# Thealexbarney/VGAudio

Measured on AMD Instinct MI355X. Metric: Msamples/s encoded (GC-ADPCM, 4096 ch) at 1/2/4/8 GPUs; % HBM roofline, higher is better.
Workload: dtype int32; 1 GPU; BASELINE configs[1]: 4096 mono channels x 48 kHz x 60 s GC-ADPCM coefficient search + encode per GPU; parallelism=units sharded x1, channels_per_gpu=4096, samples_per_channel=2880000, bit_exact_channels_checked=0

## Files before the change

### include/vgaudio_hip_testing.h

```cpp
#ifndef VGAUDIO_HIP_TESTING_H
#define VGAUDIO_HIP_TESTING_H

#ifdef __cplusplus
extern "C" {
#endif

int vga_testing_force_open_seams_this_thread(int mode);

int vga_testing_gc_encoder_layout_this_thread(int channels_per_wave);
int vga_testing_gc_coefs_variant_this_thread(int variant);
int vga_testing_gc_encoder_segments_this_thread(int segments);
int vga_testing_gc_encoder_persistent_this_thread(int mode);

int vga_testing_gc_plan_pieces(int cus, int groups, int frames, long long group_frames, int ragged, int *out5);

int vga_testing_gc_encode_stats(unsigned long long *out8, int reset);
int vga_testing_gc_encode_stats_n(unsigned long long *out, int n, int reset);

int vga_testing_gc_seam_handover_this_thread(int on);
int vga_testing_gc_slow_order_host(const short *coefs, int nch, int *order);
int vga_testing_gc_slow_order_device(const void *d_coefs, int nch, int *order);

void vga_testing_host_pipeline_this_thread(int feeders, int drainers, int chunk_units, int slot_bytes);

void vga_testing_host_pipeline_tail_this_thread(int tail_units);

int vga_testing_plan_buckets(const int *group, const int *length, int n, int max_units, long long max_volume, int longest_first,
                             int *order_out, int *chunk_begin_out, int *chunk_length_out, int *chunk_group_out, int max_chunks);
void vga_testing_buckets_order_this_thread(int order);
void vga_testing_host_transfer_this_thread(int mode);
void vga_testing_host_transfer_piece_bytes_this_thread(int bytes);
void vga_testing_host_compute_lanes_this_thread(int lanes);

enum {
    VGA_TESTING_STEP_CHUNK_COMPUTE = 1,
    VGA_TESTING_STEP_TRANSFER = 2,
    VGA_TESTING_STEP_HCA_STREAM_FRAMES = 3
};
void vga_testing_fail_step_this_thread(int kind, int nth);

int vga_testing_last_pipeline_stats(double *out, int n);

int vga_testing_hca_frames_per_group_this_thread(int frames);

int vga_testing_hca_device_info(const void *hca_info, void *out, int out_bytes);

int vga_testing_hca_decode_classes(const void *infos, int nstreams, int *class_out);
int vga_testing_hca_decode_v_stats(long long *out, int n);
int vga_testing_hca_ragged_stats(const void *ragged, long long *out, int n);

int vga_testing_adx_read_general_this_thread(int on);

int vga_testing_adx_last_path_this_thread(int *encode, int *decode);
int vga_testing_adx_ragged_stats(const void *ragged, long long *out, int n);

int vga_testing_poison_allocations(int byte);

#ifdef __cplusplus
}
#endif
#endif
```

### vgaudio_amd/_lib.py

```python
import ctypes as C
import importlib.util
import os

_HERE = os.path.dirname(os.path.abspath(__file__))
SO_PATH = os.environ.get("VGAUDIO_HIP_LIBRARY") or os.path.join(_HERE, "libvgaudio_hip.so")

VGA_OK = 0
VGA_ERR_ARGUMENT = -1
VGA_ERR_OUT_OF_RANGE = -2
VGA_ERR_INVALID_DATA = -3
VGA_ERR_INVALID_OP = -4
VGA_ERR_DEVICE = -5

VGA_TESTING_STEP_CHUNK_COMPUTE = 1
VGA_TESTING_STEP_TRANSFER = 2
VGA_TESTING_STEP_HCA_STREAM_FRAMES = 3


class VgaError(RuntimeError):
    code = None


class ArgumentError(VgaError, ValueError):
    code = VGA_ERR_ARGUMENT


class ArgumentOutOfRangeError(ArgumentError):
    code = VGA_ERR_OUT_OF_RANGE


class InvalidDataError(VgaError):
    code = VGA_ERR_INVALID_DATA


class InvalidOperationError(VgaError):
    code = VGA_ERR_INVALID_OP


class DeviceError(VgaError):
    code = VGA_ERR_DEVICE


PROGRESS_FN = C.CFUNCTYPE(None, C.c_void_p, C.c_int64, C.c_int64)


class reporting:

    def __init__(self, progress, per_unit):
        self.progress, self.per_unit, self.last, self.fn = progress, per_unit, 0, None

    def _report(self, _user, done, _total):
        self.progress.ReportAdd((done - self.last) * self.per_unit)
        self.last = done

    def __enter__(self):
        if self.progress is not None:
            self.fn = PROGRESS_FN(self._report)
            lib().vga_set_progress_callback(C.cast(self.fn, C.c_void_p), None)
        return self

    def __exit__(self, *exc):
        if self.fn is not None:
            lib().vga_set_progress_callback(None, None)
        return False


_EXC = {e.code: e for e in (ArgumentError, ArgumentOutOfRangeError, InvalidDataError, InvalidOperationError,
                            DeviceError)}

_lib = None

i16p = C.POINTER(C.c_int16)
u8p = C.POINTER(C.c_uint8)
u32p = C.POINTER(C.c_uint32)
i16pp = C.POINTER(i16p)
u8pp = C.POINTER(u8p)
vp = C.c_void_p
i64 = C.c_int64
ci = C.c_int


class ADPCMINFO(C.Structure):
    _pack_ = 1
    _fields_ = [("coef", C.c_int16 * 16), ("gain", C.c_uint16), ("pred_scale", C.c_uint16), ("yn1", C.c_int16),
                ("yn2", C.c_int16), ("loop_pred_scale", C.c_uint16), ("loop_yn1", C.c_int16), ("loop_yn2", C.c_int16)]


SIGNATURES = {
    "vga_last_error": (C.c_char_p, []),
    "vga_device_count": (ci, []),
    "vga_set_device": (ci, [ci]),
    "vga_version": (C.c_char_p, []),
    "vga_gcadpcm_nibble_count_to_sample_count": (ci, [ci]),
    "vga_gcadpcm_sample_count_to_nibble_count": (ci, [ci]),
    "vga_gcadpcm_nibble_to_sample": (ci, [ci]),
    "vga_gcadpcm_sample_to_nibble": (ci, [ci]),
    "vga_gcadpcm_sample_count_to_byte_count": (ci, [ci]),
    "vga_gcadpcm_byte_count_to_sample_count": (ci, [ci]),
    "vga_gcadpcm_encode_batch": (ci, [i16pp, ci, ci, C.c_int16, C.c_int16, i16p, u8pp]),
    "vga_gcadpcm_calculate_coefficients_batch": (ci, [i16pp, ci, ci, i16p]),
    "vga_gcadpcm_encode_with_coefs_batch": (ci, [i16pp, ci, ci, ci, i16p, i16p, i16p, u8pp]),
    "vga_gcadpcm_decode_batch": (ci, [u8pp, i16p, ci, ci, i16p, i16p, i16pp]),
    "vga_gcadpcm_encode_batch_v": (ci, [i16pp, C.POINTER(ci), ci, i16p, i16p, i16p, u8pp]),
    "vga_gcadpcm_calculate_coefficients_batch_v": (ci, [i16pp, C.POINTER(ci), ci, i16p]),
    "vga_gcadpcm_encode_with_coefs_batch_v": (ci, [i16pp, C.POINTER(ci), ci, i16p, i16p, i16p, u8pp]),
    "vga_gcadpcm_decode_batch_v": (ci, [u8pp, i16p, C.POINTER(ci), ci, i16p, i16p, i16pp]),
    "vga_gcadpcm_ragged_create": (ci, [C.POINTER(ci), ci, C.POINTER(vp)]),
    "vga_gcadpcm_ragged_destroy": (None, [vp]),
    "vga_gcadpcm_ragged_channels": (ci, [vp]),
    "vga_gcadpcm_ragged_pcm_samples": (i64, [vp]),
    "vga_gcadpcm_ragged_adpcm_bytes": (i64, [vp]),
    "vga_gcadpcm_ragged_coefs_workspace_bytes": (C.c_size_t, [vp]),
    "vga_gcadpcm_ragged_offsets": (ci, [vp, C.POINTER(i64), C.POINTER(i64)]),
    "vga_gcadpcm_coefs_device_v": (ci, [vp, vp, vp, vp, C.c_size_t, vp]),
    "vga_gcadpcm_encode_device_v": (ci, [vp, vp, vp, vp, vp, vp, vp]),
    "vga_gcadpcm_decode_device_v": (ci, [vp, vp, vp, vp, vp, vp, vp, vp]),
    "encode": (None, [i16p, u8p, C.POINTER(ADPCMINFO), C.c_uint32]),
    "decode": (None, [u8p, i16p, C.POINTER(ADPCMINFO), C.c_uint32]),
    "correlateCoefs": (None, [i16p, C.c_uint32, i16p]),
    "encodeFrame": (None, [i16p, u8p, i16p, C.c_uint8]),
    "vga_gcadpcm_coefs_workspace_bytes": (C.c_size_t, [ci, ci]),
    "vga_gcadpcm_coefs_device": (ci, [vp, i64, ci, ci, vp, vp, C.c_size_t, vp]),
    "vga_gcadpcm_encode_device": (ci, [vp, i64, ci, ci, vp, vp, vp, vp, i64, vp]),
    "vga_gcadpcm_decode_device": (ci, [vp, i64, vp, ci, ci, vp, vp, vp, i64, vp, vp]),
    "vga_synth_pcm16_device": (ci, [vp, i64, ci, ci, ci, vp, vp]),
    "vga_adx_file_layout_for": (ci, [vp, ci, vp]),
    "vga_adx_write": (ci, [u8pp, ci, i16p, ci, vp, u8p]),
    "vga_adx_write_device": (ci, [vp, i64, ci, vp, ci, vp, vp, vp]),
    "vga_hca_file_size": (ci, [vp]),
    "vga_hca_file_header": (ci, [vp, C.c_char_p, C.c_float, ci, ci, u8p]),
    "vga_hca_write": (ci, [vp, u8p, C.c_char_p, C.c_float, ci, ci, u8p]),
    "vga_hca_write_device": (ci, [vp, vp, i64, ci, C.c_char_p, C.c_float, ci, ci, vp, i64, vp]),
    "vga_wave_parse": (ci, [u8p, i64, vp]),
    "vga_wave_read_pcm16": (ci, [u8p, i64, vp, i16pp]),
    "vga_wave_deinterleave_pcm16_device": (ci, [vp, ci, ci, vp, i64, vp]),
    "vga_wave_file_size": (i64, [vp, ci]),
    "vga_wave_write_pcm16": (ci, [i16pp, ci, vp, u8p]),
    "vga_wave_write_pcm16_device": (ci, [vp, i64, ci, vp, vp, vp]),
    "vga_adx_key_from_code": (ci, [C.c_uint64, vp]),
    "vga_adx_key_from_string": (ci, [C.c_char_p, vp]),
    "vga_adx_key_code": (C.c_uint64, [vp]),
    "vga_adx_crypt": (ci, [u8pp, ci, ci, vp, ci, ci]),
    "vga_adx_crypt_device": (ci, [vp, i64, ci, ci, vp, ci, ci, vp]),
    "vga_adx_find_key_device": (ci, [vp, i64, ci, ci, ci, ci, vp, ci, C.POINTER(ci), vp]),
    "vga_hca_key_tables": (ci, [ci, C.c_uint64, u8p, u8p]),
    "vga_hca_crypt": (ci, [u8p, ci, ci, u8p]),
    "vga_hca_find_key": (ci, [vp, u8p, ci, u8p, ci, vp]),
    "vga_hca_find_key_device": (ci, [vp, vp, ci, u8p, ci, vp, vp]),
    "vga_hca_byte_position_counts_device": (ci, [vp, i64, ci, ci, ci, ci, vp, vp]),
    "vga_adx_guess_default_candidates": (ci, [ci, vp, vp, vp, vp]),
    "vga_adx_guess_keys": (ci, [vp, ci, ci, ci, vp, ci, vp, ci, vp, ci, vp]),
    "vga_hca_crypt_device": (ci, [vp, i64, ci, ci, ci, u8p, vp]),
    "vga_release_cached_memory": (None, []),
    "vga_testing_force_open_seams_this_thread": (ci, [ci]),
    "vga_testing_host_pipeline_this_thread": (None, [ci, ci, ci, ci]),
    "vga_testing_gc_encoder_layout_this_thread": (ci, [ci]),
    "vga_testing_gc_coefs_variant_this_thread": (ci, [ci]),
    "vga_testing_gc_encoder_segments_this_thread": (ci, [ci]),
    "vga_testing_gc_encoder_persistent_this_thread": (ci, [ci]),
    "vga_testing_gc_seam_handover_this_thread": (ci, [ci]),
    "vga_testing_gc_slow_order_host": (ci, [vp, ci, vp]),
    "vga_testing_gc_slow_order_device": (ci, [vp, ci, vp]),
    "vga_testing_gc_encode_stats_n": (ci, [C.POINTER(C.c_ulonglong), ci, ci]),
    "vga_testing_last_pipeline_stats": (ci, [vp, ci]),
    "vga_testing_host_pipeline_tail_this_thread": (None, [ci]),
    "vga_testing_buckets_order_this_thread": (None, [ci]),
    "vga_testing_host_transfer_this_thread": (None, [ci]),
    "vga_testing_host_transfer_piece_bytes_this_thread": (None, [ci]),
    "vga_testing_host_compute_lanes_this_thread": (None, [ci]),
    "vga_testing_fail_step_this_thread": (None, [ci, ci]),
    "vga_testing_poison_allocations": (ci, [ci]),
    "vga_testing_plan_buckets": (ci, [C.POINTER(ci), C.POINTER(ci), ci, ci, C.c_longlong, ci, C.POINTER(ci), C.POINTER(ci), C.POINTER(ci),
                                 C.POINTER(ci), ci]),
    "vga_testing_hca_device_info": (ci, [vp, vp, ci]),
    "vga_testing_hca_decode_classes": (ci, [vp, ci, C.POINTER(ci)]),
    "vga_testing_hca_decode_v_stats": (ci, [C.POINTER(C.c_longlong), ci]),
    "vga_testing_hca_ragged_stats": (ci, [vp, C.POINTER(C.c_longlong), ci]),
    "vga_hca_ragged_layout_for": (ci, [vp, ci, C.POINTER(i64), C.POINTER(i64), vp]),
    "vga_hca_ragged_create": (ci, [vp, ci, C.POINTER(vp)]),
    "vga_hca_ragged_destroy": (None, [vp]),
    "vga_hca_ragged_streams": (ci, [vp]),
    "vga_hca_ragged_totals_of": (ci, [vp, vp]),
    "vga_hca_ragged_offsets": (ci, [vp, C.POINTER(i64), C.POINTER(i64)]),
    "vga_testing_adx_ragged_stats": (ci, [vp, C.POINTER(C.c_longlong), ci]),
    "vga_adx_ragged_layout_for": (ci, [vp, C.POINTER(ci), ci, C.POINTER(i64), C.POINTER(i64), vp]),
    "vga_adx_ragged_create": (ci, [vp, C.POINTER(ci), ci, C.POINTER(vp)]),
    "vga_adx_ragged_destroy": (None, [vp]),
    "vga_adx_ragged_channels": (ci, [vp]),
    "vga_adx_ragged_totals_of": (ci, [vp, vp]),
    "vga_adx_ragged_offsets": (ci, [vp, C.POINTER(i64), C.POINTER(i64)]),
    "vga_adx_encode_device_v": (ci, [vp, vp, vp, vp, vp, C.c_size_t, vp]),
    "vga_adx_decode_device_v": (ci, [vp, vp, vp, vp, C.c_size_t, vp, vp]),
    "vga_gc_files_layout_for": (ci, [vp, ci, vp, C.POINTER(ci), C.POINTER(i64), C.POINTER(i64), vp]),
    "vga_gc_files_create": (ci, [vp, ci, vp, C.POINTER(vp)]),
    "vga_gc_files_create_from_dsp": (ci, [C.POINTER(vp), ci, C.POINTER(i64), C.POINTER(vp)]),
    "vga_gc_files_destroy": (None, [vp]),
    "vga_gc_files_totals_of": (ci, [vp, vp]),
    "vga_gc_files_offsets": (ci, [vp, C.POINTER(ci), C.POINTER(i64), C.POINTER(i64)]),
    "vga_gc_files_ragged": (vp, [vp]),
    "vga_gcadpcm_build_channels_device_v": (ci, [vp, vp, vp, vp, vp, vp, vp, vp, C.c_size_t, vp]),
    "vga_dsp_write_device_v": (ci, [vp, vp, vp, vp, vp, vp, vp, vp]),
    "vga_dsp_read_device_v": (ci, [vp, vp, vp, vp, vp, vp, vp, vp]),
    "vga_gc_aligned_layout_for": (ci, [vp, ci, C.POINTER(ci), C.POINTER(i64), vp]),
    "vga_gc_aligned_create": (ci, [vp, ci, C.POINTER(vp)]),
    "vga_gc_aligned_destroy": (None, [vp]),
    "vga_gc_aligned_totals_of": (ci, [vp, vp]),
    "vga_gc_aligned_offsets": (ci, [vp, C.POINTER(ci), C.POINTER(i64)]),
    "vga_gc_aligned_ragged_in": (vp, [vp]),
    "vga_gc_aligned_ragged_out": (vp, [vp]),
    "vga_gcadpcm_align_channels_device_v": (ci, [vp, vp, vp, vp, vp, vp, vp, vp, vp, C.c_size_t, vp]),
    "vga_nw_files_layout_for": (ci, [vp, ci, vp, C.POINTER(ci), C.POINTER(i64), C.POINTER(i64), vp]),
    "vga_nw_files_create": (ci, [vp, ci, vp, C.POINTER(vp)]),
    "vga_nw_files_create_from_infos": (ci, [C.POINTER(vp), ci, C.POINTER(i64), C.POINTER(vp)]),
    "vga_nw_files_destroy": (None, [vp]),
    "vga_nw_files_totals_of": (ci, [vp, vp]),
    "vga_nw_files_offsets": (ci, [vp, C.POINTER(ci), C.POINTER(i64), C.POINTER(i64)]),
    "vga_nw_files_gc_files": (ci, [vp, vp]),
    "vga_nw_files_ragged": (vp, [vp]),
    "vga_nwstm_write_device_v": (ci, [vp, vp, vp, vp, vp, vp, vp, vp, vp]),
    "vga_nwstm_read_device_v": (ci, [vp, vp, vp, vp, vp, vp, vp, vp]),
    "vga_idsp_files_layout_for": (ci, [vp, ci, vp, C.POINTER(ci), C.POINTER(i64), vp]),
    "vga_idsp_files_create": (ci, [vp, ci, vp, C.POINTER(vp)]),
    "vga_idsp_files_create_from_infos": (ci, [C.POINTER(vp), ci, C.POINTER(i64), C.POINTER(vp)]),
    "vga_idsp_files_destroy": (None, [vp]),
    "vga_idsp_files_totals_of": (ci, [vp, vp]),
    "vga_idsp_files_offsets": (ci, [vp, C.POINTER(ci), C.POINTER(i64)]),
    "vga_idsp_files_gc_files": (ci, [vp, vp]),
    "vga_idsp_files_ragged": (vp, [vp]),
    "vga_idsp_write_device_v": (ci, [vp, vp, vp, vp, vp, vp, vp, vp]),
    "vga_idsp_read_device_v": (ci, [vp, vp, vp, vp, vp, vp, vp, vp]),
    "vga_idsp_files_write_regions_for": (ci, [vp, ci, vp, vp, i64, C.POINTER(i64)]),
    "vga_idsp_files_read_regions_for": (ci, [C.POINTER(vp), ci, C.POINTER(i64), vp, i64, C.POINTER(i64)]),
    "vga_idsp_files_stats": (ci, [vp, C.POINTER(i64)]),
    "vga_hps_files_layout_for": (ci, [vp, ci, C.POINTER(ci), C.POINTER(i64), C.POINTER(i64), vp]),
    "vga_hps_files_create": (ci, [vp, ci, C.POINTER(vp)]),
    "vga_hps_files_create_from_infos": (ci, [C.POINTER(vp), C.POINTER(vp), ci, C.POINTER(i64), C.POINTER(vp)]),
    "vga_hps_files_destroy": (None, [vp]),
    "vga_hps_files_totals_of": (ci, [vp, vp]),
    "vga_hps_files_offsets": (ci, [vp, C.POINTER(ci), C.POINTER(i64), C.POINTER(i64)]),
    "vga_hps_files_gc_files": (ci, [vp, vp]),
    "vga_hps_files_ragged": (vp, [vp]),
    "vga_hps_write_device_v": (ci, [vp, vp, vp, vp, vp, vp, vp, vp]),
    "vga_hps_read_device_v": (ci, [vp, vp, vp, vp, vp, vp, vp, vp]),
    "vga_hps_files_write_regions_for": (ci, [vp, ci, vp, i64, C.POINTER(i64)]),
    "vga_hps_files_read_regions_for": (ci, [C.POINTER(vp), C.POINTER(vp), ci, C.POINTER(i64), vp, i64, C.POINTER(i64)]),
    "vga_hps_files_stats": (ci, [vp, C.POINTER(i64)]),
    "vga_hca_decode_device_v": (ci, [vp, vp, vp, vp, C.c_size_t, vp, vp]),
    "vga_hca_encode_device_v": (ci, [vp, vp, vp, vp, vp]),
    "vga_hca_stream_create": (ci, [vp, vp, C.POINTER(vp)]),
    "vga_hca_stream_encode": (ci, [vp, vp, u8p, C.POINTER(ci)]),
    "vga_hca_stream_pending_frame_count": (ci, [vp]),
    "vga_hca_stream_get_pending_frame": (ci, [vp, u8p]),
    "vga_hca_stream_frames_processed": (ci, [vp]),
    "vga_hca_stream_frame_size": (ci, [vp]),
    "vga_hca_stream_destroy": (None, [vp]),
    "vga_testing_gc_encode_stats": (ci, [C.POINTER(C.c_ulonglong), ci]),
    "vga_testing_gc_plan_pieces": (ci, [ci, ci, ci, C.c_longlong, ci, C.POINTER(ci)]),
    "vga_set_devices": (ci, [vp, ci]),
    "vga_set_progress_callback": (ci, [vp, vp]),
    "vga_get_devices": (ci, [vp, ci]),
    "vga_testing_hca_frames_per_group_this_thread": (ci, [ci]),
    "vga_dsp_layout_for": (ci, [vp, ci, vp]),
    "vga_dsp_write": (ci, [u8pp, ci, i16p, i16p, i16p, i16p, ci, vp, u8p]),
    "vga_dsp_write_device": (ci, [vp, i64, ci, vp, vp, vp, vp, ci, vp, vp, vp]),
    "vga_nwstm_layout_for": (ci, [vp, ci, vp]),
    "vga_nwstm_write_device": (ci, [vp, ci, ci, vp, vp, i64, ci, vp, vp, vp, vp, vp, i64, ci, vp, i64, vp]),
    "vga_nwstm_write": (ci, [vp, ci, vp, u8pp, ci, i16p, i16p, i16p, i16p, i16pp, ci, u8p]),
    "vga_nwstm_parse": (ci, [u8p, C.c_size_t, vp]),
    "vga_nwstm_read_device": (ci, [vp, vp, i64, ci, vp, i64, vp]),
    "vga_nwstm_read": (ci, [u8p, C.c_size_t, vp, u8pp, i16pp]),
    "vga_pcm8_encode_device": (ci, [vp, i64, ci, ci, ci, vp, i64, vp]),
    "vga_pcm8_decode_device": (ci, [vp, i64, ci, ci, ci, vp, i64, vp]),
    "vga_nwstm_pcm_layout_for": (ci, [vp, ci, ci, vp]),
    "vga_nwstm_pcm_write_device": (ci, [vp, ci, ci, ci, vp, vp, ci, i64, vp, i64, vp]),
    "vga_nwstm_pcm_write": (ci, [vp, ci, ci, vp, vp, ci, u8p]),
    "vga_nwstm_pcm_parse": (ci, [u8p, C.c_size_t, vp]),
    "vga_nwstm_pcm_read_device": (ci, [vp, vp, i64, ci, vp, ci, i64, vp]),
    "vga_nwstm_pcm_read": (ci, [u8p, C.c_size_t, vp, vp, ci]),
    "vga_nwwav_parse": (ci, [u8p, C.c_size_t, vp]),
    "vga_nwwav_read": (ci, [u8p, C.c_size_t, vp, u8pp]),
    "vga_nwwav_bank_create": (ci, [vp, C.POINTER(i64), ci, C.POINTER(vp)]),
    "vga_nwwav_bank_destroy": (None, [vp]),
    "vga_nwwav_bank_channels": (ci, [vp]),
    "vga_nwwav_bank_codec_channels": (ci, [vp, ci]),
    "vga_nwwav_bank_rows": (ci, [vp, C.POINTER(ci), C.POINTER(ci), C.POINTER(ci), C.POINTER(ci), C.POINTER(i64)]),
    "vga_nwwav_bank_gc_sample_counts": (ci, [vp, C.POINTER(ci)]),
    "vga_nwwav_bank_gc_tables": (ci, [vp, i16p, i16p, i16p, i16p]),
    "vga_nwwav_bank_adpcm_bytes": (i64, [vp]),
    "vga_nwwav_bank_pcm16_samples": (i64, [vp]),
    "vga_nwwav_bank_pcm8_bytes": (i64, [vp]),
    "vga_nwwav_bank_source_bytes": (i64, [vp]),
    "vga_nwwav_bank_read_device": (ci, [vp, vp, vp, vp, vp, vp]),
    "vga_wave_pcm8_file_size": (i64, [vp, ci]),
    "vga_wave_write_pcm8": (ci, [vp, ci, ci, vp, u8p]),
    "vga_wave_write_pcm8_device": (ci, [vp, ci, i64, ci, vp, vp, vp]),
    "vga_wave_read_pcm8": (ci, [u8p, i64, vp, vp, ci]),
    "vga_wave_deinterleave_pcm8_device": (ci, [vp, ci, ci, vp, ci, i64, vp]),
    "vga_hps_layout_for": (ci, [vp, ci, vp]),
    "vga_hps_block_map": (ci, [vp, ci, vp, ci]),
    "vga_hps_write_device": (ci, [vp, ci, ci, vp, i64, ci, vp, vp, vp, vp, i64, ci, vp, i64, vp]),
    "vga_hps_write": (ci, [vp, ci, u8pp, ci, i16p, i16p, i16p, i16pp, ci, u8p]),
    "vga_hps_parse": (ci, [u8p, C.c_size_t, vp, vp, ci]),
    "vga_hps_read_device": (ci, [vp, vp, vp, i64, ci, vp, i64, vp]),
    "vga_hps_read": (ci, [u8p, C.c_size_t, vp, vp, u8pp]),
    "vga_idsp_layout_for": (ci, [vp, ci, vp]),
    "vga_idsp_write_device": (ci, [vp, ci, ci, vp, i64, ci, vp, vp, vp, vp, vp, i64, vp]),
    "vga_idsp_write": (ci, [vp, ci, u8pp, ci, i16p, i16p, i16p, i16p, u8p]),
    "vga_idsp_parse": (ci, [u8p, C.c_size_t, vp]),
    "vga_idsp_read_device": (ci, [vp, vp, i64, ci, vp, i64, vp]),
    "vga_idsp_read": (ci, [u8p, C.c_size_t, vp, u8pp]),
    "vga_genh_parse": (ci, [u8p, C.c_size_t, vp]),
    "vga_genh_read_device": (ci, [vp, vp, i64, ci, vp, i64, vp]),
    "vga_genh_read": (ci, [u8p, C.c_size_t, vp, u8pp]),
    "vga_dsp_parse": (ci, [u8p, C.c_size_t, vp]),
    "vga_dsp_read_device": (ci, [vp, vp, i64, ci, vp, i64, vp]),
    "vga_dsp_read": (ci, [u8p, C.c_size_t, vp, u8pp]),
    "vga_adx_parse": (ci, [u8p, C.c_size_t, vp]),
    "vga_adx_read_device": (ci, [vp, vp, i64, ci, vp, i64, vp]),
    "vga_adx_read": (ci, [u8p, C.c_size_t, vp, u8pp]),
    "vga_hca_parse": (ci, [u8p, C.c_size_t, vp]),
    "vga_hca_read_device": (ci, [vp, vp, i64, ci, vp, i64, vp, vp]),
    "vga_hca_read": (ci, [u8p, C.c_size_t, vp, u8p, C.POINTER(ci)]),
    "vga_testing_adx_read_general_this_thread": (ci, [ci]),
    "vga_testing_adx_last_path_this_thread": (ci, [C.POINTER(ci), C.POINTER(ci)]),
    "vga_gcadpcm_channel_layout_for": (ci, [vp, vp]),
    "vga_gcadpcm_build_channels_batch": (ci, [u8pp, i16p, ci, vp, u8pp, i16pp, i16pp, i16p]),
    "vga_gcadpcm_build_channels_workspace_bytes": (C.c_size_t, [ci, vp]),
    "vga_gcadpcm_build_channels_device": (ci, [vp, i64, vp, ci, vp, vp, i64, vp, i64, vp, i64, vp, vp, C.c_size_t, vp]),
    "vga_adx_default_params": (None, [vp]),
    "vga_adx_calculate_coefficients": (ci, [ci, ci, i16p]),
    "vga_adx_nibble_count_to_sample_count": (ci, [ci, ci]),
    "vga_adx_sample_count_to_nibble_count": (ci, [ci, ci]),
    "vga_adx_sample_count_to_byte_count": (ci, [ci, ci]),
    "vga_adx_encoded_byte_count": (ci, [ci, vp]),
    "vga_adx_encode_batch": (ci, [i16pp, ci, ci, vp, u8pp, i16p]),
    "vga_adx_decode_batch": (ci, [u8pp, ci, ci, ci, vp, i16pp]),
    "vga_adx_encode_batch_v": (ci, [i16pp, C.POINTER(ci), ci, vp, u8pp, i16p]),
    "vga_adx_decode_batch_v": (ci, [u8pp, C.POINTER(ci), ci, C.POINTER(ci), vp, i16pp]),
    "vga_hca_encode_batch_v": (ci, [i16pp, ci, vp, vp, u8pp]),
    "vga_hca_decode_batch_v": (ci, [vp, u8pp, ci, i16pp]),
    "vga_adx_encode_device": (ci, [vp, i64, ci, ci, vp, vp, i64, vp, vp]),
    "vga_adx_decode_device": (ci, [vp, i64, ci, ci, ci, vp, vp, i64, vp, vp]),
    "vga_hca_encoder_initialize": (ci, [vp, vp]),
    "vga_hca_encode_batch": (ci, [i16pp, ci, vp, vp, u8pp]),
    "vga_hca_decode_batch": (ci, [vp, u8pp, ci, i16pp]),
    "vga_hca_decode_workspace_bytes": (C.c_size_t, [vp, ci]),
    "vga_hca_encode_device": (ci, [vp, i64, i64, ci, ci, vp, vp, i64, vp, vp]),
    "vga_hca_decode_device": (ci, [vp, vp, i64, ci, vp, i64, i64, vp, C.c_size_t, vp, vp]),
    "vga_adx_files_layout_for": (ci, [vp, ci, C.POINTER(i64), C.POINTER(ci), C.POINTER(i64), C.POINTER(i64), vp]),
    "vga_adx_files_create": (ci, [vp, ci, C.POINTER(i64), C.POINTER(vp)]),
    "vga_adx_files_create_from_infos": (ci, [vp, ci, C.POINTER(i64), C.POINTER(vp)]),
    "vga_adx_files_destroy": (None, [vp]),
    "vga_adx_files_totals_of": (ci, [vp, vp]),
    "vga_adx_files_offsets": (ci, [vp, C.POINTER(ci), C.POINTER(i64), C.POINTER(i64)]),
    "vga_adx_write_device_v": (ci, [vp, vp, vp, vp, vp]),
    "vga_adx_read_device_v": (ci, [vp, vp, vp, vp, vp]),
    "vga_adx_files_write_items_for": (ci, [vp, ci, C.POINTER(i64), ci, vp, i64, C.POINTER(i64)]),
    "vga_adx_files_read_items_for": (ci, [vp, ci, C.POINTER(i64), ci, vp, i64, C.POINTER(i64)]),
    "vga_adx_files_stats": (ci, [vp, C.POINTER(i64)]),
    "vga_adx_files_force_general_this_thread": (ci, [ci]),
    "vga_wave_files_layout_for": (ci, [vp, ci, C.POINTER(i64), C.POINTER(i64), C.POINTER(ci), C.POINTER(i64), C.POINTER(i64), vp]),
    "vga_wave_files_create": (ci, [vp, ci, C.POINTER(i64), C.POINTER(i64), C.POINTER(vp)]),
    "vga_wave_files_create_from_infos": (ci, [vp, ci, C.POINTER(i64), C.POINTER(i64), C.POINTER(vp)]),
    "vga_wave_files_destroy": (None, [vp]),
    "vga_wave_files_totals_of": (ci, [vp, vp]),
    "vga_wave_files_offsets": (ci, [vp, C.POINTER(ci), C.POINTER(i64), C.POINTER(i64)]),
    "vga_wave_read_device_v": (ci, [vp, vp, vp, vp]),
    "vga_wave_write_device_v": (ci, [vp, vp, vp, vp]),
    "vga_wave_files_write_items_for": (ci, [vp, ci, C.POINTER(i64), C.POINTER(i64), ci, vp, i64, C.POINTER(i64)]),
    "vga_wave_files_read_items_for": (ci, [vp, ci, C.POINTER(i64), C.POINTER(i64), ci, vp, i64, C.POINTER(i64)]),
    "vga_wave_files_stats": (ci, [vp, C.POINTER(i64)]),
    "vga_wave_files_force_general_this_thread": (ci, [ci]),
    "vga_nw_pcm_files_layout_for": (ci, [vp, ci, vp, ci, C.POINTER(i64), C.POINTER(i64), C.POINTER(ci), C.POINTER(i64), C.POINTER(i64), vp]),
    "vga_nw_pcm_files_create": (ci, [vp, ci, vp, ci, C.POINTER(i64), C.POINTER(i64), C.POINTER(vp)]),
    "vga_nw_pcm_files_create_from_infos": (ci, [vp, ci, C.POINTER(i64), C.POINTER(i64), C.POINTER(vp)]),
    "vga_nw_pcm_files_destroy": (None, [vp]),
    "vga_nw_pcm_files_totals_of": (ci, [vp, vp]),
    "vga_nw_pcm_files_offsets": (ci, [vp, C.POINTER(ci), C.POINTER(i64), C.POINTER(i64)]),
    "vga_nwstm_pcm_write_device_v": (ci, [vp, vp, vp, vp]),
    "vga_nwstm_pcm_read_device_v": (ci, [vp, vp, vp, vp]),
    "vga_nw_pcm_files_write_items_for": (ci, [vp, ci, vp, ci, C.POINTER(i64), C.POINTER(i64), ci, vp, i64, C.POINTER(i64)]),
    "vga_nw_pcm_files_read_items_for": (ci, [vp, ci, C.POINTER(i64), C.POINTER(i64), ci, vp, i64, C.POINTER(i64)]),
    "vga_nw_pcm_files_stats": (ci, [vp, C.POINTER(i64)]),
    "vga_nw_pcm_files_force_general_this_thread": (ci, [ci]),
    "vga_hca_files_layout_for": (ci, [vp, ci, C.POINTER(i64), C.POINTER(i64), C.POINTER(i64), vp]),
    "vga_hca_files_create": (ci, [vp, ci, C.POINTER(i64), vp, ci, C.POINTER(vp)]),
    "vga_hca_files_create_from_infos": (ci, [vp, ci, C.POINTER(i64), C.POINTER(ci), vp, ci, C.POINTER(i64), C.POINTER(vp)]),
    "vga_hca_files_destroy": (None, [vp]),
    "vga_hca_files_totals_of": (ci, [vp, vp]),
    "vga_hca_files_offsets": (ci, [vp, C.POINTER(i64), C.POINTER(i64)]),
    "vga_hca_write_device_v": (ci, [vp, vp, vp, vp]),
    "vga_hca_read_device_v": (ci, [vp, vp, vp, vp, vp]),
    "vga_hca_files_write_items_for": (ci, [vp, ci, C.POINTER(i64), ci, vp, i64, C.POINTER(i64)]),
    "vga_hca_files_read_items_for": (ci, [vp, ci, C.POINTER(i64), C.POINTER(i64), ci, vp, i64, C.POINTER(i64)]),
    "vga_hca_files_stats": (ci, [vp, C.POINTER(i64)]),
    "vga_hca_files_force_general_this_thread": (ci, [ci]),
}


class AdxFileParamsC(C.Structure):
    _fields_ = [(n, C.c_int) for n in ("sample_rate", "sample_count", "looping", "loop_start", "loop_end", "alignment_samples",
                                       "frame_size", "version", "type", "highpass_frequency", "encryption_type", "trim_file")]


class AdxFileLayoutC(C.Structure):
    _fields_ = [(n, C.c_int) for n in ("sample_count", "frame_count", "base_header_size", "alignment_bytes", "header_size",
                                       "audio_offset", "audio_size", "footer_offset", "footer_size", "loop_start_offset",
                                       "loop_end_offset", "file_size")]


class AdxFileC(C.Structure):
    _fields_ = [("channels", C.c_int), ("params", AdxFileParamsC)]


class AdxFilesTotalsC(C.Structure):
    _fields_ = [("files", C.c_int), ("channels", C.c_int), ("audio_bytes", C.c_int64), ("image_bytes", C.c_int64)]


class AdxFilesItemC(C.Structure):
    _fields_ = [("form", C.c_int), ("file", C.c_int), ("x", C.c_int), ("y", C.c_uint32), ("granule", C.c_int),
                ("begin", C.c_int64), ("end", C.c_int64), ("keep_end", C.c_int64)]


class WaveInfoC(C.Structure):
    _fields_ = ([(n, C.c_int) for n in ("channel_count", "sample_rate", "bits_per_sample", "sample_count", "sample_count_declared",
                                        "looping", "loop_start", "loop_end")]
                + [("data_offset", C.c_int64), ("data_size", C.c_int), ("data_size_declared", C.c_int)])


class WaveParamsC(C.Structure):
    _fields_ = [(n, C.c_int) for n in ("sample_rate", "sample_count", "looping", "loop_start", "loop_end")]


class WaveFileC(C.Structure):
    _fields_ = [("channels", C.c_int), ("bits", C.c_int), ("params", WaveParamsC)]


class WaveFilesTotalsC(C.Structure):
    _fields_ = [("files", C.c_int), ("channels", C.c_int), ("pcm_samples", C.c_int64), ("image_bytes", C.c_int64)]


class WaveFilesItemC(C.Structure):
    _fields_ = [("form", C.c_int), ("file", C.c_int), ("x", C.c_int), ("y", C.c_uint32), ("span", C.c_int),
                ("begin", C.c_int64), ("end", C.c_int64)]


class AdxKeyC(C.Structure):
    _fields_ = [("seed", C.c_int), ("mult", C.c_int), ("inc", C.c_int)]


class DspParamsC(C.Structure):
    _fields_ = [(n, C.c_int) for n in ("sample_rate", "sample_count", "looping", "loop_start", "loop_end",
                                       "samples_per_interleave", "loop_point_alignment", "trim_file")]


class DspLayoutC(C.Structure):
    _fields_ = [(n, C.c_int) for n in ("sample_count", "loop_start", "loop_end", "start_addr", "end_addr", "cur_addr",
                                       "bytes_per_interleave", "frames_per_interleave", "audio_data_size", "file_size")]


class GcChannelParamsC(C.Structure):
    _fields_ = [(n, C.c_int) for n in ("sample_count", "looping", "loop_start", "loop_end", "loop_alignment_multiple",
                                       "samples_per_seek_table_entry")]


class GcChannelLayoutC(C.Structure):
    _fields_ = [(n, C.c_int) for n in ("alignment_needed", "loop_start_aligned", "sample_count_aligned",
                                       "seek_table_entries")]


class GcFileC(C.Structure):
    _fields_ = [("channels", C.c_int), ("sample_rate", C.c_int), ("channel", GcChannelParamsC)]


class DspFileConfigC(C.Structure):
    _fields_ = [(n, C.c_int) for n in ("samples_per_interleave", "loop_point_alignment", "trim_file")]


class GcFilesTotalsC(C.Structure):
    _fields_ = [("files", C.c_int), ("channels", C.c_int), ("pcm_samples", C.c_int64), ("adpcm_bytes", C.c_int64),
                ("seek_shorts", C.c_int64), ("image_bytes", C.c_int64), ("build_workspace_bytes", C.c_size_t)]


class GcAlignedTotalsC(C.Structure):
    _fields_ = [("files", C.c_int), ("channels", C.c_int), ("aligned_channels", C.c_int), ("pcm_samples", C.c_int64),
                ("adpcm_bytes", C.c_int64), ("out_pcm_samples", C.c_int64), ("out_adpcm_bytes", C.c_int64), ("seek_shorts", C.c_int64),
                ("workspace_bytes", C.c_size_t)]


NW_MAX_CHANNELS = NW_MAX_TRACKS = 255


class NwTrackC(C.Structure):
    _fields_ = [(n, C.c_int) for n in ("channel_count", "left", "right", "volume", "panning")]


class NwParamsC(C.Structure):
    _fields_ = ([(n, C.c_int) for n in ("target", "sample_rate", "sample_count", "looping", "loop_start", "loop_end",
                                        "samples_per_interleave", "samples_per_seek_table_entry", "loop_point_alignment",
                                        "track_type", "seek_table_type")]
                + [("version", C.c_uint32)]
                + [(n, C.c_int) for n in ("endianness", "track_count", "keep_seek_table", "keep_loop_context")])


class NwLayoutC(C.Structure):
    _fields_ = ([("target", C.c_int), ("endianness", C.c_int), ("version", C.c_uint32)]
                + [(n, C.c_int) for n in ("include_track_info", "include_region_info", "include_unaligned_loop",
                                          "version_word", "looping", "loop_start", "loop_end", "sample_count",
                                          "alignment_needed")]
                + [("channel", GcChannelParamsC)]
                + [(n, C.c_int) for n in (
                    "channel_sample_count", "channel_adpcm_bytes", "channel_seek_entries", "samples_per_interleave",
                    "interleave_size", "interleave_count", "last_block_samples", "last_block_size_without_padding",
                    "last_block_size", "samples_per_seek_table_entry", "bytes_per_seek_table_entry",
                    "seek_table_entry_count", "track_count", "header_size", "head_block_offset", "head_block_size",
                    "head1_size", "head2_size", "head3_size", "seek_block_offset", "seek_block_size",
                    "data_block_offset", "data_block_size", "audio_data_offset", "audio_data_size", "file_size")])


class NwInfoC(C.Structure):
    _fields_ = ([("target", C.c_int), ("endianness", C.c_int), ("version", C.c_uint32)]
                + [(n, C.c_int) for n in (
                    "codec", "looping", "loop_start", "sample_count", "sample_rate", "channel_count", "has_unaligned_loop",
                    "loop_start_unaligned", "loop_end_unaligned", "interleave_count", "interleave_size",
                    "samples_per_interleave", "last_block_size_without_padding", "last_block_samples", "last_block_size",
                    "bytes_per_seek_table_entry", "samples_per_seek_table_entry", "track_type", "seek_table_type",
                    "has_track_info", "track_count")]
                + [("tracks", NwTrackC * NW_MAX_TRACKS), ("coefs", (C.c_int16 * 16) * NW_MAX_CHANNELS),
                   ("gain", C.c_int16 * NW_MAX_CHANNELS), ("start_context", (C.c_int16 * 3) * NW_MAX_CHANNELS),
                   ("loop_context", (C.c_int16 * 3) * NW_MAX_CHANNELS)]
                + [(n, C.c_int) for n in (
                    "seek_table_offset", "seek_entries", "seek_big_endian", "head_block_offset", "head_block_size",
                    "seek_block_offset", "seek_block_size", "data_block_offset", "data_block_size", "audio_data_offset",
                    "audio_data_length", "adpcm_bytes", "file_size")])


class NwFileC(C.Structure):
    _fields_ = [(n, C.c_int) for n in ("channels", "sample_rate", "sample_count", "looping", "loop_start", "loop_end")]


class NwFileConfigC(C.Structure):
    _fields_ = ([(n, C.c_int) for n in ("target", "samples_per_interleave", "samples_per_seek_table_entry", "loop_point_alignment",
                                        "track_type", "seek_table_type")]
                + [("version", C.c_uint32), ("endianness", C.c_int)])


class NwFilesTotalsC(C.Structure):
    _fields_ = [("files", C.c_int), ("channels", C.c_int), ("pcm_samples", C.c_int64), ("adpcm_bytes", C.c_int64),
                ("seek_shorts", C.c_int64), ("image_bytes", C.c_int64)]


class NwPcmFilesTotalsC(C.Structure):
    _fields_ = [("files", C.c_int), ("channels", C.c_int), ("pcm_samples", C.c_int64), ("image_bytes", C.c_int64)]


class NwPcmFilesItemC(C.Structure):
    _fields_ = [("form", C.c_int), ("file", C.c_int), ("x", C.c_int), ("y", C.c_uint32), ("conv", C.c_int),
                ("begin", C.c_int64), ("end", C.c_int64)]


# ... 202 lines not shown
```

### vgaudio_amd/csrc/capi_gcadpcm.hip

```cpp
#include "gc_capi.hpp"
#include "../../include/vgaudio_hip_testing.h"

using namespace vga;

extern "C" {

int vga_testing_gc_plan_pieces(int cus, int groups, int frames, long long group_frames, int ragged, int *out5)
{
    if (!out5 || cus <= 0 || groups <= 0 || frames <= 0) return -1;
    bool persistent = false;
    gc::Pieces seg;
    const int segments = gc::plan_encode_pieces_on(cus, groups, frames, group_frames, ragged != 0, &persistent, &seg,
                                                     encoder_layout() == 1 ? 1 : 8);
    out5[0] = segments;
    out5[1] = seg.big;
    out5[2] = seg.nb;
    out5[3] = seg.small;
    out5[4] = persistent ? 1 : 0;
    return 0;
}

int vga_gcadpcm_nibble_count_to_sample_count(int nibble_count) { return gc::nibble_count_to_sample_count(nibble_count); }
int vga_gcadpcm_sample_count_to_nibble_count(int sample_count) { return gc::sample_count_to_nibble_count(sample_count); }
int vga_gcadpcm_nibble_to_sample(int nibble) { return gc::nibble_to_sample(nibble); }
int vga_gcadpcm_sample_to_nibble(int sample) { return gc::sample_to_nibble(sample); }
int vga_gcadpcm_sample_count_to_byte_count(int sample_count) { return gc::sample_count_to_byte_count(sample_count); }
int vga_gcadpcm_byte_count_to_sample_count(int byte_count) { return gc::byte_count_to_sample_count(byte_count); }

size_t vga_gcadpcm_coefs_workspace_bytes(int nch, int length)
{
    if (nch <= 0 || length < 0) return 0;
    const size_t frames = ((size_t)length + 13) / 14;
    return (size_t)nch * (size_t)vga::gc::coef_record_pitch((int64_t)frames) * 16;
}

int vga_gcadpcm_coefs_device(const int16_t *d_pcm, int64_t pcm_pitch, int nch, int length, int16_t *d_coefs,
                             void *d_workspace, size_t workspace_bytes, void *stream)
{
    if (nch < 0 || length < 0) { set_error("negative size"); return VGA_ERR_ARGUMENT; }
    if (nch == 0) return VGA_OK;
    if (int rc = gc::check_pcm_layout(d_pcm, pcm_pitch, length, "vga_gcadpcm_coefs_device")) return rc;
    if (workspace_bytes < vga_gcadpcm_coefs_workspace_bytes(nch, length) || !d_workspace) {
        set_error("workspace too small: need %zu bytes", vga_gcadpcm_coefs_workspace_bytes(nch, length));
        return VGA_ERR_ARGUMENT;
    }
    return gc::launch_coefs(d_pcm, pcm_pitch, nch, length, d_coefs, d_workspace, (hipStream_t)stream);
}

int vga_gcadpcm_encode_device(const int16_t *d_pcm, int64_t pcm_pitch, int nch, int sample_count,
                              const int16_t *d_coefs, const int16_t *d_hist1, const int16_t *d_hist2,
                              uint8_t *d_adpcm, int64_t adpcm_pitch, void *stream)
{
    if (nch < 0 || sample_count < 0) { set_error("negative size"); return VGA_ERR_ARGUMENT; }
    if (nch == 0 || sample_count == 0) return VGA_OK;
    if (int rc = gc::check_pcm_layout(d_pcm, pcm_pitch, sample_count, "vga_gcadpcm_encode_device")) return rc;
    if (int rc = gc::check_adpcm_layout(d_adpcm, adpcm_pitch, gc::sample_count_to_byte_count(sample_count),
                                    "vga_gcadpcm_encode_device"))
        return rc;
    return gc::launch_encode(d_pcm, pcm_pitch, nch, sample_count, d_coefs, d_hist1, d_hist2, d_adpcm, adpcm_pitch,
                             (hipStream_t)stream);
}

int vga_gcadpcm_decode_device(const uint8_t *d_adpcm, int64_t adpcm_pitch, const int16_t *d_coefs, int nch,
                              int sample_count, const int16_t *d_hist1, const int16_t *d_hist2, int16_t *d_pcm,
                              int64_t pcm_pitch, int *d_status, void *stream)
{
    if (nch < 0 || sample_count < 0) { set_error("negative size"); return VGA_ERR_ARGUMENT; }
    if (nch == 0 || sample_count == 0) return VGA_OK;
    if (int rc = gc::check_pcm_layout(d_pcm, pcm_pitch, sample_count, "vga_gcadpcm_decode_device")) return rc;
    if (int rc = gc::check_adpcm_layout(d_adpcm, adpcm_pitch, gc::sample_count_to_byte_count(sample_count),
                                    "vga_gcadpcm_decode_device"))
        return rc;
    return gc::launch_decode(d_adpcm, adpcm_pitch, d_coefs, nch, sample_count, d_hist1, d_hist2, d_pcm, pcm_pitch,
                             d_status, (hipStream_t)stream);
}

int vga_synth_pcm16_device(int16_t *d_pcm, int64_t pcm_pitch, int nch, int length, int first_channel,
                           const uint32_t *d_params, void *stream)
{
    if (nch < 0 || length < 0 || pcm_pitch < length) { set_error("bad synth arguments"); return VGA_ERR_ARGUMENT; }
    return gc::launch_synth(d_pcm, pcm_pitch, nch, length, first_channel, d_params, (hipStream_t)stream);
}

static constexpr int GC_CHUNK_CHANNELS = 1024;

static int calculate_coefficients_batch_one(const int16_t *const *pcm, int nch, int length, int16_t *coefs_out)
{
    if (length < 0) { set_error("negative length"); return VGA_ERR_ARGUMENT; }
    if (int rc = gc::check_ptrs((const void *const *)pcm, length > 0 ? nch : 0, "pcm")) return rc;
    if (nch < 0 || (nch > 0 && !coefs_out)) { set_error("bad coefs_out/nch"); return VGA_ERR_ARGUMENT; }
    if (nch == 0) return VGA_OK;
    if (int rc = require_device()) return rc;
    gc::GcBatch b;
    b.pcm_pitch = round_up(length > 0 ? length : 1, 8);
    VGA_HIP_TRY(b.pcm.alloc((size_t)nch * b.pcm_pitch * sizeof(int16_t)));
    VGA_HIP_TRY(b.coefs.alloc((size_t)nch * 32));
    pipe::Job job;
    job.units = nch;
    if (length > 0) bind_in(job, (const void *const *)pcm, (size_t)length * sizeof(int16_t), b.pcm.as<char>(), (size_t)b.pcm_pitch * sizeof(int16_t));
    job.compute = chunk_compute([&](int first, int count, hipStream_t s) {
        return gc::launch_coefs(b.pcm.as<int16_t>() + (int64_t)first * b.pcm_pitch, b.pcm_pitch, count, length,
                                b.coefs.as<int16_t>() + (int64_t)first * 16, b.ws.p, s);
    });
    VGA_HIP_TRY(b.ws.alloc(vga_gcadpcm_coefs_workspace_bytes(planned_chunk_units(job, GC_CHUNK_CHANNELS), length)));
    if (int rc = run_batch_pipeline(job, GC_CHUNK_CHANNELS)) return rc;
    VGA_HIP_TRY(hipMemcpy(coefs_out, b.coefs.p, (size_t)nch * 32, hipMemcpyDeviceToHost));
    return VGA_OK;
}

int vga_gcadpcm_calculate_coefficients_batch(const int16_t *const *pcm, int nch, int length, int16_t *coefs_out)
{
    if (nch <= 0 || !pcm || !coefs_out) return calculate_coefficients_batch_one(pcm, nch, length, coefs_out);
    return for_each_device_share(nch, gc::GC_MIN_SHARE_CHANNELS, [&](int first, int count) {
        return calculate_coefficients_batch_one(pcm + first, count, length, coefs_out + (size_t)first * 16);
    });
}

static int encode_with_coefs_batch_one(const int16_t *const *pcm, int nch, int pcm_length, int sample_count, const int16_t *coefs,
                                      const int16_t *hist1, const int16_t *hist2, uint8_t *const *adpcm_out)
{
    if (sample_count == -1) sample_count = pcm_length;
    if (pcm_length < 0 || sample_count < 0) { set_error("negative length"); return VGA_ERR_ARGUMENT; }
    if (sample_count > pcm_length) {
        set_error("SampleCount (%d) exceeds pcm length (%d)", sample_count, pcm_length);
        return VGA_ERR_ARGUMENT;
    }
    if (int rc = gc::check_ptrs((const void *const *)pcm, sample_count > 0 ? nch : 0, "pcm")) return rc;
    if (int rc = gc::check_ptrs((const void *const *)adpcm_out, sample_count > 0 ? nch : 0, "adpcm_out")) return rc;
    if (nch > 0 && !coefs) { set_error("null coefs"); return VGA_ERR_ARGUMENT; }
    if (nch <= 0 || sample_count == 0) return nch < 0 ? VGA_ERR_ARGUMENT : VGA_OK;
    if (int rc = require_device()) return rc;
    gc::GcBatch b;
    VGA_HIP_TRY(b.st.create());
    b.pcm_pitch = round_up(sample_count, 8);
    VGA_HIP_TRY(b.pcm.alloc((size_t)nch * b.pcm_pitch * sizeof(int16_t)));
    if (int rc = gc::upload_hist(b.h1, b.h2, nch, hist1, hist2, &b.st)) return rc;
    VGA_HIP_TRY(b.coefs.alloc((size_t)nch * 32));
    VGA_HIP_TRY(hipMemcpyAsync(b.coefs.p, coefs, (size_t)nch * 32, hipMemcpyHostToDevice, b.st.s));
    VGA_HIP_TRY(hipStreamSynchronize(b.st.s));
    const int nbytes = gc::sample_count_to_byte_count(sample_count);
    b.adpcm_pitch = round_up(nbytes, 16);
    VGA_HIP_TRY(b.adpcm.alloc((size_t)nch * b.adpcm_pitch));
    DevBuf scratch;
    pipe::Job job;
    job.units = nch;
    bind_in(job, (const void *const *)pcm, (size_t)sample_count * sizeof(int16_t), b.pcm.as<char>(), (size_t)b.pcm_pitch * sizeof(int16_t));
    bind_out(job, (void *const *)adpcm_out, (size_t)nbytes, b.adpcm.as<char>(), (size_t)b.adpcm_pitch);
    job.compute = chunk_compute([&](int first, int count, hipStream_t s) {
        return gc::launch_encode(b.pcm.as<int16_t>() + (int64_t)first * b.pcm_pitch, b.pcm_pitch, count, sample_count,
                                 b.coefs.as<int16_t>() + (int64_t)first * 16,
                                 b.h1.p ? b.h1.as<int16_t>() + first : nullptr, b.h2.p ? b.h2.as<int16_t>() + first : nullptr,
                                 b.adpcm.as<uint8_t>() + (int64_t)first * b.adpcm_pitch, b.adpcm_pitch, s, scratch.p, scratch.bytes);
    });
    VGA_HIP_TRY(scratch.alloc(gc::encode_scratch_bytes(planned_chunk_units(job, GC_CHUNK_CHANNELS))));
    return run_batch_pipeline(job, GC_CHUNK_CHANNELS);
}

int vga_gcadpcm_encode_with_coefs_batch(const int16_t *const *pcm, int nch, int pcm_length, int sample_count,
                                        const int16_t *coefs, const int16_t *hist1, const int16_t *hist2,
                                        uint8_t *const *adpcm_out)
{
    if (nch <= 0 || !pcm || !coefs || !adpcm_out)
        return encode_with_coefs_batch_one(pcm, nch, pcm_length, sample_count, coefs, hist1, hist2, adpcm_out);
    return for_each_device_share(nch, gc::GC_MIN_SHARE_CHANNELS, [&](int first, int count) {
        return encode_with_coefs_batch_one(pcm + first, count, pcm_length, sample_count, coefs + (size_t)first * 16,
                                          hist1 ? hist1 + first : nullptr, hist2 ? hist2 + first : nullptr, adpcm_out + first);
    });
}

static int encode_batch_one(const int16_t *const *pcm, int nch, int sample_count, int16_t hist1, int16_t hist2, int16_t *coefs_out,
                           uint8_t *const *adpcm_out)
{
    if (sample_count < 0) { set_error("negative sample count"); return VGA_ERR_ARGUMENT; }
    if (int rc = gc::check_ptrs((const void *const *)pcm, sample_count > 0 ? nch : 0, "pcm")) return rc;
    if (int rc = gc::check_ptrs((const void *const *)adpcm_out, sample_count > 0 ? nch : 0, "adpcm_out")) return rc;
    if (nch < 0 || (nch > 0 && !coefs_out)) { set_error("bad coefs_out/nch"); return VGA_ERR_ARGUMENT; }
    if (nch == 0) return VGA_OK;
    if (int rc = require_device()) return rc;
    const double t_entry = pipe::detail::now();
    gc::GcBatch b;
    VGA_HIP_TRY(b.st.create());
    b.pcm_pitch = round_up(sample_count > 0 ? sample_count : 1, 8);
    VGA_HIP_TRY(b.pcm.alloc((size_t)nch * b.pcm_pitch * sizeof(int16_t)));
    std::vector<int16_t> h1v((size_t)nch, hist1), h2v((size_t)nch, hist2);
    const bool use_hist = hist1 != 0 || hist2 != 0;
    if (use_hist)
        if (int rc = gc::upload_hist(b.h1, b.h2, nch, h1v.data(), h2v.data(), &b.st)) return rc;
    VGA_HIP_TRY(hipStreamSynchronize(b.st.s));
    VGA_HIP_TRY(b.coefs.alloc((size_t)nch * 32));
    const int nbytes = gc::sample_count_to_byte_count(sample_count);
    b.adpcm_pitch = round_up(nbytes > 0 ? nbytes : 1, 16);
    VGA_HIP_TRY(b.adpcm.alloc((size_t)nch * b.adpcm_pitch));
    DevBuf scratch[pipe::kMaxComputeLanes], ws[pipe::kMaxComputeLanes];
    pipe::Job job;
    job.units = nch;
    job.compute_lanes = nch > 1 ? planned_compute_lanes(hardware_queues_requested() >= 6 ? 2 : 1) : 1;
    if (sample_count > 0) {
        bind_in(job, (const void *const *)pcm, (size_t)sample_count * sizeof(int16_t), b.pcm.as<char>(), (size_t)b.pcm_pitch * sizeof(int16_t));
        bind_out(job, (void *const *)adpcm_out, (size_t)nbytes, b.adpcm.as<char>(), (size_t)b.adpcm_pitch);
    }
    job.compute = chunk_compute([&](int first, int count, hipStream_t s) {
        const int lane = pipe::compute_lane();
        int rc = gc::launch_coefs(b.pcm.as<int16_t>() + (int64_t)first * b.pcm_pitch, b.pcm_pitch, count, sample_count,
                                  b.coefs.as<int16_t>() + (int64_t)first * 16, ws[lane].p, s);
        if (!rc)
            rc = gc::launch_encode(b.pcm.as<int16_t>() + (int64_t)first * b.pcm_pitch, b.pcm_pitch, count, sample_count,
                                   b.coefs.as<int16_t>() + (int64_t)first * 16,
                                   b.h1.p ? b.h1.as<int16_t>() + first : nullptr, b.h2.p ? b.h2.as<int16_t>() + first : nullptr,
                                   b.adpcm.as<uint8_t>() + (int64_t)first * b.adpcm_pitch, b.adpcm_pitch, s, scratch[lane].p,
                                   scratch[lane].bytes);
        return rc;
    });
    const int chunk = planned_chunk_units(job, GC_CHUNK_CHANNELS);
    for (int l = 0; l < job.compute_lanes; l++) {
        VGA_HIP_TRY(scratch[l].alloc(gc::encode_scratch_bytes(chunk)));
        VGA_HIP_TRY(ws[l].alloc(vga_gcadpcm_coefs_workspace_bytes(chunk, sample_count)));
    }
    pipe_report().t_alloc = pipe::detail::now() - t_entry;
    if (int rc = run_batch_pipeline(job, GC_CHUNK_CHANNELS)) return rc;
    VGA_HIP_TRY(hipMemcpy(coefs_out, b.coefs.p, (size_t)nch * 32, hipMemcpyDeviceToHost));
    pipe_report().t_entry = pipe::detail::now() - t_entry;
    return VGA_OK;
}

int vga_gcadpcm_encode_batch(const int16_t *const *pcm, int nch, int sample_count, int16_t hist1, int16_t hist2,
                             int16_t *coefs_out, uint8_t *const *adpcm_out)
{
    if (nch <= 0 || !pcm || !coefs_out || !adpcm_out) return encode_batch_one(pcm, nch, sample_count, hist1, hist2, coefs_out, adpcm_out);
    return for_each_device_share(nch, gc::GC_MIN_SHARE_CHANNELS, [&](int first, int count) {
        return encode_batch_one(pcm + first, count, sample_count, hist1, hist2, coefs_out + (size_t)first * 16, adpcm_out + first);
    });
}

static int decode_batch_one(const uint8_t *const *adpcm, const int16_t *coefs, int nch, int sample_count, const int16_t *hist1,
                           const int16_t *hist2, int16_t *const *pcm_out)
{
    if (sample_count < 0) { set_error("negative sample count"); return VGA_ERR_ARGUMENT; }
    if (int rc = gc::check_ptrs((const void *const *)adpcm, sample_count > 0 ? nch : 0, "adpcm")) return rc;
    if (int rc = gc::check_ptrs((const void *const *)pcm_out, sample_count > 0 ? nch : 0, "pcm_out")) return rc;
    if (nch > 0 && !coefs) { set_error("null coefs"); return VGA_ERR_ARGUMENT; }
    if (nch <= 0 || sample_count == 0) return nch < 0 ? VGA_ERR_ARGUMENT : VGA_OK;
    if (int rc = require_device()) return rc;
    gc::GcBatch b;
    VGA_HIP_TRY(b.st.create());
    const int nbytes = gc::sample_count_to_byte_count(sample_count);
    b.adpcm_pitch = round_up(nbytes, 16);
    b.pcm_pitch = round_up(sample_count, 8);
    VGA_HIP_TRY(b.adpcm.alloc((size_t)nch * b.adpcm_pitch));
    VGA_HIP_TRY(b.pcm.alloc((size_t)nch * b.pcm_pitch * 2));
    VGA_HIP_TRY(b.coefs.alloc((size_t)nch * 32));
    VGA_HIP_TRY(b.status.alloc(sizeof(int)));
    VGA_HIP_TRY(hipMemsetAsync(b.status.p, 0, sizeof(int), b.st.s));
    VGA_HIP_TRY(hipMemcpyAsync(b.coefs.p, coefs, (size_t)nch * 32, hipMemcpyHostToDevice, b.st.s));
    if (int rc = gc::upload_hist(b.h1, b.h2, nch, hist1, hist2, &b.st)) return rc;
    VGA_HIP_TRY(hipStreamSynchronize(b.st.s));
    pipe::Job job;
    job.units = nch;
    bind_in(job, (const void *const *)adpcm, (size_t)nbytes, b.adpcm.as<char>(), (size_t)b.adpcm_pitch);
    bind_out(job, (void *const *)pcm_out, (size_t)sample_count * 2, b.pcm.as<char>(), (size_t)b.pcm_pitch * 2);
    job.compute_lanes = planned_compute_lanes(1);
    job.compute = chunk_compute([&](int first, int count, hipStream_t s) {
        return gc::launch_decode(b.adpcm.as<uint8_t>() + (int64_t)first * b.adpcm_pitch, b.adpcm_pitch,
                                 b.coefs.as<int16_t>() + (int64_t)first * 16, count, sample_count,
                                 b.h1.p ? b.h1.as<int16_t>() + first : nullptr, b.h2.p ? b.h2.as<int16_t>() + first : nullptr,
                                 b.pcm.as<int16_t>() + (int64_t)first * b.pcm_pitch, b.pcm_pitch, b.status.as<int>(), s);
    });
    return run_status_job(job, 2 * GC_CHUNK_CHANNELS, b.status, gc::BAD_PREDICTOR);
}

int vga_gcadpcm_decode_batch(const uint8_t *const *adpcm, const int16_t *coefs, int nch, int sample_count,
                             const int16_t *hist1, const int16_t *hist2, int16_t *const *pcm_out)
{
    if (nch <= 0 || !adpcm || !coefs || !pcm_out) return decode_batch_one(adpcm, coefs, nch, sample_count, hist1, hist2, pcm_out);
    return for_each_device_share(nch, gc::GC_MIN_SHARE_CHANNELS, [&](int first, int count) {
        return decode_batch_one(adpcm + first, coefs + (size_t)first * 16, count, sample_count, hist1 ? hist1 + first : nullptr,
                               hist2 ? hist2 + first : nullptr, pcm_out + first);
    });
}

void correlateCoefs(int16_t *src, uint32_t samples, int16_t *coefsOut)
{
    const int16_t *chans[1] = {src};
    (void)vga_gcadpcm_calculate_coefficients_batch(chans, 1, (int)samples, coefsOut);
}

void encode(int16_t *src, uint8_t *dst, ADPCMINFO *cxt, uint32_t samples)
{
    const int16_t *chans[1] = {src};
    uint8_t *outs[1] = {dst};
    int16_t coefs[16];
    if (vga_gcadpcm_encode_batch(chans, 1, (int)samples, 0, 0, coefs, outs) != VGA_OK) return;
    if (cxt) {
        memset(cxt, 0, sizeof *cxt);
        memcpy(cxt->coef, coefs, sizeof coefs);
        cxt->pred_scale = samples ? dst[0] : 0;
    }
}

void decode(uint8_t *src, int16_t *dst, ADPCMINFO *cxt, uint32_t samples)
{
    if (!cxt) return;
    const uint8_t *ins[1] = {src};
    int16_t *outs[1] = {dst};
    int16_t coefs[16];
    memcpy(coefs, cxt->coef, sizeof coefs);
    const int16_t h1 = cxt->yn1, h2 = cxt->yn2;
    (void)vga_gcadpcm_decode_batch(ins, coefs, 1, (int)samples, &h1, &h2, outs);
}

void encodeFrame(int16_t *src, uint8_t *dst, int16_t *coefs, uint8_t one)
{
    (void)one;
    const int16_t *chans[1] = {src + 2};
    uint8_t *outs[1] = {dst};
    const int16_t h2 = src[0], h1 = src[1];
    if (vga_gcadpcm_encode_with_coefs_batch(chans, 1, 14, 14, coefs, &h1, &h2, outs) != VGA_OK) return;
    const uint8_t *ins[1] = {dst};
    int16_t *rec[1] = {src + 2};
    (void)vga_gcadpcm_decode_batch(ins, coefs, 1, 14, &h1, &h2, rec);
}

// ... 2 lines not shown
```

### vgaudio_amd/csrc/common.hpp

```cpp
#pragma once
#include <hip/hip_runtime.h>
#include <cstdarg>
#include <cstdint>
#include <cstdio>
#include <cstdlib>
#include <cstring>
#include <mutex>
#include <vector>

#include "../../include/vgaudio_hip.h"
#include "poison.hpp"

namespace vga {

void set_error(const char *fmt, ...);
bool take_error_pending();

#define VGA_HIP_TRY(expr)                                                              \
    do {                                                                               \
        hipError_t _e = (expr);                                                        \
        if (_e != hipSuccess) {                                                        \
            vga::set_error("%s failed: %s (%s:%d)", #expr, hipGetErrorString(_e),      \
                           __FILE__, __LINE__);                                        \
            return VGA_ERR_DEVICE;                                                     \
        }                                                                              \
    } while (0)

inline hipError_t poison_block(void *p, size_t bytes)
{
    const int byte = poison_byte();
    if (byte < 0 || !p || !bytes) return hipSuccess;
    const hipError_t e = hipMemset(p, byte, bytes);
    return e != hipSuccess ? e : hipStreamSynchronize(nullptr);
}
inline hipError_t device_malloc(void **out, size_t bytes)
{
    const hipError_t e = hipMalloc(out, bytes);
    return e != hipSuccess ? e : poison_block(*out, bytes);
}

class DevicePool {
public:
    static DevicePool &get()
    {
        static DevicePool pool;
        return pool;
    }
    hipError_t acquire(void **out, size_t bytes)
    {
        const hipError_t e = acquire_block(out, bytes);
        return e != hipSuccess ? e : poison_block(*out, bytes ? bytes : 1);
    }
    void release(void *p)
    {
        std::vector<void *> drop;
        {
            std::lock_guard<std::mutex> g(m_);
            bool pooled = false;
            int device = -1;
            for (auto &b : blocks_)
                if (b.p == p) { b.busy = false; pooled = true; device = b.device; }
            size_t idle = 0;
            for (auto &b : blocks_)
                if (!b.busy && b.device == device) idle += b.bytes;
            if (!pooled) drop.push_back(p);
            const size_t keep = keep_bytes();
            while (idle > keep) {
                int big = -1;
                for (int i = 0; i < (int)blocks_.size(); i++)
                    if (!blocks_[i].busy && blocks_[i].device == device && (big < 0 || blocks_[i].bytes > blocks_[big].bytes)) big = i;
                if (big < 0) break;
                idle -= blocks_[big].bytes;
                drop.push_back(blocks_[big].p);
                blocks_.erase(blocks_.begin() + big);
            }
        }
        for (void *q : drop) (void)hipFree(q);
    }
    void trim()
    {
        std::vector<void *> drop;
        {
            std::lock_guard<std::mutex> g(m_);
            for (int i = (int)blocks_.size() - 1; i >= 0; i--)
                if (!blocks_[i].busy) {
                    drop.push_back(blocks_[i].p);
                    blocks_.erase(blocks_.begin() + i);
                }
        }
        for (void *q : drop) (void)hipFree(q);
    }

    int device_of(void *p)
    {
        std::lock_guard<std::mutex> g(m_);
        for (auto &b : blocks_)
            if (b.p == p) return b.device;
        return -1;
    }

private:
    static constexpr size_t kMinPooled = (size_t)1 << 20;
    hipError_t acquire_block(void **out, size_t bytes)
    {
        if (bytes < kMinPooled) return hipMalloc(out, bytes ? bytes : 1);
        int device = 0;
        (void)hipGetDevice(&device);
        {
            std::lock_guard<std::mutex> g(m_);
            int best = -1;
            for (int i = 0; i < (int)blocks_.size(); i++) {
                const Block &b = blocks_[i];
                if (!b.busy && b.device == device && b.bytes >= bytes && b.bytes / 2 <= bytes &&
                    (best < 0 || b.bytes < blocks_[best].bytes))
                    best = i;
            }
            if (best >= 0) {
                blocks_[best].busy = true;
                *out = blocks_[best].p;
                return hipSuccess;
            }
        }
        hipError_t e = hipMalloc(out, bytes);
        if (e != hipSuccess) {
            trim();
            e = hipMalloc(out, bytes);
        }
        if (e == hipSuccess) {
            std::lock_guard<std::mutex> g(m_);
            blocks_.push_back({*out, bytes, device, true});
        }
        return e;
    }
    static size_t keep_bytes()
    {
        static const size_t v = [] {
            const char *e = std::getenv("VGA_HIP_POOL_GIB");
            const long gib = e ? std::atol(e) : 64;
            return (size_t)(gib < 0 ? 0 : gib) << 30;
        }();
        return v;
    }
    struct Block { void *p; size_t bytes; int device; bool busy; };
    std::mutex m_;
    std::vector<Block> blocks_;
};

struct DevBuf {
    void *p = nullptr;
    size_t bytes = 0;
    DevBuf() = default;
    DevBuf(const DevBuf &) = delete;
    DevBuf &operator=(const DevBuf &) = delete;
    ~DevBuf() { drop(); }
    void drop()
    {
        if (!p) return;
        if (take_error_pending()) {
            const int dev = DevicePool::get().device_of(p);
            int cur = -1;
            if (dev >= 0 && hipGetDevice(&cur) == hipSuccess && cur != dev && hipSetDevice(dev) == hipSuccess) {
                (void)hipDeviceSynchronize();
                (void)hipSetDevice(cur);
            } else
                (void)hipDeviceSynchronize();
        }
        DevicePool::get().release(p);
        p = nullptr;
    }
    hipError_t alloc(size_t n) {
        drop();
        bytes = n;
        return DevicePool::get().acquire(&p, n ? n : 1);
    }
    template <class T> T *as() const { return reinterpret_cast<T *>(p); }
};

struct AsyncBuf {
    void *p = nullptr;
    hipStream_t stream = nullptr;
    AsyncBuf() = default;
    AsyncBuf(const AsyncBuf &) = delete;
    AsyncBuf &operator=(const AsyncBuf &) = delete;
    ~AsyncBuf() { if (p) (void)hipFreeAsync(p, stream); }
    hipError_t alloc(size_t n, hipStream_t s) {
        stream = s;
        const hipError_t e = hipMallocAsync(&p, n ? n : 1, s);
        const int byte = poison_byte();
        return e != hipSuccess || byte < 0 ? e : hipMemsetAsync(p, byte, n ? n : 1, s);
    }
    template <class T> T *as() const { return reinterpret_cast<T *>(p); }
};

template <class F>
inline hipError_t allow_dynamic_lds(F *kernel, size_t bytes)
{
    return hipFuncSetAttribute(reinterpret_cast<const void *>(kernel), hipFuncAttributeMaxDynamicSharedMemorySize, (int)bytes);
}

struct Stream {
    hipStream_t s = nullptr;
    ~Stream() { if (s) (void)hipStreamDestroy(s); }
    hipError_t create() { return hipStreamCreateWithFlags(&s, hipStreamNonBlocking); }
};

inline int64_t round_up(int64_t v, int64_t m) { return (v + m - 1) / m * m; }

__device__ __forceinline__ void lds_barrier()
{
#if defined(__HIP_DEVICE_COMPILE__)
    asm volatile("s_waitcnt lgkmcnt(0)\n\ts_barrier" ::: "memory");
#endif
}

int require_device();

inline int device_cu_count()
{
    int device = 0, cus = 256;
    if (hipGetDevice(&device) == hipSuccess) (void)hipDeviceGetAttribute(&cus, hipDeviceAttributeMultiprocessorCount, device);
    return cus > 0 ? cus : 256;
}

int force_open_seams();

int encoder_layout();
int coefs_kernel_variant();
int encoder_segments_override();
int encoder_persistent_mode();
int hca_frames_per_group_override();
bool gc_seam_handover_off();
void note_adx_encode_path(int path);
void note_adx_decode_path(int path);

__host__ __device__ inline bool seam_forced_open(int mode, int channel, int seam)
{
    return mode == 1 || mode == 3 || (mode == 2 && channel % 3 == 0 && seam % 2 == 0);
}

}
```

### vgaudio_amd/csrc/gc_encode_kernel.hip

```cpp
#include "common.hpp"
#include "gc_encode_core.hpp"
#include "gcadpcm_kernels.hpp"
#include "seams.hpp"
#include "gc_plan8.hpp"

#include <cstdio>
#include <cstdlib>
#include <vector>

namespace vga {
namespace gc {

constexpr int DPP_QUAD_XOR1 = 0xB1;
constexpr int DPP_QUAD_XOR2 = 0x4E;
constexpr int DPP_ROW_HALF_MIRROR = 0x141;
constexpr int DPP_ROW_MIRROR = 0x140;

template <int CTRL>
__device__ __forceinline__ int dpp(int v)
{
    return __builtin_amdgcn_update_dpp(0, v, CTRL, 0xF, 0xF, true);
}

__device__ __forceinline__ unsigned umin32(unsigned a, unsigned b) { return a < b ? a : b; }

template <class Op>
__device__ __forceinline__ unsigned row16_reduce(unsigned v, Op op)
{
    v = op(v, (unsigned)dpp<DPP_QUAD_XOR1>((int)v));
    v = op(v, (unsigned)dpp<DPP_QUAD_XOR2>((int)v));
    v = op(v, (unsigned)dpp<DPP_ROW_HALF_MIRROR>((int)v));
    v = op(v, (unsigned)dpp<DPP_ROW_MIRROR>((int)v));
    return v;
}


#ifdef VGA_DEBUG_TIMESTAMPS
__device__ unsigned long long g_vga_enc_ts[1 << 16];
extern "C" int vga_debug_encode_timestamps(unsigned long long *out, int n)
{
    return (int)hipMemcpyFromSymbol(out, HIP_SYMBOL(g_vga_enc_ts), (size_t)n * sizeof(unsigned long long));
}
#endif
constexpr int GC_STATS = 9;
__device__ unsigned long long g_vga_gc_stats[GC_STATS];
extern "C" int vga_testing_gc_encode_stats_n(unsigned long long *out, int n, int reset)
{
    if (n < 0 || n > GC_STATS) return -1;
    if (hipDeviceSynchronize() != hipSuccess) return -1;
    if (out && n > 0 && hipMemcpyFromSymbol(out, HIP_SYMBOL(g_vga_gc_stats), (size_t)n * sizeof(unsigned long long)) != hipSuccess) return -1;
#ifdef VGA_GC_STATS
    if (out && n > 7) out[7] = 1;
#else
    if (out && n > 7) out[7] = 0;
#endif
    if (reset) {
        const unsigned long long zero[GC_STATS] = {};
        if (hipMemcpyToSymbol(HIP_SYMBOL(g_vga_gc_stats), zero, sizeof zero) != hipSuccess) return -1;
    }
    return 0;
}
extern "C" int vga_testing_gc_encode_stats(unsigned long long *out8, int reset) { return vga_testing_gc_encode_stats_n(out8, 8, reset); }
constexpr int SW = 2;
constexpr int ENC_THREADS = 64 * (SW + 1);
#ifndef VGA_GC_ENCODER_PRIO
#define VGA_GC_ENCODER_PRIO 3
#endif
#ifndef VGA_GC_HELPER_PRIO
#define VGA_GC_HELPER_PRIO 0
#endif
#ifndef VGA_GC_PERSISTENT_WAVES_PER_EU
#define VGA_GC_PERSISTENT_WAVES_PER_EU 3, 3
#endif
template <int CPW, bool SELF = false>
struct Lay {
    static_assert(!SELF || CPW == 8, "the self-served shape is the (channel, predictor) layout");
    static constexpr int EW = SELF ? 1 : SW;
    static constexpr int CS = CPW * EW;
    static constexpr int TF = 64 / CS;
    static constexpr int THREADS = SELF ? 64 : ENC_THREADS;
    static constexpr int BUFS = SELF ? 1 : 2;
};
template <int CS, int TF>
struct GcTileT {
    struct Slot {
        uint32_t xw[8];
        int in2048p[16];
        uint32_t pre[8];
        int4 out[4];
    };
    struct Group { Slot f[TF]; uint32_t pad[4]; };
    Group g[CS];
};
typedef short short2v __attribute__((ext_vector_type(2)));
struct XW7 { uint32_t v[7]; };

#define VGA_COLD __device__ __forceinline__

VGA_COLD int prescan_sequential_cold(XW7 xs, uint32_t hist, int c0, int c1)
{
    int x[16];
    unpack_row(xs.v, hist, x);
    return prescan_sequential(x, c0, c1);
}

#ifdef VGA_GC_R05_COLD
#define VGA_COLD_OPAQUE(v) ((void)0)
#else
#define VGA_COLD_OPAQUE(v) VGA_OPAQUE(v)
#endif
struct ColdState {
    uint32_t xw[7];
    int mp[14];
    uint32_t hist;
    int c0, c1, s1;
    int generic, start, drop, wide, resume;
    int bump_a, ov_a, ov_b;
};
struct ColdOut { PassOutB r; int final_sp; int fin; int sum_exact; };
__device__ __forceinline__
ColdOut encode_frame_cold(ColdState st, PassOutB r, int final_sp, int fin)
{
    uint32_t xw[7];
    int mp[14];
#pragma unroll
    for (int i = 0; i < 7; i++) xw[i] = st.xw[i];
#pragma unroll
    for (int i = 0; i < 14; i++) mp[i] = st.mp[i];
    int sum_exact = 0;
    if (st.drop) fin = 0;
    if (__any(st.generic != 0)) {
        if (st.generic) {
            int xg[16];
            unpack_row(xw, st.hist, xg);
#pragma unroll
            for (int i = 0; i < 16; i++) VGA_COLD_OPAQUE(xg[i]);
            const int start = st.start != -100 ? st.start
                                               : (st.bump_a ? apply_bumps(st.s1, st.ov_a) : apply_bumps(st.s1 + 1, st.ov_b));
            r = as_pass_b(resume_passes(xg, st.c0, st.c1, start, final_sp));
            fin = 1;
            sum_exact = 1;
        }
    }
    if (st.wide) fin = 1;
    if (__any(st.resume != 0)) {
        if (st.resume) {
            int sp = st.s1 + 1;
            for (;;) {
                sp++;
#if defined(VGA_GC_NO_FAST_PASSES) || defined(VGA_GC_NO_FAST_THIRD)
                bool short_pass = false;
#else
                bool short_pass = !__any(sp > 9);
#endif
                if (short_pass) {
                    r = pass_fast_core_b<true>(xw, st.hist, mp, st.c0, st.c1, sp);
                    short_pass = !__any(!pass_no_round_is_exact(sp, r.max_overflow));
                }
                if (!short_pass) r = pass_fast_core_b<false>(xw, st.hist, mp, st.c0, st.c1, sp);
                const bool cap = sp >= 12;
                if ((unsigned)r.max_overflow > (cap ? 3u : 248u)) {
                    int xg[16];
                    unpack_row(xw, st.hist, xg);
#pragma unroll
                    for (int i = 0; i < 16; i++) VGA_COLD_OPAQUE(xg[i]);
                    r = as_pass_b(resume_passes(xg, st.c0, st.c1, sp - 1, final_sp));
                    sum_exact = 1;
                    break;
                }
                final_sp = sp;
                if (cap || r.max_overflow <= 1) break;
            }
            fin = 1;
        }
    }
    ColdOut o;
    o.r = r;
    o.final_sp = final_sp;
    o.fin = fin;
    o.sum_exact = sum_exact;
    return o;
}

template <bool REPAIR, int CPW, bool RAGGED, bool SELF = false>
__device__ __forceinline__ void gc_encode_piece(
    const int bx, const int by,
    const int16_t *__restrict__ pcm, int64_t pcm_pitch, int nch, int total_samples, const Pieces seg,
    const int16_t *__restrict__ coefs, const int16_t *__restrict__ hist1,
    const int16_t *__restrict__ hist2, uint8_t *__restrict__ adpcm, int64_t adpcm_pitch, int16_t *__restrict__ seg_state,
    const int *__restrict__ first_open, const Ragged &rg)
{
    constexpr bool repair = REPAIR;
    constexpr int CS = Lay<CPW, SELF>::CS, TF = Lay<CPW, SELF>::TF, BUFS = Lay<CPW, SELF>::BUFS;
    static_assert(!(SELF && REPAIR), "the repair launch keeps the 2 + 1 shape");
    using GcTile = GcTileT<CS, TF>;
    int64_t first_frame = seg.first(by);
    int repair_piece = 0;
    if (repair) {
        int k = SEAM_OPEN_LIMIT;
        for (int g = 0; g < CS; g++) {
            const int slot = bx * CS + g;
            if (slot < nch) {
                const int c = RAGGED ? rg.order[slot] : slot;
                k = first_open[c] < k ? first_open[c] : k;
            }
        }
        if (!is_open(k)) return;
        repair_piece = k;
        first_frame = seg.first(k);
    }
    const int total_wg = RAGGED ? rg.length[rg.order[bx * CS]] : total_samples;
    if (first_frame * 14 >= total_wg) return;
    const int64_t piece_samples = repair ? (int64_t)0x7fffffff : (int64_t)seg.frames(by) * 14;
    auto piece_samples_of = [&](int total) {
        const int64_t rem = (int64_t)total - first_frame * 14;
        return (int)(rem < 0 ? 0 : (rem < piece_samples ? rem : piece_samples));
    };
    pcm += first_frame * 14;
    adpcm += first_frame * 8;
    using Slot = typename GcTile::Slot;
    static_assert(TF % 2 == 0, "the frame loop takes a tile's frames in pairs");
    struct Tiles { GcTile t[BUFS]; Slot end; };
    __shared__ Tiles s_tiles;
    GcTile (&s_tile)[BUFS] = s_tiles.t;
    __shared__ int s_ncold[Lay<CPW, SELF>::EW];
    const int tid = threadIdx.x;
    const int wave = SELF ? 0 : tid >> 6;
    const bool helper = !SELF && wave == SW;
    const int lane = tid & 63;
    constexpr int LPC = 64 / CPW;
    int grp = helper ? lane / TF : wave * CPW + lane / LPC;
    const int l16 = lane & (LPC - 1);
    const int hfr = lane % TF;
    const int slot_raw = bx * CS + grp;
    const bool live = slot_raw < nch;
    const int slot = live ? slot_raw : nch - 1;
    const int ch = RAGGED ? rg.order[slot] : slot;
    const int16_t *src = pcm + (RAGGED ? rg.pcm_off[ch] : (int64_t)ch * pcm_pitch);
    uint8_t *dst = adpcm + (RAGGED ? rg.adpcm_off[ch] : (int64_t)ch * adpcm_pitch);

    const int sample_count = piece_samples_of(RAGGED ? rg.length[ch] : total_samples);
    const int full_frames = sample_count / 14;
    const int tail = sample_count - full_frames * 14;
    const int frames = full_frames + (tail ? 1 : 0);
    const int frames_wg = RAGGED ? (piece_samples_of(total_wg) + 13) / 14 : frames;
    const int tiles = (frames_wg + TF - 1) / TF;

    auto load_frame = [&](int tile, uint32_t (&w)[7], int (&in)[14]) __attribute__((always_inline)) {
        const int fr = RAGGED ? imax(imin(tile * TF + hfr, frames - 1), 0) : imin(tile * TF + hfr, frames - 1);
        if (fr < full_frames) {
            const uint32_t *p32 = reinterpret_cast<const uint32_t *>(src + (int64_t)fr * 14);
#pragma unroll
            for (int i = 0; i < 7; i++) w[i] = p32[i];
#pragma unroll
            for (int i = 0; i < 7; i++) {
                in[2 * i] = (int)(int16_t)(w[i] & 0xFFFF);
                in[2 * i + 1] = (int)w[i] >> 16;
            }
        } else {
#pragma unroll
            for (int s = 0; s < 14; s++) in[s] = (s < tail) ? (int)src[(int64_t)fr * 14 + s] : 0;
#pragma unroll
            for (int i = 0; i < 7; i++) w[i] = (uint32_t)(in[2 * i] & 0xFFFF) | ((uint32_t)in[2 * i + 1] << 16);
        }
    };
    auto prepare_from = [&](int tile, const uint32_t (&w)[7], const int (&in)[14], const uint32_t (&cpk)[8], const bool numer,
                            auto pair_of) __attribute__((always_inline)) {
        Slot &T = s_tile[tile & (BUFS - 1)].g[grp].f[hfr];
        uint4 *xr = reinterpret_cast<uint4 *>(&T.xw[0]);
        xr[0] = make_uint4(w[0], w[1], w[2], w[3]);
        xr[1] = make_uint4(w[4], w[5], w[6], (!RAGGED || tile * TF + hfr < frames) ? 1u : 0u);
        int4 *qr = reinterpret_cast<int4 *>(&T.in2048p[0]);
        qr[0] = make_int4(pass_b_row(in[0]), pass_b_row(in[1]), pass_b_row(in[2]), pass_b_row(in[3]));
        qr[1] = make_int4(pass_b_row(in[4]), pass_b_row(in[5]), pass_b_row(in[6]), pass_b_row(in[7]));
        qr[2] = make_int4(pass_b_row(in[8]), pass_b_row(in[9]), pass_b_row(in[10]), pass_b_row(in[11]));
        qr[3] = make_int4(pass_b_row(in[12]), pass_b_row(in[13]), 0, 0);
        uint32_t pair[12];
#pragma unroll
        for (int k = 0; k < 12; k++)
            pair[k] = (k & 1) ? __builtin_amdgcn_alignbit(w[(k + 1) / 2], w[(k - 1) / 2], 16) : w[k / 2];
        uint4 *pr = reinterpret_cast<uint4 *>(&T.pre[0]);
        if constexpr (!SELF) {
            uint32_t pre[8];
#pragma unroll
            for (int p = 0; p < 8; p++) {
                int dmax = 0, dmin = 0;
#ifdef VGA_GC_ABLATE_HELPER_PRESCAN
                dmax = in[2 + p] & 1023;
                dmin = -(in[3 + p] & 1023);
#else
#pragma unroll
                for (int k = 0; k < 12; k++) {
                    const int predicted = div2048(__builtin_amdgcn_sdot2(__builtin_bit_cast(short2v, pair[k]),
                                                                         __builtin_bit_cast(short2v, cpk[p]), 0, false));
                    const int d = in[k + 2] - predicted;
                    dmax = imax(dmax, d);
                    dmin = imin(dmin, d);
                }
#endif
                pre[p] = (uint32_t)(clamp16i(dmax) & 0xFFFF) | ((uint32_t)clamp16i(dmin) << 16);
            }
            pr[0] = make_uint4(pre[0], pre[1], pre[2], pre[3]);
            pr[1] = make_uint4(pre[4], pre[5], pre[6], pre[7]);
        } else if (__builtin_expect(numer, 1)) {
            int a2048[12];
#pragma unroll
            for (int k = 0; k < 12; k++) a2048[k] = in[k + 2] * 2048;
            uint32_t pre[8];
#pragma unroll
            for (int q = 0; q < 8; q++) pre[q] = prescan_numer_word(pair, a2048, cpk[q]);
            pr[0] = make_uint4(pre[0], pre[1], pre[2], pre[3]);
            pr[1] = make_uint4(pre[4], pre[5], pre[6], pre[7]);
        } else {
#pragma unroll 1
            for (int q = 0; q < 8; q++) {
                const uint32_t cp = pair_of(q);
                int dmax = 0, dmin = 0;
#pragma unroll
                for (int k = 0; k < 12; k++) {
                    const int d = in[k + 2] - div2048(dot2_i16_wrap(pair[k], cp));
                    dmax = imax(dmax, d);
                    dmin = imin(dmin, d);
                }
                T.pre[q] = sat_pack16(dmax, dmin);
            }
        }
    };
    auto flush = [&](int tile) __attribute__((always_inline)) {
        const int fr = tile * TF + hfr;
        if (!live || fr >= frames) return;
        const int4 *rec = &s_tile[tile & (BUFS - 1)].g[grp].f[hfr].out[0];
        const int4 r0 = rec[0], r1 = rec[1], r2 = rec[2], r3 = rec[3];
        const int q[14] = {r0.x, r0.y, r0.z, r0.w, r1.x, r1.y, r1.z, r1.w, r2.x, r2.y, r2.z, r2.w, r3.x, r3.y};
        uint2 v;
        pack_frame_mod16(q, r3.z, r3.w, v.x, v.y);
        if (fr < full_frames) {
            *reinterpret_cast<uint2 *>(dst + (int64_t)fr * 8) = v;
        } else {
            const int nbytes = (tail + 2 + 1) / 2;
            const uint64_t both = ((uint64_t)v.y << 32) | v.x;
            for (int b = 0; b < nbytes; b++) dst[(int64_t)fr * 8 + b] = (uint8_t)(both >> (8 * b));
        }
    };
    if (helper) {
        __builtin_amdgcn_s_setprio(VGA_GC_HELPER_PRIO);
        uint32_t cpk[8];
#pragma unroll
        for (int p = 0; p < 8; p++)
            cpk[p] = (uint32_t)(uint16_t)coefs[ch * 16 + 2 * p + 1] | ((uint32_t)(uint16_t)coefs[ch * 16 + 2 * p] << 16);
        auto prepare = [&](int tile) {
            uint32_t w[7];
            int in[14];
            load_frame(tile, w, in);
            prepare_from(tile, w, in, cpk, false, [](int) { return 0u; });
        };
        if (tiles > 0) prepare(0);
        __syncthreads();
        for (int tile = 0; tile < tiles; tile++) {
            if (tile + 1 < tiles) prepare(tile + 1);
            if (tile > 0) flush(tile - 1);
            __syncthreads();
        }
        if (tiles > 0) flush(tiles - 1);
        return;
    }

    if constexpr (!SELF) __builtin_amdgcn_s_setprio(VGA_GC_ENCODER_PRIO);
    const int wave_u = __builtin_amdgcn_readfirstlane(wave);
    int p = CPW == 4 ? l16 >> 1 : l16;
    const bool cand_b = CPW == 4 && (l16 & 1) != 0;
    const int c0 = coefs[ch * 16 + 2 * p];
    const int c1 = coefs[ch * 16 + 2 * p + 1];
    const bool coef_ok = pass_b_coef_ok(c0, c1);
    int h0 = hist2 ? hist2[ch] : 0;
    int h1 = hist1 ? hist1[ch] : 0;
    if (repair) {
        h0 = seg_state[((int64_t)(repair_piece - 1) * nch + ch) * 2];
        h1 = seg_state[((int64_t)(repair_piece - 1) * nch + ch) * 2 + 1];
    } else if (by > 0 && (!RAGGED || frames > 0)) {
        h0 = src[-2];
        h1 = src[-1];
    }
    uint32_t hpk = pack16(h0, h1);

    if (lane == 0) s_ncold[wave] = 0;
    struct Row { uint32_t xw[7]; int mp[14]; };
    auto read_row = [&](const Slot &T, Row &R) {
        const uint4 *xr = reinterpret_cast<const uint4 *>(&T.xw[0]);
        const uint4 a0 = xr[0], a1 = xr[1];
        asm volatile("" ::"v"(a1.w));
        uint32_t *xw = R.xw;
        xw[0] = a0.x; xw[1] = a0.y; xw[2] = a0.z; xw[3] = a0.w; xw[4] = a1.x; xw[5] = a1.y; xw[6] = a1.z;
        const int4 *qr = reinterpret_cast<const int4 *>(&T.in2048p[0]);
        const int4 e0 = qr[0], e1 = qr[1], e2 = qr[2], e3 = qr[3];
        asm volatile("" ::"v"(e3.z), "v"(e3.w));
        int *mp = R.mp;
        mp[0] = e0.x; mp[1] = e0.y; mp[2] = e0.z; mp[3] = e0.w; mp[4] = e1.x; mp[5] = e1.y; mp[6] = e1.z; mp[7] = e1.w;
        mp[8] = e2.x; mp[9] = e2.y; mp[10] = e2.z; mp[11] = e2.w; mp[12] = e3.x; mp[13] = e3.y;
    };
    auto read_pre = [&](const Slot &T) __attribute__((always_inline)) -> uint32_t {
        int pp = p;
        asm volatile("" : "+v"(pp));
        return T.pre[pp];
    };
    auto slot_has_frame = [&](const Slot &T) __attribute__((always_inline)) -> bool {
        if constexpr (RAGGED) return T.xw[7] != 0u;
        else return true;
    };
    auto pack = [](const uint32_t (&xw)[7]) {
        XW7 xs;
#pragma unroll
        for (int i = 0; i < 7; i++) xs.v[i] = xw[i];
        return xs;
    };
    const uint32_t cpk = pack16(c1, c0);
    auto wide_total = [&](const uint32_t (&xw)[7], const int (&mp)[14], int sp) -> uint64_t {
        int row[14];
#pragma unroll
        for (int i = 0; i < 14; i++) row[i] = mp[i] - PASS_B_OFF;
        return pass_fast_core_wide(xw, hpk, row, c0, c1, sp).total;
    };
    const bool head_numer = __builtin_amdgcn_ballot_w64(!coef_ok) == 0;
    auto prescan_head = [&](const Row &R, int &d0, int &d1, int &P0) __attribute__((always_inline)) {
        P0 = predicted_b(hpk, cpk);
        if (__builtin_expect(head_numer, 1)) {
            d0 = head_distance_numer_b(R.mp[0], P0);
            d1 = head_distance_numer_b(R.mp[1], predicted_b(__builtin_amdgcn_alignbit(R.xw[0], hpk, 16), cpk));
        } else {
            d0 = pair_lo(R.xw[0]) - div2048(dot2_i16_wrap(hpk, cpk));
            d1 = pair_hi(R.xw[0]) - div2048(dot2_i16_wrap(__builtin_amdgcn_alignbit(R.xw[0], hpk, 16), cpk));
        }
    };
    auto first_scale = [&](const Row &R, uint32_t pre, int d0, int d1) __attribute__((always_inline)) -> int {
        const int dmax = imax(imax((int)(int16_t)(pre & 0xFFFF), d0), d1);
        const int dmin = imin(imin((int)pre >> 16, d0), d1);
        int sum, pos;
        int s1 = first_scale_power_nt(dmax, dmin, sum, pos);
        if (__builtin_expect(__builtin_amdgcn_ballot_w64(sum == 0) != 0, 0)) {
            if (sum == 0 && first_scale_tie(pos)) s1 = first_scale_power_from_md(prescan_sequential_cold(pack(R.xw), hpk, c0, c1));
        }
        return s1;
    };

    auto encode_frame = [&](Row &R, Slot &S, uint32_t pre) {
        const uint32_t (&xw)[7] = R.xw;
        int s1, P0;
        {
            int d0, d1;
            prescan_head(R, d0, d1, P0);
            s1 = first_scale(R, pre, d0, d1);
        }
        int final_sp = imin(s1 + (cand_b ? 1 : 0), 12);
        const bool at_cap = final_sp >= 12;
        const unsigned ov_limit = at_cap ? 3u : 248u;
        PassOutB r = pass_fast_core_b<false, true>(xw, hpk, R.mp, c0, c1, final_sp, P0);
        const bool rare = !coef_ok || (!at_cap && (unsigned)r.max_overflow > ov_limit);
        const int eff = at_cap ? 0 : r.max_overflow;
        const int eff_other = dpp<DPP_QUAD_XOR1>(eff);
        bool fin = eff < 2 && (eff_other | (cand_b ? 0 : 2)) >= 2;
        const bool resume = !cand_b && imin(eff, eff_other) >= 2;
        const bool inexact = fin && at_cap && (unsigned)r.max_overflow > ov_limit;
        constexpr unsigned SAT = (1u << 28) - 1;
        auto argmin32 = [&](const PassOutB &r, bool fin, bool &sat) __attribute__((always_inline)) -> int {
            const unsigned tot = umin32((unsigned)(r.total >> 32) ? SAT : (unsigned)r.total, SAT);
            const unsigned key = fin ? ((tot << 4) | (unsigned)l16) : 0xFFFFFFFFu;
            const unsigned best = row16_reduce(key, [](unsigned a, unsigned b) { return a < b ? a : b; });
            sat = __any((best >> 4) >= SAT);
            return (int)(best & 15u);
        };
        auto argmin64 = [&](uint64_t total, bool fin) __attribute__((always_inline)) -> int {
            uint64_t key = fin ? ((total << 4) | (uint64_t)l16) : ~0ull;
#define VGA_MIN64_STAGE(CTRL)                                                          \
            {                                                                          \
                const unsigned olo = (unsigned)dpp<CTRL>((int)(uint32_t)key);          \
                const unsigned ohi = (unsigned)dpp<CTRL>((int)(uint32_t)(key >> 32));  \
                const uint64_t okey = ((uint64_t)ohi << 32) | olo;                     \
                key = okey < key ? okey : key;                                         \
            }
            VGA_MIN64_STAGE(DPP_QUAD_XOR1)
            VGA_MIN64_STAGE(DPP_QUAD_XOR2)
            VGA_MIN64_STAGE(DPP_ROW_HALF_MIRROR)
            VGA_MIN64_STAGE(DPP_ROW_MIRROR)
#undef VGA_MIN64_STAGE
            return (int)(key & 15u);
        };
        auto commit = [&](const PassOutB &r, int final_sp, int winner) __attribute__((always_inline)) {
            const bool won = l16 == winner;
            const unsigned pay = row16_reduce(won ? r.hist_pair : 0u,
                                              [](unsigned a, unsigned b) { return a | b; });
            if (won) {
// ... 205 lines not shown
        int unused[14];
        if (tiles > 0) {
            load_frame(0, wn, unused);
            prepare_self(0, wn);
            own_lds_done();
        }
        for (int tile = 0; tile < tiles; tile++) {
            const bool more = tile + 1 < tiles;
            if (more) load_frame(tile + 1, wn, unused);
            encode_tile(tile);
            own_lds_done();
            flush(tile);
            if (more) prepare_self(tile + 1, wn);
            own_lds_done();
        }
    } else {
    __syncthreads();
    for (int tile = 0; tile < tiles; tile++) {
        encode_tile(tile);
        __syncthreads();
    }
    }
    if (seg_state && !repair && live && l16 == 0) {
        int16_t *st = seg_state + ((int64_t)by * nch + ch) * 2;
        st[0] = (int16_t)pair_lo(hpk);
        st[1] = (int16_t)pair_hi(hpk);
    }
    if (lane == 0) {
        atomicAdd(&g_vga_gc_stats[3], (unsigned long long)frames_wg);
        atomicAdd(&g_vga_gc_stats[4], (unsigned long long)s_ncold[wave]);
        if (wave == 0) atomicAdd(&g_vga_gc_stats[6], 1ull);
    }
#ifdef VGA_DEBUG_TIMESTAMPS
    if (!repair && tid == 0 && gridDim.y != 1) g_vga_enc_ts[2 * ((blockIdx.y * gridDim.x + blockIdx.x) & 32767) + 1] = wall_clock64();
#endif
}


template <bool REPAIR, int CPW, bool RAGGED>
__global__ __launch_bounds__(ENC_THREADS) __attribute__((amdgpu_waves_per_eu(3, 3))) void gc_encode_kernel(
    const int16_t *__restrict__ pcm, int64_t pcm_pitch, int nch, int total_samples, const Pieces seg,
    const int16_t *__restrict__ coefs, const int16_t *__restrict__ hist1,
    const int16_t *__restrict__ hist2, uint8_t *__restrict__ adpcm, int64_t adpcm_pitch, int16_t *__restrict__ seg_state,
    const int *__restrict__ first_open, const Ragged rg)
{
    gc_encode_piece<REPAIR, CPW, RAGGED>(blockIdx.x, blockIdx.y, pcm, pcm_pitch, nch, total_samples, seg, coefs, hist1, hist2, adpcm,
                                         adpcm_pitch, seg_state, first_open, rg);
}

__device__ __forceinline__ void store_frame_bytes(uint8_t *dst, uint32_t d0, uint32_t d1, int nbytes)
{
    const uint64_t bits = ((uint64_t)d1 << 32) | d0;
    for (int b = 0; b < nbytes; b++) dst[b] = (uint8_t)(bits >> (8 * b));
}

template <int LPC>
__device__ __forceinline__ void seam_run(const int16_t *__restrict__ src, uint8_t *__restrict__ dst, int c0, int c1, bool coef_ok,
                                         int pr, int ch, int k, int64_t f0, int total_samples, int piece_frames, int max_frames, int force_open,
                                         int &h0, int &h1, int g2, int g1, bool &open, int &frames_run)
{
    static_assert(LPC == 8 || LPC == 16, "a lane per predictor, or per (predictor, candidate)");
    const bool cand_b = LPC == 16 && (threadIdx.x & 1) != 0;
    const int full_frames = total_samples / 14;
    const int64_t f_end = imin((int)imin((int)(f0 + piece_frames), (int)(f0 + max_frames)), full_frames);
    const int64_t f_last = full_frames > 0 ? full_frames - 1 : 0;
    auto fetch = [&](int64_t f, uint32_t (&w)[7], uint2 &old) {
        const int64_t fc = f < f_last ? f : f_last;
        const uint32_t *p32 = reinterpret_cast<const uint32_t *>(src + fc * 14);
#pragma unroll
        for (int i = 0; i < 7; i++) w[i] = p32[i];
        old = *reinterpret_cast<const uint2 *>(dst + fc * 8);
    };
    uint32_t w[7], wn[7];
    uint2 old, oldn;
    fetch(f0, w, old);
    for (int64_t f = f0; ; f++) {
        const bool in_range = f < f_end;
        if (!__any(open && in_range)) break;
        const bool act = open && in_range;
        frames_run += act ? 1 : 0;
        fetch(f + 1, wn, oldn);
        int x[16], mp[14];
        x[0] = h0;
        x[1] = h1;
        const uint32_t hpk = pack16(h0, h1);
#pragma unroll
        for (int i = 0; i < 7; i++) {
            x[2 + 2 * i] = (int)(int16_t)(w[i] & 0xFFFF);
            x[3 + 2 * i] = (int)w[i] >> 16;
        }
#pragma unroll
        for (int i = 0; i < 14; i++) mp[i] = x[2 + i] * 2048 + 1024;
        {
            const int ps = (int)(old.x & 0xFFu);
            const int scale = (1 << (ps & 0xF)) * 2048;
            const int pred = (ps >> 4) & 7;
            const int k1 = __shfl(c0, LPC == 16 ? 2 * pred : pred, LPC), k2 = __shfl(c1, LPC == 16 ? 2 * pred : pred, LPC);
            const uint64_t bits = ((uint64_t)old.y << 32) | old.x;
#pragma unroll
            for (int s2 = 0; s2 < 14; s2++) {
                const int byte = (int)((bits >> (8 * (1 + (s2 >> 1)))) & 0xFFu);
                const int nib = (s2 & 1) ? (byte & 0xF) : (byte >> 4);
                const int v = clamp16i((k1 * g1 + k2 * g2 + scale * ((nib ^ 8) - 8) + 1024) >> 11);
                g2 = g1;
                g1 = v;
            }
        }
        int s1;
        {
            int dmax = 0, dmin = 0;
            prescan_range(x, c0, c1, 0, 14, dmax, dmin);
            s1 = first_scale_power_from_range(dmax, dmin);
            if (s1 == -100) s1 = first_scale_power_from_md(prescan_sequential(x, c0, c1));
        }
        const int sp_a = imin(s1, 12), sp_b = imin(s1 + 1, 12);
        PassOut r;
        int final_sp;
        bool fin = true;
        if (LPC == 8) {
        const PassOut rb = pass_fast_core(w, hpk, mp, c0, c1, sp_b);
        const PassOut ra = pass_fast_core(w, hpk, mp, c0, c1, sp_a);
        const bool cap_a = sp_a >= 12, cap_b = sp_b >= 12;
        const bool rare = !coef_ok || (unsigned)ra.max_overflow > (cap_a ? 2u : 248u) || (unsigned)rb.max_overflow > (cap_b ? 2u : 248u);
        const int eff_a = cap_a ? 0 : ra.max_overflow, eff_b = cap_b ? 0 : rb.max_overflow;
        const bool fin_a = eff_a < 2;
        const bool resume = !fin_a && eff_b >= 2;
#pragma unroll
        for (int i = 0; i < 14; i++) r.q[i] = fin_a ? ra.q[i] : rb.q[i];
        r.total = fin_a ? ra.total : rb.total;
        r.hist_pair = fin_a ? ra.hist_pair : rb.hist_pair;
        final_sp = fin_a ? sp_a : sp_b;
        if (__any(rare || resume)) {
            if (rare || resume) {
                const PassOut rc = resume_passes(x, c0, c1, rare ? s1 - 1 : s1 + 1, final_sp);
#pragma unroll
                for (int i = 0; i < 14; i++) r.q[i] = rc.q[i];
                r.total = rc.total;
                r.hist_pair = rc.hist_pair;
            }
        }
        } else {
            final_sp = cand_b ? sp_b : sp_a;
            r = pass_fast_core(w, hpk, mp, c0, c1, final_sp);
            const bool cap = final_sp >= 12;
            const bool rare_mine = !coef_ok || (unsigned)r.max_overflow > (cap ? 2u : 248u);
            const int eff = cap ? 0 : r.max_overflow;
            const int eff_other = dpp<DPP_QUAD_XOR1>(eff);
            const int rare_other = dpp<DPP_QUAD_XOR1>(rare_mine ? 1 : 0);
            const bool rare = rare_mine || rare_other != 0;
            const int eff_a = cand_b ? eff_other : eff, eff_b = cand_b ? eff : eff_other;
            const bool fin_a = eff_a < 2;
            const bool resume = !fin_a && eff_b >= 2;
            fin = cand_b ? !fin_a : fin_a;
            if (__any(rare || resume)) {
                if (rare || resume) {
                    fin = !cand_b;
                    if (!cand_b) r = resume_passes(x, c0, c1, rare ? s1 - 1 : s1 + 1, final_sp);
                }
            }
        }
        const int lidx = LPC == 16 ? (int)(threadIdx.x & 15) : pr;
        uint64_t key = (act && fin) ? ((r.total << 4) | (uint64_t)lidx) : ~0ull;
#define VGA_MIN64_STAGE(CTRL)                                                          \
        {                                                                              \
            const unsigned olo = (unsigned)dpp<CTRL>((int)(uint32_t)key);              \
            const unsigned ohi = (unsigned)dpp<CTRL>((int)(uint32_t)(key >> 32));      \
            const uint64_t okey = ((uint64_t)ohi << 32) | olo;                         \
            key = okey < key ? okey : key;                                             \
        }
        VGA_MIN64_STAGE(DPP_QUAD_XOR1)
        VGA_MIN64_STAGE(DPP_QUAD_XOR2)
        VGA_MIN64_STAGE(DPP_ROW_HALF_MIRROR)
        if (LPC == 16) VGA_MIN64_STAGE(DPP_ROW_MIRROR)
#undef VGA_MIN64_STAGE
        const bool won = act && fin && lidx == (int)(key & 15u);
        unsigned pay = won ? r.hist_pair : 0u;
        pay |= (unsigned)dpp<DPP_QUAD_XOR1>((int)pay);
        pay |= (unsigned)dpp<DPP_QUAD_XOR2>((int)pay);
        pay |= (unsigned)dpp<DPP_ROW_HALF_MIRROR>((int)pay);
        if (LPC == 16) pay |= (unsigned)dpp<DPP_ROW_MIRROR>((int)pay);
        if (won) {
            uint32_t d0, d1;
            pack_frame(r.q, pr, final_sp, d0, d1);
            *reinterpret_cast<uint2 *>(dst + f * 8) = make_uint2(d0, d1);
        }
        if (act) {
            h0 = (int)(int16_t)(pay & 0xFFFF);
            h1 = (int)pay >> 16;
            if (h0 == g2 && h1 == g1 && !seam_forced_open(force_open, ch, k)) open = false;
        }
#pragma unroll
        for (int i = 0; i < 7; i++) w[i] = wn[i];
        old = oldn;
    }
}

template <int LPC>
__device__ __forceinline__ void encode_tail_frame(const int16_t *__restrict__ src, uint8_t *__restrict__ dst, int c0, int c1,
                                                  bool coef_ok, int pr, int total_samples, int h0, int h1, bool act)
{
    const int full_frames = total_samples / 14, tail = total_samples - full_frames * 14;
    int x[16], mp[14];
    x[0] = h0;
    x[1] = h1;
    const uint32_t hpk = pack16(h0, h1);
#pragma unroll
    for (int i = 0; i < 14; i++) x[2 + i] = i < tail ? (int)src[(int64_t)full_frames * 14 + i] : 0;
#pragma unroll
    for (int i = 0; i < 14; i++) mp[i] = x[2 + i] * 2048 + 1024;
    int s1;
    {
        int dmax = 0, dmin = 0;
        prescan_range(x, c0, c1, 0, 14, dmax, dmin);
        s1 = first_scale_power_from_range(dmax, dmin);
        if (s1 == -100) s1 = first_scale_power_from_md(prescan_sequential(x, c0, c1));
    }
    const int sp_a = imin(s1, 12), sp_b = imin(s1 + 1, 12);
    uint32_t w[7];
    pack_row(x, w);
    const PassOut rb = pass_fast_core(w, hpk, mp, c0, c1, sp_b);
    const PassOut ra = pass_fast_core(w, hpk, mp, c0, c1, sp_a);
    const bool cap_a = sp_a >= 12, cap_b = sp_b >= 12;
    const bool rare = !coef_ok || (unsigned)ra.max_overflow > (cap_a ? 2u : 248u) || (unsigned)rb.max_overflow > (cap_b ? 2u : 248u);
    const int eff_a = cap_a ? 0 : ra.max_overflow, eff_b = cap_b ? 0 : rb.max_overflow;
    const bool fin_a = eff_a < 2;
    const bool resume = !fin_a && eff_b >= 2;
    PassOut r;
#pragma unroll
    for (int i = 0; i < 14; i++) r.q[i] = fin_a ? ra.q[i] : rb.q[i];
    r.total = fin_a ? ra.total : rb.total;
    int final_sp = fin_a ? sp_a : sp_b;
    if (rare || resume) {
        const PassOut rc = resume_passes(x, c0, c1, rare ? s1 - 1 : s1 + 1, final_sp);
#pragma unroll
        for (int i = 0; i < 14; i++) r.q[i] = rc.q[i];
        r.total = rc.total;
    }
    const bool in_it = act && (LPC == 8 || (threadIdx.x & 1) == 0);
    uint64_t key = in_it ? ((r.total << 3) | (uint64_t)pr) : ~0ull;
#define VGA_MIN64_STAGE(CTRL)                                                          \
    {                                                                                  \
        const unsigned olo = (unsigned)dpp<CTRL>((int)(uint32_t)key);                  \
        const unsigned ohi = (unsigned)dpp<CTRL>((int)(uint32_t)(key >> 32));          \
        const uint64_t okey = ((uint64_t)ohi << 32) | olo;                             \
        key = okey < key ? okey : key;                                                 \
    }
    VGA_MIN64_STAGE(DPP_QUAD_XOR1)
    VGA_MIN64_STAGE(DPP_QUAD_XOR2)
    VGA_MIN64_STAGE(DPP_ROW_HALF_MIRROR)
    if (LPC == 16) VGA_MIN64_STAGE(DPP_ROW_MIRROR)
#undef VGA_MIN64_STAGE
    if (in_it && pr == (int)(key & 7u)) {
        uint32_t d0, d1;
        pack_frame(r.q, pr, final_sp, d0, d1);
        const int nibbles = tail + 2;
        store_frame_bytes(dst + (int64_t)full_frames * 8, d0, d1, nibbles / 2 + (nibbles & 1));
    }
}

template <int LPC>
__device__ __forceinline__ void seam_piece(
    const int slot_raw, const int k, const int lane,
    const int16_t *__restrict__ pcm, int64_t pcm_pitch, int nch, int total_samples, const Pieces seg,
    const int16_t *__restrict__ coefs, uint8_t *adpcm, int64_t adpcm_pitch,
    const int16_t *seg_state, int *first_open, int *seam_flag, int *seam_end, int force_open, const Ragged &rg)
{
    const int pr = LPC == 16 ? (lane >> 1) & 7 : lane & 7;
    const bool lead = (lane & (LPC - 1)) == 0;
    const int64_t f0 = seg.first(k);
    const int slot = slot_raw < nch ? slot_raw : nch - 1;
    const int ch = rg.order ? rg.order[slot] : slot;
    if (rg.order) total_samples = rg.length[ch];
    const bool valid = slot_raw < nch && f0 * 14 < total_samples;
    const int16_t *src = pcm + (rg.order ? rg.pcm_off[ch] : (int64_t)ch * pcm_pitch);
    uint8_t *dst = adpcm + (rg.order ? rg.adpcm_off[ch] : (int64_t)ch * adpcm_pitch);
    const int16_t *cf = coefs + ch * 16;
    const int c0 = cf[2 * pr], c1 = cf[2 * pr + 1];
    const bool coef_ok = (c0 < 0 ? -c0 : c0) + (c1 < 0 ? -c1 : c1) <= 32767;
    int h0 = valid ? seg_state[((int64_t)(k - 1) * nch + ch) * 2] : 0;
    int h1 = valid ? seg_state[((int64_t)(k - 1) * nch + ch) * 2 + 1] : 0;
    const int g2 = valid ? src[f0 * 14 - 2] : 0, g1 = valid ? src[f0 * 14 - 1] : 0;
    bool open = valid;
    int frames_run = 0;
    seam_run<LPC>(src, dst, c0, c1, coef_ok, pr, ch, k, f0, total_samples, seg.frames(k), seg.frames(k), force_open, h0, h1, g2, g1, open, frames_run);
    if (valid && lead) {
        atomicAdd(&g_vga_gc_stats[open ? 1 : 0], 1ull);
        atomicAdd(&g_vga_gc_stats[2], (unsigned long long)frames_run);
        seam_flag[(int64_t)(k - 1) * nch + ch] = open ? 1 : 0;
        if (open) {
            seam_end[(int64_t)(k - 1) * nch + ch] = (int)(((unsigned)h1 << 16) | ((unsigned)h0 & 0xFFFFu));
            atomicMin(&first_open[ch], k);
        }
    }
}

constexpr int HAND_ARRIVED = 1;
constexpr int HAND_V = 2;
constexpr int HAND_EVER = 4;
struct Handover {
    int *word = nullptr;
    int *token = nullptr, *v = nullptr;
};

__device__ __forceinline__ void self_served_seams(
    const int g, const int seam_a, const int seam_b, const int lane, const int groups, const int segments,
    const int16_t *__restrict__ pcm, int64_t pcm_pitch, int nch, int total_samples, const Pieces seg,
    const int16_t *__restrict__ coefs, uint8_t *adpcm, int64_t adpcm_pitch,
    const int16_t *seg_state, int *first_open, int *seam_flag, int *seam_end, int force_open, const Handover hand)
{
    const int pr = lane & 7;
    const bool lead = pr == 0;
    const int slot_raw = g * PLAN8_SLOTS + (lane >> 3);
    const bool live = slot_raw < nch;
    const int ch = live ? slot_raw : nch - 1;
    const int16_t *src = pcm + (int64_t)ch * pcm_pitch;
    uint8_t *dst = adpcm + (int64_t)ch * adpcm_pitch;
    const int16_t *cf = coefs + ch * 16;
    const int c0 = cf[2 * pr], c1 = cf[2 * pr + 1];
    const bool coef_ok = (c0 < 0 ? -c0 : c0) + (c1 < 0 ? -c1 : c1) <= 32767;
    auto second_on = [&](int piece) {
        __threadfence();
        int old = 0;
        if (lane == 0) old = atomicAdd(&hand.word[(int64_t)(piece - 1) * groups + g], 1);
        const bool second = __builtin_amdgcn_readfirstlane(old) == 1;
        if (second) __threadfence();
        return second;
    };
    int own = 0;
    int p = 0;
    int state = 0, v0 = 0, v1 = 0;
    for (;;) {
        const bool cont = p != 0;
        int k;
        if (cont) k = p;
        else if (own == 0) { own = 1; k = seam_a; }
        else if (own == 1) { own = 2; k = seam_b; }
        else break;
        p = 0;
        if (k == 0) continue;
        const int64_t f0 = seg.first(k);
        const bool valid = live && f0 * 14 < total_samples;
        const int64_t idx = (int64_t)(k - 1) * nch + ch;
        const int t0 = valid ? seg_state[idx * 2] : 0, t1 = valid ? seg_state[idx * 2 + 1] : 0;
        int h0 = cont ? v0 : t0, h1 = cont ? v1 : t1;
        const int g2 = cont ? t0 : (valid ? src[f0 * 14 - 2] : 0), g1 = cont ? t1 : (valid ? src[f0 * 14 - 1] : 0);
        bool open = cont ? valid && (state & HAND_V) != 0 : valid;
        const bool ran = open;
        int frames_run = 0;
        if (__any(open))
            seam_run<8>(src, dst, c0, c1, coef_ok, pr, ch, k, f0, total_samples, seg.frames(k), seg.frames(k), force_open, h0, h1, g2, g1, open, frames_run);
        if (!cont) {
            if (valid && lead) {
                atomicAdd(&g_vga_gc_stats[open ? 1 : 0], 1ull);
                atomicAdd(&g_vga_gc_stats[2], (unsigned long long)frames_run);
                seam_flag[idx] = open ? 1 : 0;
                if (open) {
                    seam_end[idx] = (int)(((unsigned)h1 << 16) | ((unsigned)h0 & 0xFFFFu));
                    atomicMin(&first_open[ch], k);
                }
            }
            if (!hand.word) continue;
            if (k == 1) {
                state = HAND_ARRIVED | (open ? HAND_V | HAND_EVER : 0);
                v0 = h0;
                v1 = h1;
            } else {
                if (second_on(k)) {
                    state = hand.token[idx];
                    const int v = hand.v[idx];
                    v0 = (int)(int16_t)(v & 0xFFFF);
                    v1 = v >> 16;
                    p = k;
                }
                continue;
            }
        } else {
            if (valid && lead && frames_run) atomicAdd(&g_vga_gc_stats[2], (unsigned long long)frames_run);
            const bool flagged = valid && seam_flag[idx] != 0;
            if (ran && open) {
                v0 = h0;
                v1 = h1;
            } else if (flagged) {
                const int ended = seam_end[idx];
                state |= HAND_V | HAND_EVER;
                v0 = (int)(int16_t)(ended & 0xFFFF);
                v1 = ended >> 16;
            } else
                state &= ~HAND_V;
        }
        const bool last = k + 1 >= segments || seg.first(k + 1) * 14 >= total_samples;
        const int64_t nidx = (int64_t)(last ? segments - 1 : k) * nch + ch;
        if (live && lead) {
            hand.v[nidx] = (int)(((unsigned)v1 << 16) | ((unsigned)v0 & 0xFFFFu));
            hand.token[nidx] = state;
            if (last && (state & HAND_EVER) != 0) atomicAdd(&g_vga_gc_stats[8], 1ull);
        }
        if (last) continue;
        if (second_on(k + 1)) p = k + 1;
    }
}

template <int LPC>
__global__ __launch_bounds__(64) void gc_encode_seam_kernel(
    const int16_t *__restrict__ pcm, int64_t pcm_pitch, int nch, int total_samples, const Pieces seg,
    const int16_t *__restrict__ coefs, uint8_t *__restrict__ adpcm, int64_t adpcm_pitch,
    const int16_t *__restrict__ seg_state, int *__restrict__ first_open, int *__restrict__ seam_flag,
    int *__restrict__ seam_end, int force_open, const Ragged rg)
{
    seam_piece<LPC>(blockIdx.x * (64 / LPC) + (threadIdx.x / LPC), blockIdx.y + 1, threadIdx.x, pcm, pcm_pitch, nch, total_samples, seg, coefs, adpcm,
               adpcm_pitch, seg_state, first_open, seam_flag, seam_end, force_open, rg);
}

template <int CPW, bool RAGGED>
__global__ __launch_bounds__(ENC_THREADS) __attribute__((amdgpu_waves_per_eu(VGA_GC_PERSISTENT_WAVES_PER_EU))) void gc_encode_persistent_kernel(
    const int16_t *__restrict__ pcm, int64_t pcm_pitch, int nch, int total_samples, const Pieces seg,
    const int16_t *__restrict__ coefs, const int16_t *__restrict__ hist1,
    const int16_t *__restrict__ hist2, uint8_t *adpcm, int64_t adpcm_pitch, int16_t *seg_state,
    const Ragged rg, int groups, int segments, int *__restrict__ queue, int *__restrict__ seam_count, int *first_open,
    int *seam_flag, int *seam_end, int force_open)
{
    static_assert(CPW == 8, "the seams inside the persistent kernel use the (channel, predictor) layout");
    constexpr int CS = Lay<CPW>::CS;
    __shared__ int s_item;
    __shared__ int s_seam[2];
    const int items = RAGGED && rg.items ? rg.n_items : groups * segments;
#ifdef VGA_DEBUG_TIMESTAMPS
    if (threadIdx.x == 0) g_vga_enc_ts[2 * (blockIdx.x & 32767)] = wall_clock64();
#endif
    for (;;) {
        if (threadIdx.x == 0) s_item = atomicAdd(queue, 1);
        __syncthreads();
        const int item = s_item;
        __syncthreads();
        if (item >= items) {
#ifdef VGA_DEBUG_TIMESTAMPS
            if (threadIdx.x == 0) g_vga_enc_ts[2 * (blockIdx.x & 32767) + 1] = wall_clock64();
#endif
            return;
        }
        int g = item % groups, y = item / groups;
        if (RAGGED && rg.items) {
            const uint32_t v = rg.items[item];
            g = (int)(v & 0xFFFFFu);
            y = (int)(v >> 20);
        }
        gc_encode_piece<false, CPW, RAGGED>(g, y, pcm, pcm_pitch, nch, total_samples, seg, coefs, hist1, hist2, adpcm, adpcm_pitch,
                                            seg_state, (const int *)nullptr, rg);
        if (segments <= 1) continue;
        __threadfence();
        __syncthreads();
        if (threadIdx.x == 0) {
            const int total_wg = RAGGED ? rg.length[rg.order[g * CS]] : total_samples;
            auto exists = [&](int piece) { return piece < segments && seg.first(piece) * 14 < total_wg; };
            int at_start = 0, at_end = 0;
            if (exists(y)) {
                if (y >= 1 && atomicAdd(&seam_count[(int64_t)(y - 1) * groups + g], 1) == 1) at_start = y;
                if (exists(y + 1) && atomicAdd(&seam_count[(int64_t)y * groups + g], 1) == 1) at_end = y + 1;
            }
            s_seam[0] = at_start;
            s_seam[1] = at_end;
        }
        __syncthreads();
        const int seam_a = s_seam[0], seam_b = s_seam[1];
        if ((seam_a | seam_b) != 0) {
            __threadfence();
            const int wave = threadIdx.x >> 6, lane = threadIdx.x & 63;
            if (wave < SW) {
                const int slot = g * CS + wave * CPW + (lane >> 3);
                if (seam_a)
                    seam_piece<8>(slot, seam_a, lane, pcm, pcm_pitch, nch, total_samples, seg, coefs, adpcm, adpcm_pitch, seg_state,
                               first_open, seam_flag, seam_end, force_open, rg);
                if (seam_b)
                    seam_piece<8>(slot, seam_b, lane, pcm, pcm_pitch, nch, total_samples, seg, coefs, adpcm, adpcm_pitch, seg_state,
                               first_open, seam_flag, seam_end, force_open, rg);
            }
        }
    }
}

__global__ __launch_bounds__(64) void gc_slow_groups_kernel(const int16_t *__restrict__ coefs, int nch, int groups8, int *__restrict__ order)
{
    const int lane = threadIdx.x;
    auto flagged = [&](int g) {
        bool slow = false;
        if (g < groups8)
            for (int s = 0; s < PLAN8_SLOTS; s++) {
                const int ch = g * PLAN8_SLOTS + s;
                if (ch < nch) slow = plan8_slow_channel(coefs + (int64_t)ch * 16) || slow;
            }
        return slow;
    };
    int total = 0;
    for (int base = 0; base < groups8; base += 64) total += __popcll(__ballot(flagged(base + lane)));
    int s = 0, r = total;
    const unsigned long long lower = (1ull << lane) - 1;
    for (int base = 0; base < groups8; base += 64) {
        const int g = base + lane;
        const bool f = flagged(g);
        const unsigned long long m = __ballot(f), rest = __ballot(!f && g < groups8);
        if (g < groups8) order[f ? s + __popcll(m & lower) : r + __popcll(rest & lower)] = g;
        s += __popcll(m);
        r += __popcll(rest);
    }
    if (lane == 0) order[groups8] = total;
}
extern "C" int vga_testing_gc_slow_order_host(const int16_t *coefs, int nch, int *order)
{
    if (!coefs || !order || nch <= 0) return -1;
    const int groups8 = (nch + PLAN8_SLOTS - 1) / PLAN8_SLOTS;
    std::vector<unsigned char> flagged((size_t)groups8, 0);
    for (int ch = 0; ch < nch; ch++)
        if (plan8_slow_channel(coefs + (int64_t)ch * 16)) flagged[(size_t)(ch / PLAN8_SLOTS)] = 1;
    return plan8_slow_order(flagged.data(), groups8, order);
}
extern "C" int vga_testing_gc_slow_order_device(const void *d_coefs, int nch, int *order)
{
    if (!d_coefs || !order || nch <= 0) return -1;
    const int groups8 = (nch + PLAN8_SLOTS - 1) / PLAN8_SLOTS;
    int *d_order = nullptr;
    if (hipMalloc(&d_order, (size_t)(groups8 + 1) * sizeof(int)) != hipSuccess) return -1;
    hipLaunchKernelGGL(gc_slow_groups_kernel, dim3(1), dim3(64), 0, (hipStream_t)0, static_cast<const int16_t *>(d_coefs), nch, groups8, d_order);
    std::vector<int> host((size_t)groups8 + 1);
    const bool ok = hipGetLastError() == hipSuccess &&
                    hipMemcpy(host.data(), d_order, host.size() * sizeof(int), hipMemcpyDeviceToHost) == hipSuccess;
    (void)hipFree(d_order);
    if (!ok) return -1;
    for (int g = 0; g < groups8; g++) order[g] = host[(size_t)g];
    return host[(size_t)groups8];
}

template <bool RAGGED>
__global__ __launch_bounds__(64) __attribute__((amdgpu_waves_per_eu(3, 3))) void gc_encode_self_served_kernel(
    const int16_t *__restrict__ pcm, int64_t pcm_pitch, int nch, int total_samples, const Pieces seg,
    const int16_t *__restrict__ coefs, const int16_t *__restrict__ hist1,
    const int16_t *__restrict__ hist2, uint8_t *adpcm, int64_t adpcm_pitch, int16_t *seg_state,
    const Ragged rg, int groups, int items, int segments, int *__restrict__ queue, int *__restrict__ seam_count, int *first_open,
    int *seam_flag, int *seam_end, int force_open, const Handover hand, const int *__restrict__ slow_order)
{
    constexpr int CS = PLAN8_SLOTS;
    static_assert(Lay<8, true>::CS == CS && Lay<8, true>::THREADS == 64, "one wave, eight channel slots");
    const int lane = threadIdx.x;
    const uint32_t *host_items = RAGGED ? rg.items : nullptr;
    const int *order = RAGGED ? nullptr : slow_order;
    const int slow = order ? order[groups] : 0;
#ifdef VGA_DEBUG_TIMESTAMPS
    if (lane == 0) g_vga_enc_ts[2 * (blockIdx.x & 32767)] = wall_clock64();
#endif
    for (;;) {
        int item = 0;
        if (lane == 0) item = atomicAdd(queue, 1);
        item = __builtin_amdgcn_readfirstlane(item);
        if (item >= items) {
#ifdef VGA_DEBUG_TIMESTAMPS
            if (lane == 0) g_vga_enc_ts[2 * (blockIdx.x & 32767) + 1] = wall_clock64();
#endif
            return;
        }
        int g, y;
        if (!plan8_item(item, groups, nch, host_items, order, slow, segments, g, y)) continue;
        gc_encode_piece<false, 8, RAGGED, true>(g, y, pcm, pcm_pitch, nch, total_samples, seg, coefs, hist1, hist2, adpcm, adpcm_pitch,
                                                seg_state, (const int *)nullptr, rg);
        if (segments <= 1) continue;
        __threadfence();
        int at_start = 0, at_end = 0;
        if (lane == 0) {
            const int total_wg = RAGGED ? rg.length[rg.order[g * CS]] : total_samples;
            auto exists = [&](int piece) { return piece < segments && seg.first(piece) * 14 < total_wg; };
            if (exists(y)) {
                if (y >= 1 && atomicAdd(&seam_count[(int64_t)(y - 1) * groups + g], 1) == 1) at_start = y;
                if (exists(y + 1) && atomicAdd(&seam_count[(int64_t)y * groups + g], 1) == 1) at_end = y + 1;
            }
        }
        const int seam_a = __builtin_amdgcn_readfirstlane(at_start), seam_b = __builtin_amdgcn_readfirstlane(at_end);
        if ((seam_a | seam_b) != 0) {
            __threadfence();
            if constexpr (RAGGED) {
                const int slot = g * CS + (lane >> 3);
                if (seam_a)
                    seam_piece<8>(slot, seam_a, lane, pcm, pcm_pitch, nch, total_samples, seg, coefs, adpcm, adpcm_pitch, seg_state,
                               first_open, seam_flag, seam_end, force_open, rg);
                if (seam_b)
                    seam_piece<8>(slot, seam_b, lane, pcm, pcm_pitch, nch, total_samples, seg, coefs, adpcm, adpcm_pitch, seg_state,
                               first_open, seam_flag, seam_end, force_open, rg);
            } else
                self_served_seams(g, seam_a, seam_b, lane, groups, segments, pcm, pcm_pitch, nch, total_samples, seg, coefs, adpcm,
                                  adpcm_pitch, seg_state, first_open, seam_flag, seam_end, force_open, hand);
        }
    }
}

template <int LPC>
__global__ __launch_bounds__(64) void gc_encode_chain_kernel(
    const int16_t *__restrict__ pcm, int64_t pcm_pitch, int nch, int total_samples, const Pieces seg, int segments,
    const int16_t *__restrict__ coefs, uint8_t *__restrict__ adpcm, int64_t adpcm_pitch,
    int16_t *__restrict__ seg_state, int *__restrict__ first_open, const int *__restrict__ seam_flag,
    const int *__restrict__ seam_end, int force_open, const Ragged rg, const int *__restrict__ hand_token,
    const int *__restrict__ hand_v)
{
    const int lane = threadIdx.x;
    const int pr = LPC == 16 ? (lane >> 1) & 7 : lane & 7;
    const bool lead = (lane & (LPC - 1)) == 0;
    const int slot_raw = blockIdx.x * (64 / LPC) + lane / LPC;
    const bool live = slot_raw < nch;
    const int slot = live ? slot_raw : nch - 1;
    const int ch = rg.order ? rg.order[slot] : slot;
    if (rg.order) total_samples = rg.length[ch];
    const int64_t rec_idx = (int64_t)(segments - 1) * nch + ch;
    const int record = hand_token && live ? hand_token[rec_idx] : 0;
    const bool resolved = record != 0;
    const int mine_raw = live ? first_open[ch] : SEAM_NONE;
    const int mine = resolved ? SEAM_NONE : mine_raw;
    int kmin = mine, kmin_raw = mine_raw;
#pragma unroll
    for (int o = LPC; o < 64; o <<= 1) {
        kmin = imin(kmin, __shfl_xor(kmin, o));
        kmin_raw = imin(kmin_raw, __shfl_xor(kmin_raw, o));
    }
    if (kmin_raw >= segments) return;
    const bool tail_left = resolved && (record & HAND_V) != 0 && total_samples % 14 != 0;
    if (live && lead && (mine < segments || tail_left)) atomicAdd(&g_vga_gc_stats[5], 1ull);
    int frames_run = 0;
    const int16_t *src = pcm + (rg.order ? rg.pcm_off[ch] : (int64_t)ch * pcm_pitch);
    uint8_t *dst = adpcm + (rg.order ? rg.adpcm_off[ch] : (int64_t)ch * adpcm_pitch);
    const int16_t *cf = coefs + ch * 16;
    const int c0 = cf[2 * pr], c1 = cf[2 * pr + 1];
    const bool coef_ok = (c0 < 0 ? -c0 : c0) + (c1 < 0 ? -c1 : c1) <= 32767;
    bool have = false;
    int v0 = 0, v1 = 0;
    int last_k = 0;
    for (int k = kmin; k < segments; k++) {
        const int64_t f0 = seg.first(k);
        const bool exists = f0 * 14 < total_samples;
        if (!__any(exists)) break;
        last_k = k;
        const bool is_last = seg.first(k + 1) * 14 >= total_samples || k == segments - 1;
        const int64_t idx = (int64_t)(k - 1) * nch + ch;
        const bool flagged = live && !resolved && exists && seam_flag[idx] != 0;
        const int ended = seam_end[idx];
        const bool ran = live && have && exists;
        bool open = ran;
        int h0 = v0, h1 = v1;
        if (__any(ran)) {
            const int g2 = seg_state[idx * 2], g1 = seg_state[idx * 2 + 1];
            if (ran && lead && is_last) {
                seg_state[idx * 2] = (int16_t)v0;
                seg_state[idx * 2 + 1] = (int16_t)v1;
            }
            seam_run<LPC>(src, dst, c0, c1, coef_ok, pr, ch, k, f0, total_samples, seg.frames(k), seg.frames(k), force_open, h0, h1, g2, g1, open, frames_run);
        }
        if (!exists) {
        } else if (ran && open) {
            v0 = h0;
            v1 = h1;
        } else if (flagged) {
            have = true;
            v0 = (int)(int16_t)(ended & 0xFFFF);
            v1 = ended >> 16;
        } else
            have = false;
    }
    if (tail_left) {
        const int v = hand_v[rec_idx];
        have = true;
        v0 = (int)(int16_t)(v & 0xFFFF);
        v1 = v >> 16;
    }
    if (__any(live && have && total_samples % 14 != 0))
        encode_tail_frame<LPC>(src, dst, c0, c1, coef_ok, pr, total_samples, v0, v1, live && have && total_samples % 14 != 0);
    (void)last_k;
    if (live && lead && frames_run) atomicAdd(&g_vga_gc_stats[2], (unsigned long long)frames_run);
    if (live && lead) first_open[ch] = SEAM_NONE;
}

constexpr int MIN_PIECE_FRAMES = 3584;

constexpr int RAGGED_OVERSUBSCRIPTION = 4;
constexpr int PERSISTENT_MIN_GROUPS_FACTOR = 32;
constexpr int PERSISTENT_SCHEDULE_GROUPS_FACTOR = 8;
constexpr int PERSISTENT_ITEMS_PER_WORKGROUP = 4;
constexpr int PERSISTENT_BIG_ROUNDS = 3;
constexpr int PERSISTENT_SMALL_ROUNDS = 2;
constexpr int PERSISTENT_SMALL_FRAMES = 4096;
constexpr int SELF_SERVED_BIG_ROUNDS = 4;
constexpr int SELF_SERVED_SMALL_ROUNDS = 1;
constexpr int MAX_PIECES = 1024;

static int persistent_wgs_per_cu()
{
#ifdef VGA_TUNING
    if (const char *e = std::getenv("VGA_HIP_GC_WGS_PER_CU")) return imin(imax(std::atoi(e), 1), 5);
#endif
    return 4;
}

int plan_encode_pieces(int groups, int frames, int64_t group_frames, bool ragged, bool *persistent_out, Pieces *seg_out, int layout)
{
    return plan_encode_pieces_on(device_cu_count(), groups, frames, group_frames, ragged, persistent_out, seg_out, layout);
}

int plan_encode_pieces_on(int cus, int groups, int frames, int64_t group_frames, bool ragged, bool *persistent_out, Pieces *seg_out, int layout)
{
    const bool self = layout == 1;
    const int pmode = encoder_persistent_mode();
    const bool persistent = self || (layout != 4 && (pmode == 2 || (pmode == 0 && (ragged || groups * PERSISTENT_MIN_GROUPS_FACTOR >= cus * 4))));
    int segments = cus * 4 / (groups > 0 ? groups : 1);
    if (persistent && (pmode == 2 || ragged)) segments = (cus * 4 * PERSISTENT_ITEMS_PER_WORKGROUP + groups - 1) / groups;
    if (ragged) {
        const int64_t want = (int64_t)cus * 4 * (persistent ? PERSISTENT_ITEMS_PER_WORKGROUP : RAGGED_OVERSUBSCRIPTION);
        int64_t piece = (group_frames + want - 1) / want;
        if (piece < MIN_PIECE_FRAMES) piece = MIN_PIECE_FRAMES;
        segments = (int)((frames + piece - 1) / piece);
    }
    if (segments > frames / MIN_PIECE_FRAMES) segments = frames / MIN_PIECE_FRAMES;
    if (segments < 1) segments = 1;
    if (segments > MAX_PIECES) segments = MAX_PIECES;
    if (encoder_segments_override() > 0) segments = imin(imin(imax(frames / 64, 1), encoder_segments_override()), MAX_PIECES);
    Pieces seg;
    seg.big = (frames + segments - 1) / segments;
    seg.nb = segments;
    seg.small = seg.big;
    if (persistent && encoder_segments_override() <= 0 && frames >= 4 * MIN_PIECE_FRAMES &&
        (ragged || groups * PERSISTENT_SCHEDULE_GROUPS_FACTOR >= cus * 4)) {
        int big_rounds = ragged ? PERSISTENT_BIG_ROUNDS + 1 : PERSISTENT_BIG_ROUNDS, small_rounds = PERSISTENT_SMALL_ROUNDS, small = PERSISTENT_SMALL_FRAMES;
        if (self && !ragged) { big_rounds = SELF_SERVED_BIG_ROUNDS; small_rounds = SELF_SERVED_SMALL_ROUNDS; }
#ifdef VGA_TUNING
        if (const char *e = std::getenv("VGA_HIP_GC_SCHEDULE")) std::sscanf(e, "%d,%d,%d", &big_rounds, &small_rounds, &small);
#endif
        small = imax(small, MIN_PIECE_FRAMES);
        big_rounds = imax(big_rounds, 1);
        const int wgs = cus * (self ? PLAN8_WGS_PER_CU : persistent_wgs_per_cu());
        const int queue_groups = self ? 2 * groups : groups;
        const int64_t per_wg = group_frames * (self ? 2 : 1) / wgs + 1;
        int ns = (small_rounds * wgs + queue_groups / 2) / queue_groups;
        if ((int64_t)ns * small > frames / 2) ns = frames / (2 * small);
        int big = (int)imax((int)((per_wg - (int64_t)small_rounds * small) / big_rounds), small);
        int nb = (int)((frames - (int64_t)ns * small + big - 1) / big);
        if (nb < 1) nb = 1;
        if (!ragged) big = (int)((frames - (int64_t)ns * small + nb - 1) / nb);
        if (big < small) big = small;
        seg.big = big;
        seg.nb = nb;
        seg.small = small;
        segments = nb + ns;
        while (segments > 1 && seg.first(segments - 1) >= frames) segments--;
        if (segments > MAX_PIECES) {
            segments = MAX_PIECES;
            seg.big = seg.small = (frames + segments - 1) / segments;
            seg.nb = segments;
            while (segments > 1 && seg.first(segments - 1) >= frames) segments--;
        }
    }
    if (seg.first(segments) < frames) {
        seg.big = seg.small = (frames + segments - 1) / segments;
        seg.nb = segments;
    }
    *persistent_out = persistent;
    *seg_out = seg;
    return segments;
}

#ifndef VGA_GC_SELF_SERVED_DEFAULT
#define VGA_GC_SELF_SERVED_DEFAULT 1
#endif
static bool self_served_shape(int layout_hook, int groups16, int cus, bool ragged)
{
    if (layout_hook == 1) return true;
    if (layout_hook != 0 || encoder_persistent_mode() != 0) return false;
    return VGA_GC_SELF_SERVED_DEFAULT != 0 && (ragged || groups16 * PERSISTENT_SCHEDULE_GROUPS_FACTOR >= cus * 4);
}
int encoder_plan_layout(int groups16, bool ragged) { return self_served_shape(encoder_layout(), groups16, device_cu_count(), ragged) ? 1 : 8; }

template <int CPW, bool RAGGED>
static int launch_encode_layout(const int16_t *d_pcm, int64_t pcm_pitch, int nch, int sample_count, const int16_t *d_coefs,
                                const int16_t *d_hist1, const int16_t *d_hist2, uint8_t *d_adpcm, int64_t adpcm_pitch,
                                hipStream_t stream, void *d_scratch, size_t scratch_bytes, const Ragged &rg)
{
    constexpr int CS = Lay<CPW>::CS;
    if (RAGGED) sample_count = rg.max_length;
    if (nch <= 0 || sample_count <= 0) return VGA_OK;
    const int groups = (nch + CS - 1) / CS;
    const int cus = device_cu_count();
    const int frames = (sample_count + 13) / 14;
    bool persistent = false;
    Pieces seg;
    int segments;
    const bool want_self = CPW == 8 && self_served_shape(encoder_layout(), groups, cus, RAGGED);
    if (RAGGED && rg.items) {
        persistent = rg.persistent != 0;
        seg = rg.seg;
        segments = rg.segments;
    } else {
        segments = plan_encode_pieces(groups, frames, RAGGED ? rg.total_frames / CS : (int64_t)groups * frames, RAGGED, &persistent, &seg,
                                      want_self ? 1 : CPW);
    }
    const bool self = want_self && persistent;
    const Plan8 p8 = self ? plan_groups_of_eight(cus, nch, segments, RAGGED && rg.items ? rg.n_items : -1) : Plan8{};
    const int seam_groups = self ? p8.groups : groups;
    AsyncBuf scratch;
    int16_t *seg_state = nullptr;
    int *first_open = nullptr, *seam_flag = nullptr, *seam_end = nullptr, *queue = nullptr, *seam_count = nullptr;
    const bool handover = self && !RAGGED && segments > 1 && !gc_seam_handover_off();
    Handover hand;
    int *slow_order = nullptr;
    if (segments > 1 || persistent) {
        const size_t state_bytes = segments > 1 ? (size_t)round_up((int64_t)segments * nch * 2 * (int64_t)sizeof(int16_t), 16) : 0;
        const size_t open_bytes = (size_t)round_up((int64_t)nch * (int64_t)sizeof(int), 16);
        const size_t count_bytes = persistent && segments > 1 ? (size_t)round_up((int64_t)(segments - 1) * seam_groups * (int64_t)sizeof(int), 16) : 0;
        const size_t order_bytes = handover ? (size_t)round_up((int64_t)(seam_groups + 1) * (int64_t)sizeof(int), 16) : 0;
        const size_t need = 3 * state_bytes + open_bytes + 16 + count_bytes + (handover ? count_bytes + 2 * state_bytes + order_bytes : 0);
        unsigned char *base = static_cast<unsigned char *>(d_scratch);
        if (!base || scratch_bytes < need) {
            VGA_HIP_TRY(scratch.alloc(need, stream));
            base = scratch.as<unsigned char>();
        }
        seam_flag = reinterpret_cast<int *>(base + state_bytes);
        seam_end = reinterpret_cast<int *>(base + 2 * state_bytes);
        first_open = reinterpret_cast<int *>(base + 3 * state_bytes);
        queue = reinterpret_cast<int *>(base + 3 * state_bytes + open_bytes);
        if (segments > 1) {
            seg_state = reinterpret_cast<int16_t *>(base);
            VGA_HIP_TRY(fill_no_open_seams(first_open, nch, stream));
        } else
            seg_state = nullptr;
        seam_count = queue + 4;
        if (persistent) VGA_HIP_TRY(hipMemsetAsync(queue, 0, 16 + count_bytes * (handover ? 2 : 1), stream));
        if (handover) {
            unsigned char *words = base + 3 * state_bytes + open_bytes + 16 + count_bytes;
            hand.word = reinterpret_cast<int *>(words);
            hand.token = reinterpret_cast<int *>(words + count_bytes);
            hand.v = reinterpret_cast<int *>(words + count_bytes + state_bytes);
            slow_order = reinterpret_cast<int *>(words + count_bytes + 2 * state_bytes);
            VGA_HIP_TRY(hipMemsetAsync(hand.token + (size_t)(segments - 1) * nch, 0, (size_t)nch * sizeof(int), stream));
        }
    }
    if (self) {
        if constexpr (CPW == 8) {
            if (slow_order) hipLaunchKernelGGL(gc_slow_groups_kernel, dim3(1), dim3(64), 0, stream, d_coefs, nch, p8.groups, slow_order);
            hipLaunchKernelGGL((gc_encode_self_served_kernel<RAGGED>), dim3(p8.wgs), dim3(Lay<8, true>::THREADS), 0, stream, d_pcm, pcm_pitch,
                               nch, sample_count, seg, d_coefs, d_hist1, d_hist2, d_adpcm, adpcm_pitch, seg_state, rg, p8.groups, p8.items,
                               segments, queue, seam_count, first_open, seam_flag, seam_end, force_open_seams(), hand, (const int *)slow_order);
        }
    } else if (persistent) {
        const int items = RAGGED && rg.items ? rg.n_items : groups * segments;
        const int wgs = imin(items, cus * persistent_wgs_per_cu());
        if constexpr (CPW == 8)
            hipLaunchKernelGGL((gc_encode_persistent_kernel<CPW, RAGGED>), dim3(wgs), dim3(ENC_THREADS), 0, stream, d_pcm, pcm_pitch, nch,
                               sample_count, seg, d_coefs, d_hist1, d_hist2, d_adpcm, adpcm_pitch, seg_state, rg, groups, segments, queue,
                               seam_count, first_open, seam_flag, seam_end, force_open_seams());
    } else
        hipLaunchKernelGGL((gc_encode_kernel<false, CPW, RAGGED>), dim3(groups, segments), dim3(ENC_THREADS), 0, stream, d_pcm, pcm_pitch, nch,
                           sample_count, seg, d_coefs, d_hist1, d_hist2, d_adpcm, adpcm_pitch, seg_state,
                           (const int *)nullptr, rg);
    VGA_HIP_TRY(hipGetLastError());
    if (segments > 1) {
        if (!persistent) {
#ifdef VGA_GC_SEAM16_ALWAYS
            const bool wide = CPW == 4;
#else
            const bool wide = CPW == 4 && nch > 64;
#endif
            if (wide)
                hipLaunchKernelGGL(gc_encode_seam_kernel<16>, dim3((nch + 3) / 4, segments - 1), dim3(64), 0, stream, d_pcm, pcm_pitch, nch,
                                   sample_count, seg, d_coefs, d_adpcm, adpcm_pitch, seg_state, first_open, seam_flag, seam_end,
                                   force_open_seams(), rg);
            else
                hipLaunchKernelGGL(gc_encode_seam_kernel<8>, dim3((nch + 7) / 8, segments - 1), dim3(64), 0, stream, d_pcm, pcm_pitch, nch,
                                   sample_count, seg, d_coefs, d_adpcm, adpcm_pitch, seg_state, first_open, seam_flag, seam_end,
                                   force_open_seams(), rg);
            VGA_HIP_TRY(hipGetLastError());
        }
#ifdef VGA_GC_SEAM16_ALWAYS
        if (CPW == 4)
#else
        if (CPW == 4 && nch > 64)
#endif
            hipLaunchKernelGGL(gc_encode_chain_kernel<16>, dim3((nch + 3) / 4), dim3(64), 0, stream, d_pcm, pcm_pitch, nch, sample_count,
                               seg, segments, d_coefs, d_adpcm, adpcm_pitch, seg_state, first_open, seam_flag, seam_end,
                               force_open_seams(), rg, (const int *)hand.token, (const int *)hand.v);
        else
            hipLaunchKernelGGL(gc_encode_chain_kernel<8>, dim3((nch + 7) / 8), dim3(64), 0, stream, d_pcm, pcm_pitch, nch, sample_count,
                               seg, segments, d_coefs, d_adpcm, adpcm_pitch, seg_state, first_open, seam_flag, seam_end,
                               force_open_seams(), rg, (const int *)hand.token, (const int *)hand.v);
        VGA_HIP_TRY(hipGetLastError());
        hipLaunchKernelGGL((gc_encode_kernel<true, CPW, RAGGED>), dim3(groups, 1), dim3(ENC_THREADS), 0, stream, d_pcm, pcm_pitch, nch, sample_count,
                           seg, d_coefs, d_hist1, d_hist2, d_adpcm, adpcm_pitch, seg_state, (const int *)first_open, rg);
        VGA_HIP_TRY(hipGetLastError());
    }
    return VGA_OK;
}

size_t encode_scratch_bytes(int nch) { return (size_t)(nch > 0 ? nch : 0) * (1024 * 20 + 4 + 1024 + 1) + 8192 + 32; }

int launch_encode(const int16_t *d_pcm, int64_t pcm_pitch, int nch, int sample_count, const int16_t *d_coefs,
                  const int16_t *d_hist1, const int16_t *d_hist2, uint8_t *d_adpcm, int64_t adpcm_pitch,
                  hipStream_t stream, void *d_scratch, size_t scratch_bytes, const Ragged *rg)
{
    if (rg)
        return launch_encode_layout<8, true>(d_pcm, 0, nch, 0, d_coefs, d_hist1, d_hist2, d_adpcm, 0, stream, d_scratch,
                                             scratch_bytes, *rg);
    int layout = encoder_layout();
    if (layout == 0)
        layout = encoder_persistent_mode() != 2 && ((nch + 15) / 16) * PERSISTENT_MIN_GROUPS_FACTOR < device_cu_count() * 4 ? 4 : 8;
    if (layout == 4)
        return launch_encode_layout<4, false>(d_pcm, pcm_pitch, nch, sample_count, d_coefs, d_hist1, d_hist2, d_adpcm, adpcm_pitch, stream,
                                              d_scratch, scratch_bytes, Ragged{});
    return launch_encode_layout<8, false>(d_pcm, pcm_pitch, nch, sample_count, d_coefs, d_hist1, d_hist2, d_adpcm, adpcm_pitch, stream,
                                          d_scratch, scratch_bytes, Ragged{});
}

}
}
```

### vgaudio_amd/csrc/gcadpcm_kernels.hpp

```cpp
#pragma once
#include <hip/hip_runtime.h>
#include <cstdint>

namespace vga {
namespace gc {

struct Pieces {
    int big = 0, nb = 0, small = 0;
    __host__ __device__ int64_t first(int k) const { return (int64_t)(k < nb ? k : nb) * big + (int64_t)(k > nb ? k - nb : 0) * small; }
    __host__ __device__ int frames(int k) const { return k < nb ? big : small; }
};
int encoder_plan_layout(int groups, bool ragged);
int plan_encode_pieces(int groups, int frames, int64_t group_frames, bool ragged, bool *persistent, Pieces *seg, int layout = 8);
int plan_encode_pieces_on(int cus, int groups, int frames, int64_t group_frames, bool ragged, bool *persistent, Pieces *seg, int layout = 8);

struct Ragged {
    const uint32_t *items = nullptr;
    int n_items = 0, segments = 0, persistent = 0;
    Pieces seg;
    const int *order = nullptr;
    const int *length = nullptr;
    const int64_t *pcm_off = nullptr;
    const int64_t *adpcm_off = nullptr;
    const int64_t *rec_off = nullptr;
    int solo_channels = 0;
    int solo_usable = 0;
    int max_length = 0;
    int64_t total_frames = 0;
};

constexpr int COEF_RECORD_BLOCK = 256;
__host__ __device__ inline int64_t coef_record_pitch(int64_t frames)
{
    return (frames > 0 ? frames + COEF_RECORD_BLOCK - 1 : COEF_RECORD_BLOCK) / COEF_RECORD_BLOCK * COEF_RECORD_BLOCK;
}

int ragged_solo_count(const int *lengths_longest_first, int nch, int64_t total_frames, int cus, int *usable_out = nullptr);
int launch_coefs(const int16_t *d_pcm, int64_t pcm_pitch, int nch, int length, int16_t *d_coefs,
                 void *d_workspace, hipStream_t stream, const Ragged *rg = nullptr);
int launch_encode(const int16_t *d_pcm, int64_t pcm_pitch, int nch, int sample_count, const int16_t *d_coefs,
                  const int16_t *d_hist1, const int16_t *d_hist2, uint8_t *d_adpcm, int64_t adpcm_pitch,
                  hipStream_t stream, void *d_scratch = nullptr, size_t scratch_bytes = 0, const Ragged *rg = nullptr);
size_t encode_scratch_bytes(int nch);
int launch_decode(const uint8_t *d_adpcm, int64_t adpcm_pitch, const int16_t *d_coefs, int nch, int sample_count,
                  const int16_t *d_hist1, const int16_t *d_hist2, int16_t *d_pcm, int64_t pcm_pitch, int *d_status,
                  hipStream_t stream, const Ragged *rg = nullptr);
int launch_align_gather(const int16_t *d_pcm, int64_t pcm_pitch, int nch, int loop_start, int loop_end,
                        int samples_to_keep, int samples_to_encode, int16_t *d_new_pcm, int64_t new_pitch,
                        int16_t *d_hist1, int16_t *d_hist2, hipStream_t stream);
int launch_channel_meta(const uint8_t *d_adpcm, int64_t adpcm_pitch, const int16_t *d_pcm, int64_t pcm_pitch, int nch,
                        int loop_start, int samples_per_entry, int entries, int16_t *d_seek, int64_t seek_pitch,
                        int16_t *d_loop_context, hipStream_t stream);
int launch_dsp_image(const uint8_t *d_adpcm, int64_t adpcm_pitch, int adpcm_len, const int16_t *d_coefs,
                     const int16_t *d_gain, const int16_t *d_start_context, const int16_t *d_loop_context, int nch,
                     int sample_count, int nibble_count, int sample_rate, int looping, int start_addr, int end_addr,
                     int cur_addr, int bytes_per_interleave, int frames_per_interleave, int audio_data_size,
                     int mono_bytes, uint8_t *d_file, size_t file_size, hipStream_t stream);
int launch_synth(int16_t *d_pcm, int64_t pitch, int nch, int length, int first_channel, const uint32_t *d_params,
                 hipStream_t stream);

}
}
```

### vgaudio_amd/csrc/host_batch.hpp

```cpp
#pragma once
#include <algorithm>
#include <atomic>
#include <cstdlib>
#include <memory>
#include <mutex>
#include "common.hpp"
#include "host_pipeline.hpp"
#include "../../include/vgaudio_hip_testing.h"

namespace vga {

struct PipeOverride {
    int feeders = 0, drainers = 0, chunk_units = 0, slot_bytes = 0, tail_units = 0;
    int buckets_order = 0;
    int transfer = 0;
    int piece_bytes = 0;
    int compute_lanes = 0;
};
struct FailStep {
    int kind = 0, nth = 0, seen = 0;
};
constexpr const char *kRefusedStep = "step refused by vga_testing_fail_step_this_thread";
int launch_transfer(const pipe::Job::TransferPiece *pieces, int n, hipStream_t stream);
int device_cu_count();

struct ThreadSettings {
    int force_open_seams = 0;
    int encoder_layout = 0;
    int coefs_variant = 0;
    int encoder_segments = 0;
    int encoder_persistent = 0;
    int hca_frames_per_group = 0;
    int gc_seam_handover_off = 0;
    PipeOverride pipe;
    FailStep fail;
};
ThreadSettings &thread_settings();
inline PipeOverride &pipe_override() { return thread_settings().pipe; }
inline bool refuse_step(int kind)
{
    FailStep &f = thread_settings().fail;
    return f.kind == kind && ++f.seen == f.nth;
}
struct PipeReport { pipe::Stats stats; double t_alloc = 0, t_entry = 0; };
PipeReport &pipe_report();
int hardware_queues_requested();
inline int planned_compute_lanes(int own_choice)
{
    const int hook = pipe_override().compute_lanes;
    return std::max(1, std::min(hook > 0 ? hook : own_choice, pipe::kMaxComputeLanes));
}

std::vector<int> batch_devices();

struct ProgressCallback { void (*fn)(void *user, int64_t done, int64_t total) = nullptr; void *user = nullptr; };
ProgressCallback progress_callback();
struct ProgressSink {
    ProgressCallback cb;
    int64_t total = 0, done = 0;
    std::mutex m;
    void add(int64_t units)
    {
        std::lock_guard<std::mutex> g(m);
        done += units;
        cb.fn(cb.user, done, total);
    }
};
ProgressSink *&current_progress_sink();

template <class Body>
inline int for_each_device_share(int units, int min_units, Body &&body)
{
    ProgressSink sink;
    sink.cb = progress_callback();
    sink.total = units;
    struct SinkScope {
        ProgressSink *before;
        explicit SinkScope(ProgressSink *s) : before(current_progress_sink()) { current_progress_sink() = s; }
        ~SinkScope() { current_progress_sink() = before; }
    } scope(sink.cb.fn && units > 0 ? &sink : nullptr);
    const std::vector<int> devices = batch_devices();
    if (devices.empty() || units <= 0) return body(0, units);
    const std::vector<pipe::Share> shares = pipe::plan_shares(devices, units, min_units);
    const ThreadSettings settings = thread_settings();
    if (shares.size() == 1) {
        int before = 0;
        VGA_HIP_TRY(hipGetDevice(&before));
        VGA_HIP_TRY(hipSetDevice(shares[0].device));
        const int rc = body(0, units);
        (void)hipSetDevice(before);
        return rc;
    }
    ProgressSink *const shared_sink = current_progress_sink();
    const pipe::Result r = pipe::run_on_devices(shares, [&](const pipe::Share &sh, std::string &why) -> int {
        if (sh.index != 0) {
            thread_settings() = settings;
            current_progress_sink() = shared_sink;
        }
        const int rc = body(sh.first, sh.count);
        if (rc) why = vga_last_error();
        return rc;
    });
    if (r.code) set_error("%s", r.why.c_str());
    return r.code;
}

template <class Body>
inline decltype(pipe::Job::compute) chunk_compute(Body body)
{
    return [body](int first, int count, hipStream_t s, std::string &why) -> int {
        if (refuse_step(VGA_TESTING_STEP_CHUNK_COMPUTE)) {
            why = kRefusedStep;
            return VGA_ERR_DEVICE;
        }
        const int rc = body(first, count, s);
        if (rc) why = vga_last_error();
        return rc;
    };
}

inline size_t job_in_total(const pipe::Job &job)
{
    if (!job.in_rows) return 0;
    const size_t rows = (size_t)job.units * job.in_rows_per_unit;
    if (!job.in_row_sizes) return rows * job.in_row_bytes;
    size_t t = 0;
    for (size_t r = 0; r < rows; r++) t += job.in_row_sizes[r];
    return t;
}
inline size_t job_out_total(const pipe::Job &job)
{
    if (!job.out_rows) return 0;
    const size_t rows = (size_t)job.units * job.out_rows_per_unit;
    if (!job.out_row_sizes) return rows * job.out_row_bytes;
    size_t t = 0;
    for (size_t r = 0; r < rows; r++) t += job.out_row_sizes[r];
    return t;
}

inline int planned_chunk_units(const pipe::Job &job, int default_chunk_units)
{
    const PipeOverride &o = pipe_override();
    const size_t in_total = job_in_total(job);
    const size_t out_total = job_out_total(job);
    int chunk = o.chunk_units > 0 ? o.chunk_units : default_chunk_units;
    if (o.chunk_units <= 0 && out_total > in_total) chunk = std::max(1, chunk / 4);
    if (o.chunk_units <= 0 && in_total + out_total < ((size_t)256 << 20)) chunk = job.units;
    return std::max(1, std::min(chunk, job.units));
}

inline int run_batch_pipeline(pipe::Job &job, int default_chunk_units)
{
    const PipeOverride &o = pipe_override();
    VGA_HIP_TRY(hipStreamSynchronize(nullptr));
    int device = 0;
    VGA_HIP_TRY(hipGetDevice(&device));
    job.device = device;
    const size_t in_total = job_in_total(job);
    const size_t out_total = job_out_total(job);
    const size_t in_row_typical = job.in_row_sizes ? in_total / std::max<size_t>(1, (size_t)job.units * job.in_rows_per_unit) : job.in_row_bytes;
    const size_t out_row_typical = job.out_row_sizes ? out_total / std::max<size_t>(1, (size_t)job.units * job.out_rows_per_unit) : job.out_row_bytes;
    job.feeders = o.feeders > 0 ? o.feeders : (o.feeders < 0 ? -o.feeders : 1);
    job.drainers = o.drainers > 0 ? o.drainers : (out_total >= ((size_t)256 << 20) ? 2 : 1);
    job.direct = o.slot_bytes < 0 || (o.slot_bytes == 0 && in_row_typical >= ((size_t)256 << 10));
    job.direct_out = o.slot_bytes < 0 || (o.slot_bytes == 0 && out_row_typical >= ((size_t)256 << 10) && out_total > in_total);
    job.shared_streams = o.feeders >= 0;
    job.slot_bytes = o.slot_bytes > 0 ? (size_t)o.slot_bytes : (o.slot_bytes < -1 ? (size_t)(-o.slot_bytes) : (size_t)32 << 20);
    job.chunk_units = planned_chunk_units(job, default_chunk_units);
    job.tail_units = in_total + out_total >= ((size_t)256 << 20) ? std::max(1, job.chunk_units * 3 / 8) : 0;
    if (o.tail_units > 0) job.tail_units = o.tail_units;
    job.head_units = 0;
    std::shared_ptr<std::atomic<int>> transfers_seen;
    if (o.transfer == 2 || (o.transfer == 0 && in_total + out_total >= ((size_t)256 << 20) && in_row_typical < ((size_t)4 << 20))) {
        const FailStep fail = thread_settings().fail;
        auto seen = std::make_shared<std::atomic<int>>(fail.seen);
        job.transfer = [fail, seen](const pipe::Job::TransferPiece *pieces, int n, hipStream_t s, std::string &why) -> int {
            if (fail.kind == VGA_TESTING_STEP_TRANSFER && seen->fetch_add(1) + 1 == fail.nth) {
                why = kRefusedStep;
                return VGA_ERR_DEVICE;
            }
            const int rc = launch_transfer(pieces, n, s);
            if (rc) why = vga_last_error();
            return rc;
        };
        job.gather_in = job.direct && job.feeders == 1;
        job.scatter_out = true;
        if (o.drainers == 0 && !job.direct_out && out_total >= ((size_t)1 << 30)) job.drainers = 4;
        job.total_cus = device_cu_count();
        job.transfer_cus = 16;
        if (o.piece_bytes > 0) job.piece_bytes = (size_t)o.piece_bytes;
        transfers_seen = seen;
    }
    if (ProgressSink *sink = current_progress_sink())
        job.chunk_done = [sink](int, int count) { sink->add(count); };
    const pipe::Result r = pipe::run(job);
    if (transfers_seen && thread_settings().fail.kind == VGA_TESTING_STEP_TRANSFER) thread_settings().fail.seen = transfers_seen->load();
    pipe_report().stats = r.stats;
    if (r.code) {
        set_error("%s", r.why.c_str());
        return r.code;
    }
    return VGA_OK;
}

inline int run_status_job(pipe::Job &job, int chunk_units, DevBuf &d_status, const char *message)
{
    if (int rc = run_batch_pipeline(job, chunk_units)) return rc;
    int status = 0;
    VGA_HIP_TRY(hipMemcpy(&status, d_status.p, sizeof(int), hipMemcpyDeviceToHost));
    if (status != 0) {
        set_error("%s", message);
        return VGA_ERR_ARGUMENT;
    }
    return VGA_OK;
}

struct BucketPlan {
    std::vector<int> order;
    std::vector<int> chunk_begin;
    std::vector<int> chunk_length;
    std::vector<int> chunk_group;
    int chunk_of(int first) const { return (int)(std::upper_bound(chunk_begin.begin(), chunk_begin.end(), first) - chunk_begin.begin()) - 1; }
};
inline BucketPlan plan_buckets(const std::vector<int> &group, const std::vector<int> &length, int max_units, int64_t max_volume,
                               bool longest_first)
{
    BucketPlan b;
    const int n = (int)group.size();
    b.order.resize(n);
    for (int i = 0; i < n; i++) b.order[i] = i;
    std::stable_sort(b.order.begin(), b.order.end(), [&](int x, int y) {
        return group[x] != group[y] ? group[x] < group[y] : length[x] < length[y];
    });
    const PipeOverride &o = pipe_override();
    if (o.chunk_units > 0) max_units = o.chunk_units;
    int first = 0;
    for (int i = 0; i <= n; i++) {
        bool cut = i == n;
        if (!cut && i > first) {
            const int u = b.order[i], f = b.order[first];
            cut = group[u] != group[f] || (int64_t)length[u] > (int64_t)length[f] + length[f] / 4 + 1024 || i - first >= max_units ||
                  (int64_t)(i - first + 1) * std::max(length[u], 1) > max_volume;
        }
        if (cut && i > first) {
            b.chunk_begin.push_back(first);
            b.chunk_length.push_back(length[b.order[i - 1]]);
            b.chunk_group.push_back(group[b.order[first]]);
            first = i;
        }
    }
    b.chunk_begin.push_back(n);
    if (o.buckets_order ? o.buckets_order == 1 : !longest_first) return b;
    BucketPlan r;
    const int chunks = (int)b.chunk_length.size();
    r.order.reserve(n);
    for (int k = chunks - 1; k >= 0; k--) {
        r.chunk_begin.push_back((int)r.order.size());
        r.chunk_length.push_back(b.chunk_length[k]);
        r.chunk_group.push_back(b.chunk_group[k]);
        r.order.insert(r.order.end(), b.order.begin() + b.chunk_begin[k], b.order.begin() + b.chunk_begin[k + 1]);
    }
    r.chunk_begin.push_back(n);
    return r;
}

struct RaggedRows {
    std::vector<size_t> size, off;
    size_t max_pitch = 16;
};
inline void bind_in(pipe::Job &job, const void *const *rows, const RaggedRows &r, char *d)
{
    job.in_rows = rows;
    job.in_row_sizes = r.size.data();
    job.d_in_offsets = r.off.data();
    job.in_row_bytes = r.max_pitch;
    job.d_in_pitch = r.max_pitch;
    job.d_in = d;
}
inline void bind_out(pipe::Job &job, void *const *rows, const RaggedRows &r, const char *d)
{
    job.out_rows = rows;
    job.out_row_sizes = r.size.data();
    job.d_out_offsets = r.off.data();
    job.out_row_bytes = r.max_pitch;
    job.d_out_pitch = r.max_pitch;
    job.d_out = d;
}

inline void bind_in(pipe::Job &job, const void *const *rows, size_t row_bytes, char *d, size_t pitch)
{
    job.in_rows = rows;
    job.in_row_bytes = row_bytes;
    job.d_in = d;
    job.d_in_pitch = pitch;
}
inline void bind_out(pipe::Job &job, void *const *rows, size_t row_bytes, const char *d, size_t pitch)
{
    job.out_rows = rows;
    job.out_row_bytes = row_bytes;
    job.d_out = d;
    job.d_out_pitch = pitch;
}

struct BucketLayout {
    struct Side {
        int rows_per_unit = 1;
        std::vector<int64_t> base, pitch;
        RaggedRows rows;
    };
    std::vector<int> chunk_begin;
    Side in, out;
    std::vector<const void *> in_host;
    std::vector<void *> out_host;

    int alloc(DevBuf &d_in, DevBuf &d_out) const
    {
        VGA_HIP_TRY(d_in.alloc((size_t)in.base.back() + 64));
        VGA_HIP_TRY(hipMemset(d_in.p, 0, (size_t)in.base.back() + 64));
        VGA_HIP_TRY(d_out.alloc((size_t)out.base.back() + 64));
        return VGA_OK;
    }
    void bind(pipe::Job &job, const DevBuf &d_in, const DevBuf &d_out) const
    {
        job.chunk_begin = chunk_begin;
        job.in_rows_per_unit = in.rows_per_unit;
        job.out_rows_per_unit = out.rows_per_unit;
        bind_in(job, in_host.data(), in.rows, d_in.as<char>());
        bind_out(job, out_host.data(), out.rows, d_out.as<char>());
    }
};
struct RowPitch { int64_t in, out; };
struct InRow { const void *p; size_t bytes; };
struct OutRow { void *p; size_t bytes; };

template <class Ptr, class RowOf>
inline void lay_out_rows(const BucketPlan &plan, BucketLayout::Side &s, std::vector<Ptr> &host, RowOf row_of)
// ... 41 lines not shown
```

### vgaudio_amd/csrc/runtime.hip

```cpp
#include "common.hpp"
#include "host_batch.hpp"
#include "../../include/vgaudio_hip_testing.h"

namespace vga {

static thread_local char g_err[512] = "";
static thread_local bool g_err_pending = false;

void set_error(const char *fmt, ...)
{
    va_list ap;
    va_start(ap, fmt);
    vsnprintf(g_err, sizeof g_err, fmt, ap);
    va_end(ap);
    g_err_pending = true;
}

bool take_error_pending()
{
    const bool was = g_err_pending;
    g_err_pending = false;
    return was;
}

int require_device()
{
    g_err_pending = false;
    int n = 0;
    hipError_t e = hipGetDeviceCount(&n);
    if (e != hipSuccess || n <= 0) {
        set_error("no HIP device available (%s); libvgaudio_hip has no CPU fallback",
                  e == hipSuccess ? "device count 0" : hipGetErrorString(e));
        return VGA_ERR_DEVICE;
    }
    return VGA_OK;
}

static thread_local ThreadSettings g_settings;
ThreadSettings &thread_settings() { return g_settings; }
int force_open_seams() { return g_settings.force_open_seams; }
int encoder_layout() { return g_settings.encoder_layout; }
int coefs_kernel_variant() { return g_settings.coefs_variant; }
int encoder_segments_override() { return g_settings.encoder_segments; }
int encoder_persistent_mode() { return g_settings.encoder_persistent; }
int hca_frames_per_group_override() { return g_settings.hca_frames_per_group; }
bool gc_seam_handover_off() { return g_settings.gc_seam_handover_off != 0; }
static thread_local int g_adx_encode_path = 0, g_adx_decode_path = 0;
void note_adx_encode_path(int path) { g_adx_encode_path = path; }
void note_adx_decode_path(int path) { g_adx_decode_path = path; }

static int g_queues_seen_by_runtime = 4;
__attribute__((constructor)) static void read_hardware_queues()
{
    if (const char *host = std::getenv("GPU_MAX_HW_QUEUES"))
        g_queues_seen_by_runtime = std::atoi(host);
}
int hardware_queues_requested() { return g_queues_seen_by_runtime; }

static std::mutex g_devices_mutex;
static std::vector<int> g_devices;
std::vector<int> batch_devices()
{
    std::lock_guard<std::mutex> g(g_devices_mutex);
    return g_devices;
}

static thread_local PipeReport g_pipe_report;
PipeReport &pipe_report() { return g_pipe_report; }
static thread_local ProgressCallback g_progress_callback;
ProgressCallback progress_callback() { return g_progress_callback; }
static thread_local ProgressSink *g_progress_sink = nullptr;
ProgressSink *&current_progress_sink() { return g_progress_sink; }

}

using namespace vga;

extern "C" {

const char *vga_last_error(void) { return g_err; }

const char *vga_version(void) { return "vgaudio_hip 0.2 (gfx950)"; }

void vga_release_cached_memory(void)
{
    DevicePool::get().trim();
    pipe::PinnedPool::get().trim();
    pipe::MaskedStreamPool::get().trim();
}

int vga_device_count(void)
{
    int n = 0;
    if (hipGetDeviceCount(&n) != hipSuccess) return 0;
    return n;
}

int vga_set_device(int device)
{
    VGA_HIP_TRY(hipSetDevice(device));
    return VGA_OK;
}

int vga_set_devices(const int *devices, int count)
{
    if (count < 0 || (count > 0 && !devices) || count > 64) { set_error("vga_set_devices: bad device list"); return VGA_ERR_ARGUMENT; }
    int n = 0;
    if (count > 0 && (hipGetDeviceCount(&n) != hipSuccess || n <= 0)) {
        set_error("no HIP device available; libvgaudio_hip has no CPU fallback");
        return VGA_ERR_DEVICE;
    }
    for (int i = 0; i < count; i++)
        if (devices[i] < 0 || devices[i] >= n) { set_error("vga_set_devices: device %d of %d does not exist", devices[i], n); return VGA_ERR_ARGUMENT; }
    std::lock_guard<std::mutex> g(g_devices_mutex);
    g_devices.assign(devices, devices + count);
    return VGA_OK;
}

int vga_get_devices(int *devices, int capacity)
{
    std::lock_guard<std::mutex> g(g_devices_mutex);
    for (int i = 0; i < (int)g_devices.size() && i < capacity && devices; i++) devices[i] = g_devices[i];
    return (int)g_devices.size();
}

int vga_set_progress_callback(vga_progress_fn fn, void *user)
{
    g_progress_callback.fn = fn;
    g_progress_callback.user = fn ? user : nullptr;
    return VGA_OK;
}

int vga_testing_force_open_seams_this_thread(int mode)
{
    const int old = g_settings.force_open_seams;
    g_settings.force_open_seams = mode;
    return old;
}
int vga_testing_gc_encoder_layout_this_thread(int channels_per_wave)
{
    const int old = g_settings.encoder_layout;
    if (channels_per_wave == 0 || channels_per_wave == 1 || channels_per_wave == 4 || channels_per_wave == 8)
        g_settings.encoder_layout = channels_per_wave;
    return old;
}
int vga_testing_gc_coefs_variant_this_thread(int variant)
{
    const int old = g_settings.coefs_variant;
    if (variant >= 0 && variant <= 3) g_settings.coefs_variant = variant;
    return old;
}
int vga_testing_gc_encoder_segments_this_thread(int segments)
{
    const int old = g_settings.encoder_segments;
    g_settings.encoder_segments = segments > 0 ? segments : 0;
    return old;
}
int vga_testing_gc_encoder_persistent_this_thread(int mode)
{
    const int old = g_settings.encoder_persistent;
    g_settings.encoder_persistent = mode >= 0 && mode <= 2 ? mode : 0;
    return old;
}
int vga_testing_gc_seam_handover_this_thread(int on)
{
    const int old = g_settings.gc_seam_handover_off ? 0 : 1;
    g_settings.gc_seam_handover_off = on ? 0 : 1;
    return old;
}
int vga_testing_hca_frames_per_group_this_thread(int frames)
{
    const int old = g_settings.hca_frames_per_group;
    g_settings.hca_frames_per_group = frames > 0 ? frames : 0;
    return old;
}
int vga_testing_adx_last_path_this_thread(int *encode, int *decode)
{
    if (encode) *encode = g_adx_encode_path;
    if (decode) *decode = g_adx_decode_path;
    return 0;
}
void vga_testing_host_pipeline_this_thread(int feeders, int drainers, int chunk_units, int slot_bytes)
{
    PipeOverride &o = g_settings.pipe;
    o.feeders = feeders;
    o.drainers = drainers;
    o.chunk_units = chunk_units;
    o.slot_bytes = slot_bytes;
}
void vga_testing_host_pipeline_tail_this_thread(int tail_units) { g_settings.pipe.tail_units = tail_units > 0 ? tail_units : 0; }
void vga_testing_buckets_order_this_thread(int order) { g_settings.pipe.buckets_order = order == 1 || order == 2 ? order : 0; }
void vga_testing_host_transfer_this_thread(int mode) { g_settings.pipe.transfer = mode == 1 || mode == 2 ? mode : 0; }
void vga_testing_host_transfer_piece_bytes_this_thread(int bytes) { g_settings.pipe.piece_bytes = bytes > 0 ? bytes : 0; }
void vga_testing_fail_step_this_thread(int kind, int nth)
{
    const bool on = kind >= VGA_TESTING_STEP_CHUNK_COMPUTE && kind <= VGA_TESTING_STEP_HCA_STREAM_FRAMES && nth > 0;
    g_settings.fail = FailStep{on ? kind : 0, on ? nth : 0, 0};
}
void vga_testing_host_compute_lanes_this_thread(int lanes) { g_settings.pipe.compute_lanes = lanes > 0 ? lanes : 0; }
int vga_testing_poison_allocations(int byte)
{
    if (byte < -1 || byte > 255) return poison_byte();
    return poison_setting().exchange(byte, std::memory_order_relaxed);
}

int vga_testing_plan_buckets(const int *group, const int *length, int n, int max_units, long long max_volume, int longest_first,
                             int *order_out, int *chunk_begin_out, int *chunk_length_out, int *chunk_group_out, int max_chunks)
{
    if (n < 0 || (n > 0 && (!group || !length))) return -1;
    const BucketPlan plan = plan_buckets(std::vector<int>(group, group + n), std::vector<int>(length, length + n), max_units, max_volume, longest_first != 0);
    const int chunks = (int)plan.chunk_begin.size() - 1;
    if (chunks > max_chunks) return -1;
    for (int i = 0; i < n && order_out; i++) order_out[i] = plan.order[i];
    for (int k = 0; k <= chunks && chunk_begin_out; k++) chunk_begin_out[k] = plan.chunk_begin[k];
    for (int k = 0; k < chunks; k++) {
        if (chunk_length_out) chunk_length_out[k] = plan.chunk_length[k];
        if (chunk_group_out) chunk_group_out[k] = plan.chunk_group[k];
    }
    return chunks;
}
int vga_testing_last_pipeline_stats(double *out, int n)
{
    const PipeReport &r = g_pipe_report;
    const double v[] = {r.stats.total, r.stats.setup, r.stats.feed_copy, r.stats.feed_wait_slot, r.stats.feed_issue, r.stats.feed_max,
                        r.stats.main_wait_upload, r.stats.main_launch, r.stats.main_tail_sync, r.stats.drain_wait_compute,
                        r.stats.drain_wait_copy, r.stats.drain_copy, r.stats.drain_max, (double)r.stats.feeders, (double)r.stats.drainers,
                        (double)r.stats.chunks, (double)r.stats.chunk_units, r.t_alloc, r.t_entry, r.stats.feed_boundary, r.stats.feed_final, r.stats.drain_register};
    const int m = (int)(sizeof v / sizeof v[0]);
    for (int i = 0; i < n && i < m; i++) out[i] = v[i];
    return m;
}

}
```

Baseline: 90930 Msamples/s.

## Add tail-graded piece schedule, coarse slow-group pieces, and fused encoder prologue kernel

```diff
diff --git a/include/vgaudio_hip_testing.h b/include/vgaudio_hip_testing.h
--- a/include/vgaudio_hip_testing.h
+++ b/include/vgaudio_hip_testing.h
@@ -13,13 +13,16 @@
 int vga_testing_gc_encoder_persistent_this_thread(int mode);
 
 int vga_testing_gc_plan_pieces(int cus, int groups, int frames, long long group_frames, int ragged, int *out5);
+int vga_testing_gc_plan_pieces_n(int cus, int groups, int frames, long long group_frames, int ragged, int coarse, int *out10);
 
 int vga_testing_gc_encode_stats(unsigned long long *out8, int reset);
 int vga_testing_gc_encode_stats_n(unsigned long long *out, int n, int reset);
 
 int vga_testing_gc_seam_handover_this_thread(int on);
+int vga_testing_gc_schedule_this_thread(int big_rounds, const int *tail_counts, const int *tail_frames, int min_tail_frames);
 int vga_testing_gc_slow_order_host(const short *coefs, int nch, int *order);
 int vga_testing_gc_slow_order_device(const void *d_coefs, int nch, int *order);
+int vga_testing_gc_prologue_device(const void *d_coefs, int nch, int zero_ints, int *order_flags, int *bad_words);
 
 void vga_testing_host_pipeline_this_thread(int feeders, int drainers, int chunk_units, int slot_bytes);
 
diff --git a/vgaudio_amd/_lib.py b/vgaudio_amd/_lib.py
--- a/vgaudio_amd/_lib.py
+++ b/vgaudio_amd/_lib.py
@@ -159,8 +159,10 @@
     "vga_testing_gc_encoder_segments_this_thread": (ci, [ci]),
     "vga_testing_gc_encoder_persistent_this_thread": (ci, [ci]),
     "vga_testing_gc_seam_handover_this_thread": (ci, [ci]),
+    "vga_testing_gc_schedule_this_thread": (ci, [ci, C.POINTER(ci), C.POINTER(ci), ci]),
     "vga_testing_gc_slow_order_host": (ci, [vp, ci, vp]),
     "vga_testing_gc_slow_order_device": (ci, [vp, ci, vp]),
+    "vga_testing_gc_prologue_device": (ci, [vp, ci, ci, vp, vp]),
     "vga_testing_gc_encode_stats_n": (ci, [C.POINTER(C.c_ulonglong), ci, ci]),
     "vga_testing_last_pipeline_stats": (ci, [vp, ci]),
     "vga_testing_host_pipeline_tail_this_thread": (None, [ci]),
@@ -256,6 +258,7 @@
     "vga_hca_stream_destroy": (None, [vp]),
     "vga_testing_gc_encode_stats": (ci, [C.POINTER(C.c_ulonglong), ci]),
     "vga_testing_gc_plan_pieces": (ci, [ci, ci, ci, C.c_longlong, ci, C.POINTER(ci)]),
+    "vga_testing_gc_plan_pieces_n": (ci, [ci, ci, ci, C.c_longlong, ci, ci, C.POINTER(ci)]),
     "vga_set_devices": (ci, [vp, ci]),
     "vga_set_progress_callback": (ci, [vp, vp]),
     "vga_get_devices": (ci, [vp, ci]),
diff --git a/vgaudio_amd/csrc/capi_gcadpcm.hip b/vgaudio_amd/csrc/capi_gcadpcm.hip
--- a/vgaudio_amd/csrc/capi_gcadpcm.hip
+++ b/vgaudio_amd/csrc/capi_gcadpcm.hip
@@ -17,6 +17,18 @@
     out5[2] = seg.nb;
     out5[3] = seg.small;
     out5[4] = persistent ? 1 : 0;
+    return 0;
+}
+
+int vga_testing_gc_plan_pieces_n(int cus, int groups, int frames, long long group_frames, int ragged, int coarse, int *out10)
+{
+    if (!out10 || cus <= 0 || groups <= 0 || frames <= 0) return -1;
+    bool persistent = false;
+    gc::TailPieces seg;
+    const int segments = gc::plan_encode_tail_pieces_on(cus, groups, frames, group_frames, ragged != 0, &persistent, &seg,
+                                                          encoder_layout() == 1 ? 1 : 8, coarse != 0);
+    const int out[10] = {segments, seg.big, seg.nb, seg.small, seg.n1, seg.s2, seg.n2, seg.s3, persistent ? 1 : 0, 0};
+    for (int i = 0; i < 10; i++) out10[i] = out[i];
     return 0;
 }
 
diff --git a/vgaudio_amd/csrc/common.hpp b/vgaudio_amd/csrc/common.hpp
--- a/vgaudio_amd/csrc/common.hpp
+++ b/vgaudio_amd/csrc/common.hpp
@@ -229,6 +229,7 @@
 int encoder_segments_override();
 int encoder_persistent_mode();
 int hca_frames_per_group_override();
+const int *gc_schedule_override();
 bool gc_seam_handover_off();
 void note_adx_encode_path(int path);
 void note_adx_decode_path(int path);
diff --git a/vgaudio_amd/csrc/gc_encode_kernel.hip b/vgaudio_amd/csrc/gc_encode_kernel.hip
--- a/vgaudio_amd/csrc/gc_encode_kernel.hip
+++ b/vgaudio_amd/csrc/gc_encode_kernel.hip
@@ -182,10 +182,10 @@
     return o;
 }
 
-template <bool REPAIR, int CPW, bool RAGGED, bool SELF = false>
+template <bool REPAIR, int CPW, bool RAGGED, bool SELF = false, class P = Pieces>
 __device__ __forceinline__ void gc_encode_piece(
     const int bx, const int by,
-    const int16_t *__restrict__ pcm, int64_t pcm_pitch, int nch, int total_samples, const Pieces seg,
+    const int16_t *__restrict__ pcm, int64_t pcm_pitch, int nch, int total_samples, const P seg,
     const int16_t *__restrict__ coefs, const int16_t *__restrict__ hist1,
     const int16_t *__restrict__ hist2, uint8_t *__restrict__ adpcm, int64_t adpcm_pitch, int16_t *__restrict__ seg_state,
     const int *__restrict__ first_open, const Ragged &rg)
@@ -997,9 +997,10 @@
     int *token = nullptr, *v = nullptr;
 };
 
+template <class P>
 __device__ __forceinline__ void self_served_seams(
-    const int g, const int seam_a, const int seam_b, const int lane, const int groups, const int segments,
-    const int16_t *__restrict__ pcm, int64_t pcm_pitch, int nch, int total_samples, const Pieces seg,
+    const int g, const int seam_a, const int seam_b, const int lane, const int groups, const int segments, const int rec_row,
+    const int16_t *__restrict__ pcm, int64_t pcm_pitch, int nch, int total_samples, const P seg,
     const int16_t *__restrict__ coefs, uint8_t *adpcm, int64_t adpcm_pitch,
     const int16_t *seg_state, int *first_open, int *seam_flag, int *seam_end, int force_open, const Handover hand)
 {
@@ -1084,7 +1085,7 @@
                 state &= ~HAND_V;
         }
         const bool last = k + 1 >= segments || seg.first(k + 1) * 14 >= total_samples;
-        const int64_t nidx = (int64_t)(last ? segments - 1 : k) * nch + ch;
+        const int64_t nidx = (int64_t)(last ? rec_row : k) * nch + ch;
         if (live && lead) {
             hand.v[nidx] = (int)(((unsigned)v1 << 16) | ((unsigned)v0 & 0xFFFFu));
             hand.token[nidx] = state;
@@ -1173,31 +1174,63 @@
     }
 }
 
-__global__ __launch_bounds__(64) void gc_slow_groups_kernel(const int16_t *__restrict__ coefs, int nch, int groups8, int *__restrict__ order)
-{
-    const int lane = threadIdx.x;
-    auto flagged = [&](int g) {
+constexpr int PROLOGUE_THREADS = 1024;
+__global__ __launch_bounds__(PROLOGUE_THREADS) void gc_self_served_prologue_kernel(
+    const int16_t *__restrict__ coefs, int nch, int groups8, int *__restrict__ order, int *__restrict__ zero, int64_t zero_ints,
+    int *__restrict__ token_row, int *__restrict__ first_open)
+{
+    const int64_t step = (int64_t)gridDim.x * PROLOGUE_THREADS;
+    for (int64_t i = (int64_t)blockIdx.x * PROLOGUE_THREADS + threadIdx.x; i < zero_ints; i += step) zero[i] = 0;
+    for (int64_t i = (int64_t)blockIdx.x * PROLOGUE_THREADS + threadIdx.x; i < nch; i += step) {
+        token_row[i] = 0;
+        first_open[i] = SEAM_NONE;
+    }
+    if (blockIdx.x != 0 || order == nullptr) return;
+    __shared__ int s_wave[PROLOGUE_THREADS / 64];
+    const int t = threadIdx.x, lane = t & 63, wave = t >> 6;
+    int *flag = order + groups8 + 1;
+    for (int base = 0; base < groups8; base += PROLOGUE_THREADS / 8) {
+        const int g = base + (t >> 3), pr = t & 7;
         bool slow = false;
         if (g < groups8)
-            for (int s = 0; s < PLAN8_SLOTS; s++) {
-                const int ch = g * PLAN8_SLOTS + s;
-                if (ch < nch) slow = plan8_slow_channel(coefs + (int64_t)ch * 16) || slow;
-            }
-        return slow;
-    };
-    int total = 0;
-    for (int base = 0; base < groups8; base += 64) total += __popcll(__ballot(flagged(base + lane)));
-    int s = 0, r = total;
-    const unsigned long long lower = (1ull << lane) - 1;
-    for (int base = 0; base < groups8; base += 64) {
-        const int g = base + lane;
-        const bool f = flagged(g);
-        const unsigned long long m = __ballot(f), rest = __ballot(!f && g < groups8);
-        if (g < groups8) order[f ? s + __popcll(m & lower) : r + __popcll(rest & lower)] = g;
-        s += __popcll(m);
-        r += __popcll(rest);
-    }
-    if (lane == 0) order[groups8] = total;
+            for (int sl = 0; sl < PLAN8_SLOTS; sl++) {
+                const int ch = g * PLAN8_SLOTS + sl;
+                if (ch < nch) slow = plan8_slow_predictor(coefs[(int64_t)ch * 16 + 2 * pr], coefs[(int64_t)ch * 16 + 2 * pr + 1]) || slow;
+            }
+        const unsigned long long m = __ballot(slow);
+        if (g < groups8 && pr == 0) flag[g] = ((m >> (lane & 56)) & 0xFFull) != 0 ? 1 : 0;
+    }
+    __syncthreads();
+    const int run = (groups8 + PROLOGUE_THREADS - 1) / PROLOGUE_THREADS;
+    const int g0 = imin(t * run, groups8), g1 = imin(g0 + run, groups8);
+    int mine = 0;
+    for (int g = g0; g < g1; g++) mine += flag[g];
+    int inc = mine;
+#pragma unroll
+    for (int o = 1; o < 64; o <<= 1) {
+        const int up = __shfl_up(inc, o);
+        if (lane >= o) inc += up;
+    }
+    if (lane == 63) s_wave[wave] = inc;
+    __syncthreads();
+    int before = 0, total = 0;
+    for (int w = 0; w < PROLOGUE_THREADS / 64; w++) {
+        const int c = s_wave[w];
+        before += w < wave ? c : 0;
+        total += c;
+    }
+    int s = before + inc - mine;
+    for (int g = g0; g < g1; g++) {
+        const int f = flag[g];
+        order[f ? s : total + (g - s)] = g;
+        s += f;
+    }
+    if (t == 0) order[groups8] = total;
+}
+static int prologue_workgroups(int64_t zero_ints, int nch)
+{
+    const int64_t want = (zero_ints + 2 * (int64_t)nch + 4 * PROLOGUE_THREADS - 1) / (4 * PROLOGUE_THREADS);
+    return want < 1 ? 1 : want > 64 ? 64 : (int)want;
 }
 extern "C" int vga_testing_gc_slow_order_host(const int16_t *coefs, int nch, int *order)
 {
@@ -1208,29 +1241,50 @@
         if (plan8_slow_channel(coefs + (int64_t)ch * 16)) flagged[(size_t)(ch / PLAN8_SLOTS)] = 1;
     return plan8_slow_order(flagged.data(), groups8, order);
 }
+extern "C" int vga_testing_gc_prologue_device(const void *d_coefs, int nch, int zero_ints, int *order_flags, int *bad_words)
+{
+    if (!d_coefs || !order_flags || nch <= 0 || zero_ints < 0) return -1;
+    const int groups8 = (nch + PLAN8_SLOTS - 1) / PLAN8_SLOTS;
+    const size_t n_order = (size_t)2 * groups8 + 1, n_all = n_order + (size_t)zero_ints + 2 * (size_t)nch + 4;
+    int *d = nullptr;
+    if (hipMalloc(&d, n_all * sizeof(int)) != hipSuccess) return -1;
+    std::vector<int> host(n_all);
+    bool ok = hipMemset(d, 0xFF, n_all * sizeof(int)) == hipSuccess;
+    int *d_zero = d + n_order, *d_token = d_zero + zero_ints, *d_open = d_token + nch;
+    if (ok) {
+        hipLaunchKernelGGL(gc_self_served_prologue_kernel, dim3(prologue_workgroups(zero_ints, nch)), dim3(PROLOGUE_THREADS), 0, (hipStream_t)0,
+                           static_cast<const int16_t *>(d_coefs), nch, groups8, d, d_zero, (int64_t)zero_ints, d_token, d_open);
+        ok = hipGetLastError() == hipSuccess && hipMemcpy(host.data(), d, n_all * sizeof(int), hipMemcpyDeviceToHost) == hipSuccess;
+    }
+    (void)hipFree(d);
+    if (!ok) return -1;
+    for (size_t i = 0; i < n_order; i++) order_flags[i] = host[i];
+    int bad = 0;
+    for (size_t i = 0; i < (size_t)zero_ints + (size_t)nch; i++) bad += host[n_order + i] != 0;
+    for (int i = 0; i < nch; i++) bad += host[n_order + (size_t)zero_ints + (size_t)nch + (size_t)i] != SEAM_NONE;
+    for (int i = 0; i < 4; i++) bad += host[n_all - 4 + (size_t)i] != -1;
+    if (bad_words) *bad_words = bad;
+    return host[(size_t)groups8];
+}
 extern "C" int vga_testing_gc_slow_order_device(const void *d_coefs, int nch, int *order)
 {
     if (!d_coefs || !order || nch <= 0) return -1;
     const int groups8 = (nch + PLAN8_SLOTS - 1) / PLAN8_SLOTS;
-    int *d_order = nullptr;
-    if (hipMalloc(&d_order, (size_t)(groups8 + 1) * sizeof(int)) != hipSuccess) return -1;
-    hipLaunchKernelGGL(gc_slow_groups_kernel, dim3(1), dim3(64), 0, (hipStream_t)0, static_cast<const int16_t *>(d_coefs), nch, groups8, d_order);
-    std::vector<int> host((size_t)groups8 + 1);
-    const bool ok = hipGetLastError() == hipSuccess &&
-                    hipMemcpy(host.data(), d_order, host.size() * sizeof(int), hipMemcpyDeviceToHost) == hipSuccess;
-    (void)hipFree(d_order);
-    if (!ok) return -1;
-    for (int g = 0; g < groups8; g++) order[g] = host[(size_t)g];
-    return host[(size_t)groups8];
+    std::vector<int> table((size_t)2 * groups8 + 1);
+    const int s = vga_testing_gc_prologue_device(d_coefs, nch, 0, table.data(), nullptr);
+    if (s < 0) return -1;
+    for (int g = 0; g < groups8; g++) order[g] = table[(size_t)g];
+    return s;
 }
 
 template <bool RAGGED>
 __global__ __launch_bounds__(64) __attribute__((amdgpu_waves_per_eu(3, 3))) void gc_encode_self_served_kernel(
-    const int16_t *__restrict__ pcm, int64_t pcm_pitch, int nch, int total_samples, const Pieces seg,
+    const int16_t *__restrict__ pcm, int64_t pcm_pitch, int nch, int total_samples, const std::conditional_t<RAGGED, Pieces, TailPieces> seg,
     const int16_t *__restrict__ coefs, const int16_t *__restrict__ hist1,
     const int16_t *__restrict__ hist2, uint8_t *adpcm, int64_t adpcm_pitch, int16_t *seg_state,
     const Ragged rg, int groups, int items, int segments, int *__restrict__ queue, int *__restrict__ seam_count, int *first_open,
-    int *seam_flag, int *seam_end, int force_open, const Handover hand, const int *__restrict__ slow_order)
+    int *seam_flag, int *seam_end, int force_open, const Handover hand, const int *__restrict__ slow_order, const TailPieces segc,
+    int segments_c)
 {
     constexpr int CS = PLAN8_SLOTS;
     static_assert(Lay<8, true>::CS == CS && Lay<8, true>::THREADS == 64, "one wave, eight channel slots");
@@ -1238,6 +1292,10 @@
     const uint32_t *host_items = RAGGED ? rg.items : nullptr;
     const int *order = RAGGED ? nullptr : slow_order;
     const int slow = order ? order[groups] : 0;
+    const bool two = !RAGGED && order != nullptr && segments_c > 0;
+    const int front = two ? slow * segments_c : 0;
+    if (two) items = front + (groups - slow) * segments;
+    const int rec_row = (two && segments_c > segments ? segments_c : segments) - 1;
 #ifdef VGA_DEBUG_TIMESTAMPS
     if (lane == 0) g_vga_enc_ts[2 * (blockIdx.x & 32767)] = wall_clock64();
 #endif
@@ -1252,15 +1310,23 @@
             return;
         }
         int g, y;
-        if (!plan8_item(item, groups, nch, host_items, order, slow, segments, g, y)) continue;
-        gc_encode_piece<false, 8, RAGGED, true>(g, y, pcm, pcm_pitch, nch, total_samples, seg, coefs, hist1, hist2, adpcm, adpcm_pitch,
+        const bool coarse = two && item < front;
+        if (!plan8_item(item, groups, nch, host_items, order, slow, two ? segments_c : segments, g, y)) continue;
+        std::conditional_t<RAGGED, Pieces, TailPieces> sg = seg;
+        int ns = segments;
+        if constexpr (!RAGGED)
+            if (coarse) {
+                sg = segc;
+                ns = segments_c;
+            }
+        gc_encode_piece<false, 8, RAGGED, true, std::conditional_t<RAGGED, Pieces, TailPieces>>(g, y, pcm, pcm_pitch, nch, total_samples, sg, coefs, hist1, hist2, adpcm, adpcm_pitch,
                                                 seg_state, (const int *)nullptr, rg);
-        if (segments <= 1) continue;
+        if (ns <= 1) continue;
         __threadfence();
         int at_start = 0, at_end = 0;
         if (lane == 0) {
             const int total_wg = RAGGED ? rg.length[rg.order[g * CS]] : total_samples;
-            auto exists = [&](int piece) { return piece < segments && seg.first(piece) * 14 < total_wg; };
+            auto exists = [&](int piece) { return piece < ns && sg.first(piece) * 14 < total_wg; };
             if (exists(y)) {
                 if (y >= 1 && atomicAdd(&seam_count[(int64_t)(y - 1) * groups + g], 1) == 1) at_start = y;
                 if (exists(y + 1) && atomicAdd(&seam_count[(int64_t)y * groups + g], 1) == 1) at_end = y + 1;
@@ -1278,19 +1344,19 @@
                     seam_piece<8>(slot, seam_b, lane, pcm, pcm_pitch, nch, total_samples, seg, coefs, adpcm, adpcm_pitch, seg_state,
                                first_open, seam_flag, seam_end, force_open, rg);
             } else
-                self_served_seams(g, seam_a, seam_b, lane, groups, segments, pcm, pcm_pitch, nch, total_samples, seg, coefs, adpcm,
+                self_served_seams(g, seam_a, seam_b, lane, groups, ns, rec_row, pcm, pcm_pitch, nch, total_samples, sg, coefs, adpcm,
                                   adpcm_pitch, seg_state, first_open, seam_flag, seam_end, force_open, hand);
         }
     }
 }
 
-template <int LPC>
-__global__ __launch_bounds__(64) void gc_encode_chain_kernel(
-    const int16_t *__restrict__ pcm, int64_t pcm_pitch, int nch, int total_samples, const Pieces seg, int segments,
+template <int LPC, class P>
+__device__ __forceinline__ void chain_walk(
+    const int16_t *__restrict__ pcm, int64_t pcm_pitch, int nch, int total_samples, const P seg, int segments,
     const int16_t *__restrict__ coefs, uint8_t *__restrict__ adpcm, int64_t adpcm_pitch,
     int16_t *__restrict__ seg_state, int *__restrict__ first_open, const int *__restrict__ seam_flag,
-    const int *__restrict__ seam_end, int force_open, const Ragged rg, const int *__restrict__ hand_token,
-    const int *__restrict__ hand_v)
+    const int *__restrict__ seam_end, int force_open, const Ragged &rg, const int *__restrict__ hand_token,
+    const int *__restrict__ hand_v, const int rec_row)
 {
     const int lane = threadIdx.x;
     const int pr = LPC == 16 ? (lane >> 1) & 7 : lane & 7;
@@ -1300,7 +1366,7 @@
     const int slot = live ? slot_raw : nch - 1;
     const int ch = rg.order ? rg.order[slot] : slot;
     if (rg.order) total_samples = rg.length[ch];
-    const int64_t rec_idx = (int64_t)(segments - 1) * nch + ch;
+    const int64_t rec_idx = (int64_t)rec_row * nch + ch;
     const int record = hand_token && live ? hand_token[rec_idx] : 0;
     const bool resolved = record != 0;
     const int mine_raw = live ? first_open[ch] : SEAM_NONE;
@@ -1366,6 +1432,28 @@
     if (live && lead && frames_run) atomicAdd(&g_vga_gc_stats[2], (unsigned long long)frames_run);
     if (live && lead) first_open[ch] = SEAM_NONE;
 }
+template <int LPC>
+__global__ __launch_bounds__(64) void gc_encode_chain_kernel(
+    const int16_t *__restrict__ pcm, int64_t pcm_pitch, int nch, int total_samples, const Pieces seg, int segments,
+    const int16_t *__restrict__ coefs, uint8_t *__restrict__ adpcm, int64_t adpcm_pitch,
+    int16_t *__restrict__ seg_state, int *__restrict__ first_open, const int *__restrict__ seam_flag,
+    const int *__restrict__ seam_end, int force_open, const Ragged rg, const int *__restrict__ hand_token,
+    const int *__restrict__ hand_v)
+{
+    chain_walk<LPC, Pieces>(pcm, pcm_pitch, nch, total_samples, seg, segments, coefs, adpcm, adpcm_pitch, seg_state, first_open, seam_flag, seam_end,
+                            force_open, rg, hand_token, hand_v, segments - 1);
+}
+__global__ __launch_bounds__(64) void gc_encode_chain_tail_kernel(
+    const int16_t *__restrict__ pcm, int64_t pcm_pitch, int nch, int total_samples, const TailPieces seg, int segments,
+    const int16_t *__restrict__ coefs, uint8_t *__restrict__ adpcm, int64_t adpcm_pitch,
+    int16_t *__restrict__ seg_state, int *__restrict__ first_open, const int *__restrict__ seam_flag,
+    const int *__restrict__ seam_end, int force_open, const int *__restrict__ hand_token,
+    const int *__restrict__ hand_v, int rec_row, const int *__restrict__ slow_flag, const TailPieces segc, int segments_c)
+{
+    const bool coarse = slow_flag != nullptr && slow_flag[blockIdx.x] != 0;
+    chain_walk<8, TailPieces>(pcm, pcm_pitch, nch, total_samples, coarse ? segc : seg, coarse ? segments_c : segments, coefs, adpcm, adpcm_pitch,
+                              seg_state, first_open, seam_flag, seam_end, force_open, Ragged{}, hand_token, hand_v, rec_row);
+}
 
 constexpr int MIN_PIECE_FRAMES = 3584;
 
@@ -1378,6 +1466,10 @@
 constexpr int PERSISTENT_SMALL_FRAMES = 4096;
 constexpr int SELF_SERVED_BIG_ROUNDS = 4;
 constexpr int SELF_SERVED_SMALL_ROUNDS = 1;
+constexpr int SELF_SERVED_TAIL_ROUNDS[3] = {1, 1, 1};
+constexpr int SELF_SERVED_TAIL_FRAMES[3] = {4096, 2048, 1024};
+constexpr int SELF_SERVED_MIN_TAIL_FRAMES = 1024;
+constexpr int SELF_SERVED_COARSE_FRAMES = 4096;
 constexpr int MAX_PIECES = 1024;
 
 static int persistent_wgs_per_cu()
@@ -1394,6 +1486,15 @@
 }
 
 int plan_encode_pieces_on(int cus, int groups, int frames, int64_t group_frames, bool ragged, bool *persistent_out, Pieces *seg_out, int layout)
+{
+    TailPieces seg;
+    const int segments = plan_encode_tail_pieces_on(cus, groups, frames, group_frames, ragged, persistent_out, &seg, layout, true);
+    *seg_out = seg.two();
+    return segments;
+}
+
+int plan_encode_tail_pieces_on(int cus, int groups, int frames, int64_t group_frames, bool ragged, bool *persistent_out, TailPieces *seg_out,
+                               int layout, bool coarse)
 {
     const bool self = layout == 1;
     const int pmode = encoder_persistent_mode();
@@ -1410,42 +1511,74 @@
     if (segments < 1) segments = 1;
     if (segments > MAX_PIECES) segments = MAX_PIECES;
     if (encoder_segments_override() > 0) segments = imin(imin(imax(frames / 64, 1), encoder_segments_override()), MAX_PIECES);
-    Pieces seg;
+    TailPieces seg;
     seg.big = (frames + segments - 1) / segments;
     seg.nb = segments;
     seg.small = seg.big;
-    if (persistent && encoder_segments_override() <= 0 && frames >= 4 * MIN_PIECE_FRAMES &&
-        (ragged || groups * PERSISTENT_SCHEDULE_GROUPS_FACTOR >= cus * 4)) {
-        int big_rounds = ragged ? PERSISTENT_BIG_ROUNDS + 1 : PERSISTENT_BIG_ROUNDS, small_rounds = PERSISTENT_SMALL_ROUNDS, small = PERSISTENT_SMALL_FRAMES;
-        if (self && !ragged) { big_rounds = SELF_SERVED_BIG_ROUNDS; small_rounds = SELF_SERVED_SMALL_ROUNDS; }
+    const int *forced = self && !ragged ? gc_schedule_override() : nullptr;
+    if (persistent && encoder_segments_override() <= 0 &&
+        (forced || (frames >= 4 * MIN_PIECE_FRAMES && (ragged || groups * PERSISTENT_SCHEDULE_GROUPS_FACTOR >= cus * 4)))) {
+        int big_rounds = ragged ? PERSISTENT_BIG_ROUNDS + 1 : PERSISTENT_BIG_ROUNDS;
+        int rounds[3] = {PERSISTENT_SMALL_ROUNDS, 0, 0}, size[3] = {PERSISTENT_SMALL_FRAMES, 0, 0}, count[3] = {-1, -1, -1}, floor = MIN_PIECE_FRAMES;
+        if (self && !ragged) {
+            big_rounds = SELF_SERVED_BIG_ROUNDS;
+            rounds[0] = SELF_SERVED_SMALL_ROUNDS;
+            if (!coarse) {
+                for (int i = 0; i < 3; i++) { rounds[i] = SELF_SERVED_TAIL_ROUNDS[i]; size[i] = SELF_SERVED_TAIL_FRAMES[i]; }
+                floor = SELF_SERVED_MIN_TAIL_FRAMES;
+            }
+        }
 #ifdef VGA_TUNING
-        if (const char *e = std::getenv("VGA_HIP_GC_SCHEDULE")) std::sscanf(e, "%d,%d,%d", &big_rounds, &small_rounds, &small);
-#endif
-        small = imax(small, MIN_PIECE_FRAMES);
+        if (const char *e = std::getenv("VGA_HIP_GC_SCHEDULE"))
+            if (!coarse) std::sscanf(e, "%d,%d,%d,%d,%d,%d,%d", &big_rounds, &rounds[0], &size[0], &rounds[1], &size[1], &rounds[2], &size[2]);
+#endif
+        if (forced) {
+            big_rounds = forced[0];
+            floor = forced[7];
+            for (int i = 0; i < 3; i++) { count[i] = forced[1 + i]; size[i] = forced[4 + i]; rounds[i] = 0; }
+            if (coarse) {
+                floor = size[0] = imax(size[0], imin(SELF_SERVED_COARSE_FRAMES, 4 * floor));
+                count[1] = count[2] = 0;
+            }
+        }
         big_rounds = imax(big_rounds, 1);
         const int wgs = cus * (self ? PLAN8_WGS_PER_CU : persistent_wgs_per_cu());
         const int queue_groups = self ? 2 * groups : groups;
         const int64_t per_wg = group_frames * (self ? 2 : 1) / wgs + 1;
-        int ns = (small_rounds * wgs + queue_groups / 2) / queue_groups;
-        if ((int64_t)ns * small > frames / 2) ns = frames / (2 * small);
-        int big = (int)imax((int)((per_wg - (int64_t)small_rounds * small) / big_rounds), small);
-        int nb = (int)((frames - (int64_t)ns * small + big - 1) / big);
+        int64_t tail = 0, tail_share = 0;
+        for (int i = 0; i < 3; i++) {
+            size[i] = imax(size[i], floor);
+            if (i > 0) size[i] = imin(size[i], size[i - 1]);
+            const bool given = count[i] >= 0;
+            if (!given) count[i] = (rounds[i] * wgs + queue_groups / 2) / queue_groups;
+            if (tail + (int64_t)count[i] * size[i] > frames / 2) count[i] = (int)((frames / 2 - tail) / size[i]);
+            tail += (int64_t)count[i] * size[i];
+            tail_share += given ? (int64_t)count[i] * size[i] * queue_groups / wgs : (int64_t)rounds[i] * size[i];
+        }
+        const int small = size[0];
+        int big = (int)imax((int)((per_wg - tail_share) / big_rounds), small);
+        int nb = (int)((frames - tail + big - 1) / big);
         if (nb < 1) nb = 1;
-        if (!ragged) big = (int)((frames - (int64_t)ns * small + nb - 1) / nb);
+        if (!ragged) big = (int)((frames - tail + nb - 1) / nb);
         if (big < small) big = small;
+        seg = TailPieces{};
         seg.big = big;
         seg.nb = nb;
         seg.small = small;
-        segments = nb + ns;
+        if (count[2] > 0) { seg.n1 = count[0]; seg.s2 = size[1]; seg.n2 = count[1]; seg.s3 = size[2]; }
+        else if (count[1] > 0) { seg.n1 = count[0]; seg.s2 = size[1]; }
+        segments = nb + count[0] + count[1] + count[2];
         while (segments > 1 && seg.first(segments - 1) >= frames) segments--;
         if (segments > MAX_PIECES) {
             segments = MAX_PIECES;
+            seg = TailPieces{};
             seg.big = seg.small = (frames + segments - 1) / segments;
             seg.nb = segments;
             while (segments > 1 && seg.first(segments - 1) >= frames) segments--;
         }
     }
     if (seg.first(segments) < frames) {
+        seg = TailPieces{};
         seg.big = seg.small = (frames + segments - 1) / segments;
         seg.nb = segments;
     }
@@ -1489,19 +1622,33 @@
                                       want_self ? 1 : CPW);
     }
     const bool self = want_self && persistent;
+    TailPieces tseg, segc;
+    int segments_c = 0;
+    if (self && !RAGGED) {
+        bool p = false;
+        segments = plan_encode_tail_pieces_on(cus, groups, frames, (int64_t)groups * frames, false, &p, &tseg, 1, false);
+        seg = tseg.two();
+    }
     const Plan8 p8 = self ? plan_groups_of_eight(cus, nch, segments, RAGGED && rg.items ? rg.n_items : -1) : Plan8{};
     const int seam_groups = self ? p8.groups : groups;
     AsyncBuf scratch;
     int16_t *seg_state = nullptr;
     int *first_open = nullptr, *seam_flag = nullptr, *seam_end = nullptr, *queue = nullptr, *seam_count = nullptr;
     const bool handover = self && !RAGGED && segments > 1 && !gc_seam_handover_off();
+    if (handover) {
+        bool p = false;
+        segments_c = plan_encode_tail_pieces_on(cus, groups, frames, (int64_t)groups * frames, false, &p, &segc, 1, true);
+        if (segments_c == segments && segc.same_as(tseg)) segments_c = 0;
+    }
+    const bool tail_chain = self && !RAGGED && (segments_c > 0 || !tseg.two_sizes());
+    const int rows = imax(segments, segments_c);
     Handover hand;
     int *slow_order = nullptr;
     if (segments > 1 || persistent) {
-        const size_t state_bytes = segments > 1 ? (size_t)round_up((int64_t)segments * nch * 2 * (int64_t)sizeof(int16_t), 16) : 0;
+        const size_t state_bytes = segments > 1 ? (size_t)round_up((int64_t)rows * nch * 2 * (int64_t)sizeof(int16_t), 16) : 0;
         const size_t open_bytes = (size_t)round_up((int64_t)nch * (int64_t)sizeof(int), 16);
-        const size_t count_bytes = persistent && segments > 1 ? (size_t)round_up((int64_t)(segments - 1) * seam_groups * (int64_t)sizeof(int), 16) : 0;
-        const size_t order_bytes = handover ? (size_t)round_up((int64_t)(seam_groups + 1) * (int64_t)sizeof(int), 16) : 0;
+        const size_t count_bytes = persistent && segments > 1 ? (size_t)round_up((int64_t)(rows - 1) * seam_groups * (int64_t)sizeof(int), 16) : 0;
+        const size_t order_bytes = handover ? (size_t)round_up((int64_t)(2 * seam_groups + 1) * (int64_t)sizeof(int), 16) : 0;
         const size_t need = 3 * state_bytes + open_bytes + 16 + count_bytes + (handover ? count_bytes + 2 * state_bytes + order_bytes : 0);
         unsigned char *base = static_cast<unsigned char *>(d_scratch);
         if (!base || scratch_bytes < need) {
@@ -1514,26 +1661,33 @@
         queue = reinterpret_cast<int *>(base + 3 * state_bytes + open_bytes);
         if (segments > 1) {
             seg_state = reinterpret_cast<int16_t *>(base);
-            VGA_HIP_TRY(fill_no_open_seams(first_open, nch, stream));
+            if (!handover) VGA_HIP_TRY(fill_no_open_seams(first_open, nch, stream));
         } else
             seg_state = nullptr;
         seam_count = queue + 4;
-        if (persistent) VGA_HIP_TRY(hipMemsetAsync(queue, 0, 16 + count_bytes * (handover ? 2 : 1), stream));
+        if (persistent && !handover) VGA_HIP_TRY(hipMemsetAsync(queue, 0, 16 + count_bytes, stream));
         if (handover) {
             unsigned char *words = base + 3 * state_bytes + open_bytes + 16 + count_bytes;
             hand.word = reinterpret_cast<int *>(words);
             hand.token = reinterpret_cast<int *>(words + count_bytes);
             hand.v = reinterpret_cast<int *>(words + count_bytes + state_bytes);
             slow_order = reinterpret_cast<int *>(words + count_bytes + 2 * state_bytes);
-            VGA_HIP_TRY(hipMemsetAsync(hand.token + (size_t)(segments - 1) * nch, 0, (size_t)nch * sizeof(int), stream));
+            if constexpr (CPW == 8 && !RAGGED) {
+                const int64_t zero_ints = (int64_t)(16 + 2 * count_bytes) / (int64_t)sizeof(int);
+                hipLaunchKernelGGL(gc_self_served_prologue_kernel, dim3(prologue_workgroups(zero_ints, nch)), dim3(PROLOGUE_THREADS), 0, stream,
+                                   d_coefs, nch, p8.groups, slow_order, queue, zero_ints, hand.token + (size_t)(rows - 1) * nch, first_open);
+                VGA_HIP_TRY(hipGetLastError());
+            }
         }
     }
     if (self) {
         if constexpr (CPW == 8) {
-            if (slow_order) hipLaunchKernelGGL(gc_slow_groups_kernel, dim3(1), dim3(64), 0, stream, d_coefs, nch, p8.groups, slow_order);
+            std::conditional_t<RAGGED, Pieces, TailPieces> self_seg;
+            if constexpr (RAGGED) self_seg = seg; else self_seg = tseg;
             hipLaunchKernelGGL((gc_encode_self_served_kernel<RAGGED>), dim3(p8.wgs), dim3(Lay<8, true>::THREADS), 0, stream, d_pcm, pcm_pitch,
-                               nch, sample_count, seg, d_coefs, d_hist1, d_hist2, d_adpcm, adpcm_pitch, seg_state, rg, p8.groups, p8.items,
-                               segments, queue, seam_count, first_open, seam_flag, seam_end, force_open_seams(), hand, (const int *)slow_order);
+                               nch, sample_count, self_seg, d_coefs, d_hist1, d_hist2, d_adpcm, adpcm_pitch, seg_state, rg, p8.groups, p8.items,
+                               segments, queue, seam_count, first_open, seam_flag, seam_end, force_open_seams(), hand, (const int *)slow_order, segc,
+                               segments_c);
         }
     } else if (persistent) {
         const int items = RAGGED && rg.items ? rg.n_items : groups * segments;
@@ -1564,6 +1718,12 @@
                                    force_open_seams(), rg);
             VGA_HIP_TRY(hipGetLastError());
         }
+        if (tail_chain)
+            hipLaunchKernelGGL(gc_encode_chain_tail_kernel, dim3((nch + 7) / 8), dim3(64), 0, stream, d_pcm, pcm_pitch, nch, sample_count, tseg,
+                               segments, d_coefs, d_adpcm, adpcm_pitch, seg_state, first_open, seam_flag, seam_end, force_open_seams(),
+                               (const int *)hand.token, (const int *)hand.v, rows - 1,
+                               (const int *)(segments_c > 0 ? slow_order + seam_groups + 1 : nullptr), segc, segments_c);
+        else
 #ifdef VGA_GC_SEAM16_ALWAYS
         if (CPW == 4)
 #else
diff --git a/vgaudio_amd/csrc/gcadpcm_kernels.hpp b/vgaudio_amd/csrc/gcadpcm_kernels.hpp
--- a/vgaudio_amd/csrc/gcadpcm_kernels.hpp
+++ b/vgaudio_amd/csrc/gcadpcm_kernels.hpp
@@ -10,9 +10,26 @@
     __host__ __device__ int64_t first(int k) const { return (int64_t)(k < nb ? k : nb) * big + (int64_t)(k > nb ? k - nb : 0) * small; }
     __host__ __device__ int frames(int k) const { return k < nb ? big : small; }
 };
+constexpr int PIECES_NO_END = 1 << 30;
+struct TailPieces {
+    int big = 0, nb = 0, small = 0;
+    int n1 = PIECES_NO_END, s2 = 0, n2 = PIECES_NO_END, s3 = 0;
+    __host__ __device__ int64_t first(int k) const
+    {
+        const int t = k > nb ? k - nb : 0;
+        const int a = t < n1 ? t : n1, b = t - a < n2 ? t - a : n2;
+        return (int64_t)(k < nb ? k : nb) * big + (int64_t)a * small + (int64_t)b * s2 + (int64_t)(t - a - b) * s3;
+    }
+    __host__ __device__ int frames(int k) const { return k < nb ? big : k - nb < n1 ? small : k - nb - n1 < n2 ? s2 : s3; }
+    bool two_sizes() const { return n1 == PIECES_NO_END; }
+    Pieces two() const { Pieces p; p.big = big; p.nb = nb; p.small = small; return p; }
+    bool same_as(const TailPieces &o) const { return big == o.big && nb == o.nb && small == o.small && n1 == o.n1 && s2 == o.s2 && n2 == o.n2 && s3 == o.s3; }
+};
 int encoder_plan_layout(int groups, bool ragged);
 int plan_encode_pieces(int groups, int frames, int64_t group_frames, bool ragged, bool *persistent, Pieces *seg, int layout = 8);
 int plan_encode_pieces_on(int cus, int groups, int frames, int64_t group_frames, bool ragged, bool *persistent, Pieces *seg, int layout = 8);
+int plan_encode_tail_pieces_on(int cus, int groups, int frames, int64_t group_frames, bool ragged, bool *persistent, TailPieces *seg, int layout,
+                               bool coarse);
 
 struct Ragged {
     const uint32_t *items = nullptr;
diff --git a/vgaudio_amd/csrc/host_batch.hpp b/vgaudio_amd/csrc/host_batch.hpp
--- a/vgaudio_amd/csrc/host_batch.hpp
+++ b/vgaudio_amd/csrc/host_batch.hpp
@@ -32,6 +32,7 @@
     int encoder_persistent = 0;
     int hca_frames_per_group = 0;
     int gc_seam_handover_off = 0;
+    int gc_schedule[8] = {0, 0, 0, 0, 0, 0, 0, 0};
     PipeOverride pipe;
     FailStep fail;
 };
diff --git a/vgaudio_amd/csrc/runtime.hip b/vgaudio_amd/csrc/runtime.hip
--- a/vgaudio_amd/csrc/runtime.hip
+++ b/vgaudio_amd/csrc/runtime.hip
@@ -45,6 +45,7 @@
 int encoder_persistent_mode() { return g_settings.encoder_persistent; }
 int hca_frames_per_group_override() { return g_settings.hca_frames_per_group; }
 bool gc_seam_handover_off() { return g_settings.gc_seam_handover_off != 0; }
+const int *gc_schedule_override() { return g_settings.gc_schedule[0] > 0 ? g_settings.gc_schedule : nullptr; }
 static thread_local int g_adx_encode_path = 0, g_adx_decode_path = 0;
 void note_adx_encode_path(int path) { g_adx_encode_path = path; }
 void note_adx_decode_path(int path) { g_adx_decode_path = path; }
@@ -166,6 +167,20 @@
 {
     const int old = g_settings.gc_seam_handover_off ? 0 : 1;
     g_settings.gc_seam_handover_off = on ? 0 : 1;
+    return old;
+}
+int vga_testing_gc_schedule_this_thread(int big_rounds, const int *tail_counts, const int *tail_frames, int min_tail_frames)
+{
+    int *s = g_settings.gc_schedule;
+    const int old = s[0];
+    for (int i = 0; i < 8; i++) s[i] = 0;
+    if (big_rounds <= 0 || !tail_counts || !tail_frames) return old;
+    s[0] = big_rounds;
+    s[7] = min_tail_frames < 64 ? 64 : min_tail_frames;
+    for (int i = 0; i < 3; i++) {
+        s[1 + i] = tail_counts[i] > 0 ? tail_counts[i] : 0;
+        s[4 + i] = tail_frames[i] < s[7] ? s[7] : tail_frames[i];
+    }
     return old;
 }
 int vga_testing_hca_frames_per_group_this_thread(int frames)
```

Measured after the change: 93870 Msamples/s, median of 6. 1.03x the previous value.
